# pmandros/node2vec2rank

Hardware: AMD Instinct MI355X
Metric: nodes ranked/sec + SpMM HBM GB/s, K-layer N-node graph at 1/2/4/8 GPUs (higher is better)
Workload: dtype fp32; 1 GPU; cfg4: 2-layer ER N=1M avg-deg 50, dims {8,16,32,64,128} x {cosine,euclidean}, sequential; nodes=1000000, layers=2, embed_dim=128, columns=10, comparisons=1, parallelism=single GPU

## Files before the change

### include/n2v2r.h

```cpp
#ifndef N2V2R_H
#define N2V2R_H

#include <stddef.h>
#include <stdint.h>

#ifdef __cplusplus
extern "C" {
#endif

typedef enum {
  N2V2R_OK = 0,
  N2V2R_ERR_BAD_ARG = 1,
  N2V2R_ERR_UNSUPPORTED_METRIC = 2,
  N2V2R_ERR_NO_CONVERGENCE = 3,
  N2V2R_ERR_HIP = 4,
  N2V2R_ERR_OUT_OF_MEMORY = 5,
  N2V2R_ERR_NOT_READY = 6,
  N2V2R_ERR_UNSUPPORTED_AGG = 7,
  N2V2R_ERR_INTERNAL = 8,
  N2V2R_ERR_RCCL = 9
} n2v2r_status;

enum { N2V2R_SEQUENTIAL = 0, N2V2R_ONE_VS_BEFORE = 1, N2V2R_ONE_VS_REST = 2 };
enum { N2V2R_COSINE = 0, N2V2R_EUCLIDEAN = 1, N2V2R_CORRELATION = 2 };
enum { N2V2R_SYM_DETECT = -1, N2V2R_SYM_NO = 0, N2V2R_SYM_YES = 1 };
enum { N2V2R_AGG_BORDA = 0, N2V2R_AGG_NONE = -1 };

enum { N2V2R_EIG_FULL_FIRST_PASS = 1, N2V2R_EIG_DENSE_RR = 2,
       N2V2R_EIG_TEST_REDO_CYCLE = 4 ,
       N2V2R_EIG_TEST_BAND_FAIL = 8 ,
       N2V2R_EIG_TEST_STURM_FAIL = 32 ,
       N2V2R_EIG_TIME_SPMM = 16 ,
       N2V2R_EIG_TEST_NO_STAGNATION = 64 ,
       N2V2R_EIG_TEST_FAIL_ALONE = 128  };

typedef struct n2v2r_handle n2v2r_handle;
typedef struct n2v2r_simgroup n2v2r_simgroup;

typedef struct {
  int block;
  int max_basis;
  int keep;
  int max_restarts;
  double tol;
  uint64_t seed;
  int solver_flags;
} n2v2r_eig_opts;

typedef struct {
  int restarts;
  int block_applications;
  int converged;
  int basis;
  double max_residual;
  double ms_total, ms_spmm, ms_ortho, ms_rr_host;
  int64_t spmm_launches;
  double spmm_algo_bytes;
  int stagnated;
  int rr_fallbacks;
  double gpu_ms_spmm[2];
  int64_t spmm_timed_launches[2];
  double spmm_stage_bytes[2];
  double est_scale;
  int lean_checks;
  int pool_blocks;
  int spmm_form;
  double stag_cap;
  int y_captured;
  int tri_fallbacks;
} n2v2r_eig_stats;

int n2v2r_create(int device, n2v2r_handle** out);
void n2v2r_destroy(n2v2r_handle* h);
int n2v2r_last_error(const n2v2r_handle* h, char* buf, size_t len);
const char* n2v2r_version(void);

#define N2V2R_UNIQUE_ID_BYTES 128
int n2v2r_comm_unique_id(char* out, size_t len);
int n2v2r_create_rccl(int device, int rank, int world, const char* unique_id, n2v2r_handle** out);
int n2v2r_simgroup_create(int world, n2v2r_simgroup** out);
void n2v2r_simgroup_destroy(n2v2r_simgroup* g);
int n2v2r_create_sim(int device, n2v2r_simgroup* g, int rank, n2v2r_handle** out);
int n2v2r_dist_info(const n2v2r_handle* h, int* rank, int* world, int64_t* row0, int64_t* n_local);

int n2v2r_create_multi(const int* devices, int n_gpus, n2v2r_handle** out);
int n2v2r_multi_devices(const n2v2r_handle* h, int* devices, int cap);

int n2v2r_set_num_layers(n2v2r_handle* h, int num_layers, int64_t n);
int n2v2r_set_layer_csr(n2v2r_handle* h, int k, int64_t n, int64_t nnz, const int64_t* indptr,
                        const int32_t* indices, const float* data, int symmetric);
int n2v2r_set_layer_dense(n2v2r_handle* h, int k, int64_t n, const float* A, int symmetric);
enum { N2V2R_CORR_UNSIGNED = 0, N2V2R_CORR_SIGNED = 1, N2V2R_CORR_SIGNED_HYBRID = 2,
       N2V2R_CORR_RAW = 3 };
int n2v2r_set_layer_corr(n2v2r_handle* h, int k, int64_t n, int64_t samples,
                         const double* E , int kind, double power);
int n2v2r_set_layer_csr_rows(n2v2r_handle* h, int k, int64_t n, int64_t row0, int64_t n_rows,
                             int64_t nnz, const int64_t* indptr, const int32_t* indices,
                             const float* data);

int n2v2r_uase(n2v2r_handle* h, int d, const n2v2r_eig_opts* opts, n2v2r_eig_stats* stats);
int n2v2r_get_embedding(n2v2r_handle* h, float* Y );
int n2v2r_get_left_embedding(n2v2r_handle* h, float* X );
int n2v2r_get_singular_values(n2v2r_handle* h, double* s );
int n2v2r_set_embedding(n2v2r_handle* h, int num_layers, int64_t n, int d, const float* Y);

int n2v2r_rank(n2v2r_handle* h, int strategy, const int* dims, int n_dims, const int* metrics,
               int n_metrics, int method, int* n_comparisons, int* n_cols);
int n2v2r_get_distances(n2v2r_handle* h, int comparison, double* D );
int n2v2r_get_borda(n2v2r_handle* h, int comparison, int64_t* borda );
int n2v2r_rank_timing(n2v2r_handle* h, double* ms_distances, double* ms_borda);

int n2v2r_pairwise_distances(n2v2r_handle* h, const double* m1, const double* m2, int64_t n,
                             int dim, int metric, double* out);
int n2v2r_borda_columns(n2v2r_handle* h, const double* D , int64_t n,
                        int n_cols, int64_t* borda);
int n2v2r_column_sums(n2v2r_handle* h, int k, float* out );
int n2v2r_borda_columns_ex(n2v2r_handle* h, const double* D , int64_t n,
                           int n_cols, const int32_t* given_cols, int n_given,
                           const int32_t* given_orders, int64_t* borda, int32_t* tied);

int n2v2r_project(n2v2r_handle* h, int64_t m, int64_t n, const double* W, int on_columns,
                  double* out);

int n2v2r_synchronize(n2v2r_handle* h);


#ifdef __cplusplus
}
#endif

#endif
```

### include/n2v2r_diag.h

```cpp
#ifndef N2V2R_DIAG_H
#define N2V2R_DIAG_H

#include "n2v2r.h"

#ifdef __cplusplus
extern "C" {
#endif

int n2v2r_bench_spmm(n2v2r_handle* h, int k, int transpose, int b, int reps, const float* X,
                     float* Y, double* avg_ms, double* algo_bytes);
int n2v2r_bench_spmm_tiled(n2v2r_handle* h, int k, int transpose, int b, int nb, int reps,
                           const float* X, float* Y, double* avg_ms);

int n2v2r_spmm_col_blocks(const n2v2r_handle* h, int b);

int n2v2r_rr_top(n2v2r_handle* h, int c, const double* H, int p, double* w, float* S);

int n2v2r_rr_band_top(n2v2r_handle* h, int c, int kp, const double* hband, int64_t hband_len,
                      const double* theta_prev, int p, double* w, float* S);

int n2v2r_h2d_layer_bytes(const n2v2r_handle* h, int64_t* per_rank, int cap);

int n2v2r_get_layer_dense(n2v2r_handle* h, int k, float* A );

#ifdef __cplusplus
}
#endif

#endif
```

### node2vec2rank_amd/_lib.py

```python
from __future__ import annotations

import atexit
import ctypes
import os
import threading
import weakref

import numpy as np

from .coexpression import Coexpression

_HERE = os.path.dirname(os.path.abspath(__file__))
LIB_PATH = os.environ.get("N2V2R_LIB", os.path.join(_HERE, "lib", "libn2v2r_hip.so"))

OK = 0
ERR_BAD_ARG = 1
ERR_UNSUPPORTED_METRIC = 2
ERR_NO_CONVERGENCE = 3
ERR_HIP = 4
ERR_OUT_OF_MEMORY = 5
ERR_NOT_READY = 6
ERR_UNSUPPORTED_AGG = 7
ERR_INTERNAL = 8
ERR_RCCL = 9
AGG_BORDA, AGG_NONE = 0, -1
EIG_TIME_SPMM = 16
EIG_TEST_NO_STAGNATION = 64
EIG_TEST_FAIL_ALONE = 128

STRATEGY = {"sequential": 0, "one_vs_before": 1, "one_vs_rest": 2}
METRIC = {"cosine": 0, "euclidean": 1, "correlation": 2}
SYM_DETECT, SYM_NO, SYM_YES = -1, 0, 1

EXPORTED = [
    "n2v2r_create", "n2v2r_destroy", "n2v2r_last_error", "n2v2r_version",
    "n2v2r_set_num_layers", "n2v2r_set_layer_csr", "n2v2r_uase", "n2v2r_get_embedding",
    "n2v2r_get_left_embedding", "n2v2r_get_singular_values", "n2v2r_set_embedding",
    "n2v2r_rank", "n2v2r_get_distances", "n2v2r_get_borda", "n2v2r_rank_timing",
    "n2v2r_pairwise_distances", "n2v2r_borda_columns", "n2v2r_borda_columns_ex",
    "n2v2r_column_sums",
    "n2v2r_synchronize", "n2v2r_bench_spmm", "n2v2r_bench_spmm_tiled", "n2v2r_spmm_col_blocks",
    "n2v2r_comm_unique_id", "n2v2r_create_rccl", "n2v2r_simgroup_create",
    "n2v2r_simgroup_destroy", "n2v2r_create_sim", "n2v2r_dist_info", "n2v2r_set_layer_csr_rows",
    "n2v2r_rr_top", "n2v2r_rr_band_top", "n2v2r_set_layer_dense", "n2v2r_project",
    "n2v2r_create_multi", "n2v2r_multi_devices", "n2v2r_h2d_layer_bytes",
    "n2v2r_set_layer_corr", "n2v2r_get_layer_dense",
]
UNIQUE_ID_BYTES = 128


class ArpackNoConvergence(RuntimeError):
    """UASE eigensolver did not reach the residual tolerance (scipy raises
    ``ArpackNoConvergence`` in the reference's svds path)."""


class EigOpts(ctypes.Structure):
    _fields_ = [("block", ctypes.c_int), ("max_basis", ctypes.c_int), ("keep", ctypes.c_int),
                ("max_restarts", ctypes.c_int), ("tol", ctypes.c_double),
                ("seed", ctypes.c_uint64), ("solver_flags", ctypes.c_int)]


class EigStats(ctypes.Structure):
    _fields_ = [("restarts", ctypes.c_int), ("block_applications", ctypes.c_int),
                ("converged", ctypes.c_int), ("basis", ctypes.c_int),
                ("max_residual", ctypes.c_double), ("ms_total", ctypes.c_double),
                ("ms_spmm", ctypes.c_double), ("ms_ortho", ctypes.c_double),
                ("ms_rr_host", ctypes.c_double), ("spmm_launches", ctypes.c_int64),
                ("spmm_algo_bytes", ctypes.c_double), ("stagnated", ctypes.c_int),
                ("rr_fallbacks", ctypes.c_int), ("gpu_ms_spmm", ctypes.c_double * 2),
                ("spmm_timed_launches", ctypes.c_int64 * 2),
                ("spmm_stage_bytes", ctypes.c_double * 2), ("est_scale", ctypes.c_double),
                ("lean_checks", ctypes.c_int), ("pool_blocks", ctypes.c_int),
                ("spmm_form", ctypes.c_int), ("stag_cap", ctypes.c_double),
                ("y_captured", ctypes.c_int), ("tri_fallbacks", ctypes.c_int)]

    def as_dict(self):
        out = {}
        for k, _ in self._fields_:
            v = getattr(self, k)
            out[k] = list(v) if isinstance(v, ctypes.Array) else v
        return out


_lib = None
_lock = threading.RLock()

_vp = ctypes.c_void_p
_i = ctypes.c_int
_i64 = ctypes.c_int64


def _p(dtype):
    return np.ctypeslib.ndpointer(dtype=dtype, flags="C_CONTIGUOUS")


def load(path: str | None = None):
    global _lib
    with _lock:
        if _lib is not None:
            return _lib
        p = path or LIB_PATH
        if not os.path.exists(p):
            raise RuntimeError(
                f"n2v2r HIP library not found at {p}; build it with "
                "`python -m node2vec2rank_amd.build` (there is no CPU fallback)")
        lib = ctypes.CDLL(p)
        atexit.register(_teardown)
        sig = {
            "n2v2r_create": (_i, [_i, ctypes.POINTER(_vp)]),
            "n2v2r_destroy": (None, [_vp]),
            "n2v2r_last_error": (_i, [_vp, ctypes.c_char_p, ctypes.c_size_t]),
            "n2v2r_version": (ctypes.c_char_p, []),
            "n2v2r_set_num_layers": (_i, [_vp, _i, _i64]),
            "n2v2r_set_layer_csr": (_i, [_vp, _i, _i64, _i64, _p(np.int64), _p(np.int32),
                                         _p(np.float32), _i]),
            "n2v2r_uase": (_i, [_vp, _i, ctypes.POINTER(EigOpts), ctypes.POINTER(EigStats)]),
            "n2v2r_get_embedding": (_i, [_vp, _p(np.float32)]),
            "n2v2r_get_left_embedding": (_i, [_vp, _p(np.float32)]),
            "n2v2r_get_singular_values": (_i, [_vp, _p(np.float64)]),
            "n2v2r_set_embedding": (_i, [_vp, _i, _i64, _i, _p(np.float32)]),
            "n2v2r_rank": (_i, [_vp, _i, _p(np.int32), _i, _p(np.int32), _i, _i,
                                ctypes.POINTER(_i), ctypes.POINTER(_i)]),
            "n2v2r_get_distances": (_i, [_vp, _i, _p(np.float64)]),
            "n2v2r_get_borda": (_i, [_vp, _i, _p(np.int64)]),
            "n2v2r_rank_timing": (_i, [_vp, ctypes.POINTER(ctypes.c_double),
                                       ctypes.POINTER(ctypes.c_double)]),
            "n2v2r_pairwise_distances": (_i, [_vp, _p(np.float64), _p(np.float64), _i64, _i, _i,
                                              _p(np.float64)]),
            "n2v2r_borda_columns": (_i, [_vp, _p(np.float64), _i64, _i, _p(np.int64)]),
            "n2v2r_borda_columns_ex": (_i, [_vp, _p(np.float64), _i64, _i, _vp, _i, _vp,
                                            _p(np.int64), _p(np.int32)]),
            "n2v2r_column_sums": (_i, [_vp, _i, _p(np.float32)]),
            "n2v2r_synchronize": (_i, [_vp]),
            "n2v2r_bench_spmm": (_i, [_vp, _i, _i, _i, _i, _p(np.float32), _vp,
                                      ctypes.POINTER(ctypes.c_double),
                                      ctypes.POINTER(ctypes.c_double)]),
            "n2v2r_bench_spmm_tiled": (_i, [_vp, _i, _i, _i, _i, _i, _p(np.float32), _vp,
                                            ctypes.POINTER(ctypes.c_double)]),
            "n2v2r_spmm_col_blocks": (_i, [_vp, _i]),
            "n2v2r_rr_top": (_i, [_vp, _i, _p(np.float64), _i, _p(np.float64), _p(np.float32)]),
            "n2v2r_rr_band_top": (_i, [_vp, _i, _i, _p(np.float64), ctypes.c_int64, _vp, _i,
                                       _p(np.float64), _p(np.float32)]),
            "n2v2r_set_layer_dense": (_i, [_vp, _i, _i64, _p(np.float32), _i]),
            "n2v2r_project": (_i, [_vp, _i64, _i64, _p(np.float64), _i, _p(np.float64)]),
            "n2v2r_comm_unique_id": (_i, [ctypes.c_char_p, ctypes.c_size_t]),
            "n2v2r_create_rccl": (_i, [_i, _i, _i, ctypes.c_char_p, ctypes.POINTER(_vp)]),
            "n2v2r_simgroup_create": (_i, [_i, ctypes.POINTER(_vp)]),
            "n2v2r_simgroup_destroy": (None, [_vp]),
            "n2v2r_create_sim": (_i, [_i, _vp, _i, ctypes.POINTER(_vp)]),
            "n2v2r_dist_info": (_i, [_vp, ctypes.POINTER(_i), ctypes.POINTER(_i),
                                     ctypes.POINTER(_i64), ctypes.POINTER(_i64)]),
            "n2v2r_set_layer_csr_rows": (_i, [_vp, _i, _i64, _i64, _i64, _i64, _p(np.int64),
                                              _p(np.int32), _p(np.float32)]),
            "n2v2r_create_multi": (_i, [_p(np.int32), _i, ctypes.POINTER(_vp)]),
            "n2v2r_multi_devices": (_i, [_vp, _vp, _i]),
            "n2v2r_h2d_layer_bytes": (_i, [_vp, _vp, _i]),
            "n2v2r_set_layer_corr": (_i, [_vp, _i, _i64, _i64, _p(np.float64), _i,
                                          ctypes.c_double]),
            "n2v2r_get_layer_dense": (_i, [_vp, _i, _p(np.float32)]),
        }
        for name, (res, args) in sig.items():
            f = getattr(lib, name)
            f.restype = res
            f.argtypes = args
        _lib = lib
        return lib


def comm_unique_id() -> bytes:
    lib = load()
    buf = ctypes.create_string_buffer(UNIQUE_ID_BYTES)
    st = lib.n2v2r_comm_unique_id(buf, UNIQUE_ID_BYTES)
    if st != OK:
        raise RuntimeError(f"n2v2r_comm_unique_id failed with status {st}")
    return buf.raw


class SimGroup:

    def __init__(self, world: int):
        self.lib = load()
        g = _vp()
        st = self.lib.n2v2r_simgroup_create(int(world), ctypes.byref(g))
        if st != OK:
            raise RuntimeError(f"n2v2r_simgroup_create failed with status {st}")
        self.g = g
        self.world = int(world)

    def close(self):
        if getattr(self, "g", None):
            self.lib.n2v2r_simgroup_destroy(self.g)
            self.g = None


_live = weakref.WeakSet()


def _teardown():
    for eng in list(_live):
        try:
            eng.close()
        except Exception:
            pass
    path = os.environ.get("N2V2R_EXIT_MAPS")
    if path:
        try:
            with open("/proc/self/maps") as src, open(path, "w") as dst:
                dst.write(src.read())
        except OSError:
            pass


class Engine:

    def __init__(self, device: int = 0, _handle=None):
        self.lib = load()
        if _handle is None:
            h = _vp()
            st = self.lib.n2v2r_create(int(device), ctypes.byref(h))
            if st != OK:
                raise RuntimeError(
                    f"n2v2r_create(device={device}) failed with status {st}: no usable HIP GPU "
                    "(the engine has no CPU fallback)")
        else:
            h = _handle
        self.h = h
        self.device = device
        _live.add(self)

    @classmethod
    def rccl(cls, device: int, rank: int, world: int, unique_id: bytes) -> "Engine":
        lib = load()
        h = _vp()
        st = lib.n2v2r_create_rccl(int(device), int(rank), int(world), bytes(unique_id),
                                   ctypes.byref(h))
        if st != OK:
            raise RuntimeError(f"n2v2r_create_rccl(rank={rank}, world={world}) failed: {st}")
        return cls(device, _handle=h)

    @classmethod
    def multi(cls, devices) -> "Engine":
        lib = load()
        devs = np.ascontiguousarray([int(d) for d in devices], dtype=np.int32)
        h = _vp()
        st = lib.n2v2r_create_multi(devs, int(devs.size), ctypes.byref(h))
        if st != OK:
            raise RuntimeError(f"n2v2r_create_multi(devices={devs.tolist()}) failed with status "
                               f"{st}" + (" (RCCL)" if st == ERR_RCCL else ""))
        eng = cls(int(devs[0]), _handle=h)
        eng.devices = tuple(int(d) for d in devs)
        return eng

    @classmethod
    def sim(cls, device: int, group: SimGroup, rank: int) -> "Engine":
        lib = load()
        h = _vp()
        st = lib.n2v2r_create_sim(int(device), group.g, int(rank), ctypes.byref(h))
        if st != OK:
            raise RuntimeError(f"n2v2r_create_sim(rank={rank}) failed with status {st}")
        return cls(device, _handle=h)

    def h2d_layer_bytes(self):
        out = np.zeros(64, dtype=np.int64)
        w = self.lib.n2v2r_h2d_layer_bytes(self.h, out.ctypes.data_as(ctypes.c_void_p), 64)
        if w < 0:
            self._check(w, "h2d_layer_bytes")
        return [int(x) for x in out[:w]]

    def dist_info(self):
        r, w, r0, nl = _i(), _i(), _i64(), _i64()
        self._check(self.lib.n2v2r_dist_info(self.h, ctypes.byref(r), ctypes.byref(w),
                                             ctypes.byref(r0), ctypes.byref(nl)), "dist_info")
        return r.value, w.value, r0.value, nl.value

    def close(self):
        if getattr(self, "h", None):
            self.lib.n2v2r_destroy(self.h)
            self.h = None

    def __del__(self):
        try:
            self.close()
        except Exception:
            pass

    def _err(self) -> str:
        buf = ctypes.create_string_buffer(1024)
        self.lib.n2v2r_last_error(self.h, buf, len(buf))
        return buf.value.decode(errors="replace")

    def _check(self, st: int, what: str):
        if st == OK:
            return
        msg = f"{what}: {self._err()}"
        if st == ERR_UNSUPPORTED_METRIC:
            raise NotImplementedError("Unsupported metric")
        if st == ERR_UNSUPPORTED_AGG:
            raise NotImplementedError("Aggregation method not found. Available methods: Borda")
        if st == ERR_NOT_READY:
            raise ValueError("No n2v2r embeddings found")
        if st == ERR_NO_CONVERGENCE:
            raise ArpackNoConvergence(msg)
        if st == ERR_OUT_OF_MEMORY:
            raise MemoryError(msg)
        if st == ERR_BAD_ARG:
            raise ValueError(msg)
        if st == ERR_RCCL:
            raise RuntimeError(f"RCCL failure: {msg}")
        raise RuntimeError(msg)

    def set_layers(self, layers, symmetric=SYM_DETECT, storage="auto"):
        import scipy.sparse as sp
        corr = [isinstance(a, Coexpression) for a in layers]
        if any(corr):
            if storage == "csr":
                raise ValueError("Coexpression layers are stored dense: storage='csr' does not "
                                 "apply")
            if any(sp.issparse(a) for a in layers):
                raise ValueError("a sparse layer cannot share a handle with Coexpression layers "
                                 "(all layers of a handle are CSR or all dense): pass it as a "
                                 "dense array")
            arrs = [a if c else np.ascontiguousarray(np.asarray(a), dtype=np.float32)
                    for a, c in zip(layers, corr)]
            n = arrs[0].shape[0]
            for a in arrs:
                if a.shape != (n, n):
                    raise ValueError("all layers must be square and share the node set")
            self._check(self.lib.n2v2r_set_num_layers(self.h, len(arrs), n), "set_num_layers")
            for k, a in enumerate(arrs):
                if isinstance(a, Coexpression):
                    st = self.lib.n2v2r_set_layer_corr(self.h, k, n, a.expression.shape[1],
                                                       a.expression, a.kind_id, a.power)
                else:
                    st = self.lib.n2v2r_set_layer_dense(self.h, k, n, a, int(symmetric))
                self._check(st, f"layer {k}")
            self.n = n
            self.num_layers = len(arrs)
            self.storage = "dense"
            return
        if storage == "auto":
            storage = "csr"
            if all(not sp.issparse(a) for a in layers):
                arrs = [np.asarray(a) for a in layers]
                if all(_denser_than_quarter(a) for a in arrs):
                    storage = "dense"
        if storage == "dense":
            arrs = [np.ascontiguousarray(np.asarray(a.todense() if sp.issparse(a) else a),
                                         dtype=np.float32) for a in layers]
            n = arrs[0].shape[0]
            for a in arrs:
                if a.shape != (n, n):
                    raise ValueError("all layers must be square and share the node set")
            self._check(self.lib.n2v2r_set_num_layers(self.h, len(arrs), n), "set_num_layers")
            for k, a in enumerate(arrs):
                self._check(self.lib.n2v2r_set_layer_dense(self.h, k, n, a, int(symmetric)),
                            f"layer {k}")
            self.n = n
            self.num_layers = len(arrs)
            self.storage = "dense"
            return
        mats = [sp.csr_matrix(a, dtype=np.float32) for a in layers]
        n = mats[0].shape[0]
        for m in mats:
            if m.shape != (n, n):
                raise ValueError("all layers must be square and share the node set")
        self._check(self.lib.n2v2r_set_num_layers(self.h, len(mats), n), "set_num_layers")
        for k, m in enumerate(mats):
            indptr = np.ascontiguousarray(m.indptr, dtype=np.int64)
            indices = np.ascontiguousarray(m.indices, dtype=np.int32)
            data = np.ascontiguousarray(m.data, dtype=np.float32)
            self._check(self.lib.n2v2r_set_layer_csr(self.h, k, n, int(m.nnz), indptr, indices,
                                                     data, int(symmetric)), f"layer {k}")
        self.n = n
        self.num_layers = len(mats)
        self.storage = "csr"

    def set_layer_rows(self, n: int, num_layers: int, local_layers):
        import scipy.sparse as sp
        self._check(self.lib.n2v2r_set_num_layers(self.h, int(num_layers), int(n)),
                    "set_num_layers")
        _, _, row0, nl = self.dist_info()
        for k, blk in enumerate(local_layers):
            m = sp.csr_matrix(blk, dtype=np.float32)
            m.sum_duplicates()
            m.sort_indices()
            if m.shape != (nl, n):
                raise ValueError(f"layer {k}: local block must be {nl} x {n}, got {m.shape}")
            self._check(self.lib.n2v2r_set_layer_csr_rows(
                self.h, k, int(n), int(row0), int(nl), int(m.nnz),
                np.ascontiguousarray(m.indptr, dtype=np.int64),
                np.ascontiguousarray(m.indices, dtype=np.int32),
                np.ascontiguousarray(m.data, dtype=np.float32)), f"layer {k} rows")
        self.n = int(n)
        self.num_layers = int(num_layers)

    def uase(self, d: int, block=0, max_basis=0, keep=0, max_restarts=0, tol=0.0, seed=0,
             solver_flags=0, raise_on_no_convergence=True):
        o = EigOpts(int(block), int(max_basis), int(keep), int(max_restarts), float(tol),
                    int(seed) & 0xFFFFFFFFFFFFFFFF, int(solver_flags))
        s = EigStats()
        st = self.lib.n2v2r_uase(self.h, int(d), ctypes.byref(o), ctypes.byref(s))
        if st == ERR_NO_CONVERGENCE and not raise_on_no_convergence:
            pass
        else:
            self._check(st, "uase")
        self.d = int(d)
        return s.as_dict()

    def _n_local(self):
        return self.dist_info()[3]

    def embedding(self):
        Y = np.empty((self.num_layers, self._n_local(), self.d), dtype=np.float32)
        self._check(self.lib.n2v2r_get_embedding(self.h, Y), "get_embedding")
        return Y

    def left_embedding(self):
        X = np.empty((self._n_local(), self.d), dtype=np.float32)
        self._check(self.lib.n2v2r_get_left_embedding(self.h, X), "get_left_embedding")
        return X

    def singular_values(self):
        s = np.empty(self.d, dtype=np.float64)
        self._check(self.lib.n2v2r_get_singular_values(self.h, s), "get_singular_values")
        return s

    def set_embedding(self, Y):
        Y = np.ascontiguousarray(Y, dtype=np.float32)
        K, n, d = Y.shape
        self._check(self.lib.n2v2r_set_embedding(self.h, K, n, d, Y), "set_embedding")
        self.num_layers, self.n, self.d = K, n, d

    def rank(self, strategy: str, dims, metrics, method: int = AGG_BORDA):
        if strategy not in STRATEGY:
            raise ValueError(f"unknown comp_strategy {strategy!r}")
        mids = []
        for m in metrics:
            if m not in METRIC:
                raise NotImplementedError("Unsupported metric")
            mids.append(METRIC[m])
        dims_a = np.ascontiguousarray(dims, dtype=np.int32)
        met_a = np.ascontiguousarray(mids, dtype=np.int32)
        ncmp = ctypes.c_int()
        ncol = ctypes.c_int()
        self._check(self.lib.n2v2r_rank(self.h, STRATEGY[strategy], dims_a, len(dims_a), met_a,
                                        len(met_a), int(method), ctypes.byref(ncmp),
                                        ctypes.byref(ncol)), "rank")
        self.ncmp, self.ncols = ncmp.value, ncol.value
        return self.ncmp, self.ncols

    def distances(self, comparison: int):
        D = np.empty((self.ncols, self.n), dtype=np.float64)
        self._check(self.lib.n2v2r_get_distances(self.h, int(comparison), D), "get_distances")
        return D.T

    def borda(self, comparison: int):
        b = np.empty(self.n, dtype=np.int64)
        self._check(self.lib.n2v2r_get_borda(self.h, int(comparison), b), "get_borda")
        return b

    def rank_timing(self):
        a, b = ctypes.c_double(), ctypes.c_double()
        self.lib.n2v2r_rank_timing(self.h, ctypes.byref(a), ctypes.byref(b))
        return a.value, b.value

    def pairwise_distances(self, m1, m2, metric: str):
        if metric not in METRIC:
            raise NotImplementedError("Unsupported metric")
        a = np.ascontiguousarray(m1, dtype=np.float64)
        b = np.ascontiguousarray(m2, dtype=np.float64)
        if a.ndim == 1:
            a = a[:, None]
            b = b[:, None]
        n, dim = a.shape
        out = np.empty(n, dtype=np.float64)
        self._check(self.lib.n2v2r_pairwise_distances(self.h, a, b, n, dim, METRIC[metric], out),
                    "pairwise_distances")
        return out

    def borda_columns(self, D, tie_order: str = "stable", return_tied: bool = False):
        if tie_order not in ("stable", "reference"):
            raise ValueError(f"unknown tie_order {tie_order!r}")
        Dc = np.ascontiguousarray(np.asarray(D, dtype=np.float64).T)
        c, n = Dc.shape
        out = np.empty(n, dtype=np.int64)
        tied = np.zeros(c, dtype=np.int32)
        self._check(self.lib.n2v2r_borda_columns_ex(self.h, Dc, n, c, None, 0, None, out, tied),
                    "borda_columns")
        cols = np.flatnonzero(tied)
        if tie_order == "reference" and cols.size:
            orders = np.empty((cols.size, n), dtype=np.int32)
            for g, j in enumerate(cols):
                orders[g] = reference_descending_order(Dc[j])
            gc = np.ascontiguousarray(cols, dtype=np.int32)
            self._check(self.lib.n2v2r_borda_columns_ex(
                self.h, Dc, n, c, gc.ctypes.data_as(_vp), int(cols.size),
                orders.ctypes.data_as(_vp), out, tied), "borda_columns")
        return (out, tied.astype(bool)) if return_tied else out

    def column_sums(self, k: int):
        out = np.empty(self.n, dtype=np.float32)
        self._check(self.lib.n2v2r_column_sums(self.h, int(k), out), "column_sums")
        return out

    def layer_dense(self, k: int):
        A = np.zeros((self.n, self.n), dtype=np.float32)
        self._check(self.lib.n2v2r_get_layer_dense(self.h, int(k), A), "layer_dense")
        return A

    def bench_spmm(self, k: int, X, transpose: bool = False, reps: int = 20, want_y=True):
        X = np.ascontiguousarray(X, dtype=np.float32)
        n, b = X.shape
        Y = np.empty((self._n_local(), b), dtype=np.float32) if want_y else None
        ms, by = ctypes.c_double(), ctypes.c_double()
        yp = Y.ctypes.data_as(ctypes.c_void_p) if want_y else None
        self._check(self.lib.n2v2r_bench_spmm(self.h, int(k), int(bool(transpose)), int(b),
                                              int(reps), X, yp, ctypes.byref(ms),
                                              ctypes.byref(by)), "bench_spmm")
        return Y, ms.value, by.value

    def bench_spmm_tiled(self, k: int, X, transpose: bool = False, nb: int = 0, reps: int = 20,
                         want_y=True):
        X = np.ascontiguousarray(X, dtype=np.float32)
        n, b = X.shape
        Y = np.empty((self._n_local(), b), dtype=np.float32) if want_y else None
        ms = ctypes.c_double()
        yp = Y.ctypes.data_as(ctypes.c_void_p) if want_y else None
        self._check(self.lib.n2v2r_bench_spmm_tiled(self.h, int(k), int(bool(transpose)), int(b),
                                                    int(nb), int(reps), X, yp, ctypes.byref(ms)),
                    "bench_spmm_tiled")
        return Y, ms.value

    def spmm_col_blocks(self, b: int = 8) -> bool:
        r = self.lib.n2v2r_spmm_col_blocks(self.h, int(b))
        if r < 0 or r > 1:
            self._check(r, "spmm_col_blocks")
        return r == 1

    def project(self, W, on: str = "columns"):
        W = np.ascontiguousarray(np.asarray(W), dtype=np.float64)
        m, n = W.shape
        oc = on.casefold() == "columns"
        if not oc and on.casefold() != "rows":
            raise ValueError("Unknown projection type, options are columns or rows")
        k = n if oc else m
        out = np.empty((k, k), dtype=np.float64)
        self._check(self.lib.n2v2r_project(self.h, m, n, W, int(oc), out), "project")
        return out

    def rr_top(self, H, p: int):
        H = np.ascontiguousarray(H, dtype=np.float64)
        c = H.shape[0]
        w = np.empty(p, dtype=np.float64)
        S = np.empty((c, p), dtype=np.float32)
        self._check(self.lib.n2v2r_rr_top(self.h, c, H, int(p), w, S), "rr_top")
        return w, S

    def rr_band_top(self, hband, c: int, kp: int, theta_prev, p: int):
        hband = np.ascontiguousarray(hband, dtype=np.float64).ravel()
        tp = None
        if kp > 0:
            tp = np.ascontiguousarray(theta_prev, dtype=np.float64)
        w = np.empty(p, dtype=np.float64)
        S = np.empty((c, p), dtype=np.float32)
        self._check(self.lib.n2v2r_rr_band_top(
            self.h, int(c), int(kp), hband, int(hband.size),
            None if tp is None else tp.ctypes.data_as(ctypes.c_void_p), int(p), w, S),
            "rr_band_top")
        return w, S

    def synchronize(self):
        self._check(self.lib.n2v2r_synchronize(self.h), "synchronize")


def reference_descending_order(col) -> np.ndarray:
    import pandas as pd
    return pd.Series(np.asarray(col, dtype=np.float64)).sort_values(
        ascending=False).index.to_numpy(dtype=np.int64)


_default = {}


def new_engine(device) -> Engine:
    if isinstance(device, tuple):
        return Engine.multi(device)
    return Engine(device)


def default_engine(device: int = 0) -> Engine:
    e = _default.get(device)
    if e is None or e.h is None:
        e = Engine(device)
        _default[device] = e
    return e


def _denser_than_quarter(a) -> bool:
    if a.size == 0:
        return False
    a2 = a.reshape(a.shape[0], -1) if a.ndim > 1 else a.reshape(1, -1)
    rows, cols = a2.shape
    stride = max(1, rows // max(1, (1 << 21) // max(1, cols)))
    if stride > 1:
        sample = a2[::stride]
        p = np.count_nonzero(sample) / sample.size
        if p > 0.3:
            return True
        if p < 0.2:
            return False
    need = a.size // 4
    step = max(1, (1 << 24) // max(1, cols))
    nz = 0
    for r in range(0, rows, step):
        nz += int(np.count_nonzero(a2[r:r + step]))
        if nz > need:
            return True
        if nz + (rows - r - step) * cols <= need:
            return False
    return nz > need


POOL_MAX = 4
_pool = {}
_pool_tick = [0]


def engine_owner(eng: Engine):
    ref = getattr(eng, "_owner", None)
    return ref() if ref is not None else None


def acquire_engine(device: int, owner) -> Engine:
    import weakref
    with _lock:
        handles = _pool.setdefault(device, [])
        handles[:] = [e for e in handles if e.h is not None]
        free = [e for e in handles if engine_owner(e) is None]
        if free:
            eng = free[0]
        elif len(handles) < POOL_MAX:
            eng = new_engine(device)
            handles.append(eng)
        else:
            eng = min(handles, key=lambda e: getattr(e, "_tick", 0))
            prev = engine_owner(eng)
            if prev is not None and hasattr(prev, "_hand_over"):
                prev._hand_over()
        _pool_tick[0] += 1
        eng._tick = _pool_tick[0]
        eng._owner = weakref.ref(owner)
        return eng
```

### node2vec2rank_amd/build.py

```python
from __future__ import annotations

import os
import subprocess
import sys

HERE = os.path.dirname(os.path.abspath(__file__))
CSRC = os.path.join(HERE, "csrc")
OUT_DIR = os.path.join(HERE, "lib")
_TAG = os.environ.get("N2V2R_BUILD_TAG", "")
LIB = os.path.join(OUT_DIR, f"libn2v2r_hip_{_TAG}.so" if _TAG else "libn2v2r_hip.so")
OBJ_DIR = os.path.join(OUT_DIR, f"obj_{_TAG}" if _TAG else "obj")

HIP_SOURCES = ["spmm.hip", "dense.hip", "gemm.hip", "corr.hip", "rank.hip", "rr.hip", "rr_band.hip",
               "rr_sturm.hip", "ingest.hip", "engine.cpp", "layers.cpp", "comm.cpp", "solver.cpp",
               "ranking.cpp", "multi.cpp"]
HOST_SOURCES: list = []
HEADERS = ["common.h", "spmm_args.h", "engine.h", os.path.join("..", "..", "include", "n2v2r.h"),
           os.path.join("..", "..", "include", "n2v2r_diag.h")]
ARCH = os.environ.get("N2V2R_OFFLOAD_ARCH", "gfx950")
_EXTRA = os.environ.get("N2V2R_EXTRA_HIP_FLAGS", "").split() if _TAG else []


def _hipcc():
    for c in (os.environ.get("HIPCC"), "/opt/rocm/bin/hipcc", "hipcc"):
        if c and (os.path.isabs(c) and os.path.exists(c) or not os.path.isabs(c)):
            return c
    raise RuntimeError("hipcc not found")


def _newer(target, deps):
    if not os.path.exists(target):
        return True
    t = os.path.getmtime(target)
    return any(os.path.getmtime(d) > t for d in deps if os.path.exists(d))


def build(force: bool = False, verbose: bool = False) -> str:
    os.makedirs(OBJ_DIR, exist_ok=True)
    hipcc = _hipcc()
    headers = [os.path.join(CSRC, h) for h in HEADERS]
    objs, cmds = [], []
    for src in HIP_SOURCES + HOST_SOURCES:
        path = os.path.join(CSRC, src)
        obj = os.path.join(OBJ_DIR, src + ".o")
        objs.append(obj)
        if not force and not _newer(obj, [path, __file__] + headers):
            continue
        if src in HIP_SOURCES:
            lang = ["-x", "hip"]
            cmd = [hipcc, *lang, f"--offload-arch={ARCH}", "-O3", "-std=c++17", "-fPIC",
                   "-munsafe-fp-atomics", *_EXTRA, "-c", path, "-o", obj]
        else:
            cmd = ["g++", "-O3", "-march=x86-64-v3", "-std=c++17", "-fPIC", "-c", path, "-o", obj]
        cmds.append(cmd)
    from concurrent.futures import ThreadPoolExecutor
    jobs = max(1, min(8, len(cmds), os.cpu_count() or 1))

    def _run(cmd):
        if verbose:
            print(" ".join(cmd), flush=True)
        subprocess.run(cmd, check=True)

    with ThreadPoolExecutor(jobs) as ex:
        list(ex.map(_run, cmds))
    if force or _newer(LIB, objs):
        tmp = LIB + ".tmp"
        cmd = [hipcc, f"--offload-arch={ARCH}", "-shared", "-fPIC", *objs, "-o", tmp,
               "-L/opt/rocm/lib", "-lrccl", "-Wl,-rpath,/opt/rocm/lib"]
        if verbose:
            print(" ".join(cmd), flush=True)
        subprocess.run(cmd, check=True)
        os.replace(tmp, LIB)
    return LIB


if __name__ == "__main__":
    print(build(force="--force" in sys.argv, verbose=True))
```

### node2vec2rank_amd/csrc/engine.cpp

```cpp
#include "engine.h"

using namespace n2v2r_int;

namespace n2v2r_int {
n2v2r_handle* new_handle(int device) {
  int count = 0;
  if (hipGetDeviceCount(&count) != hipSuccess || count <= 0) return nullptr;
  if (device < 0 || device >= count) return nullptr;
  auto* h = new (std::nothrow) n2v2r_handle();
  if (!h) return nullptr;
  h->device = device;
  if (hipSetDevice(device) != hipSuccess ||
      hipStreamCreateWithFlags(&h->stream, hipStreamNonBlocking) != hipSuccess) {
    delete h;
    return nullptr;
  }
  return h;
}

}

extern "C" {

const char* n2v2r_version(void) { return "n2v2r-mi355x 0.2.0 (gfx950)"; }

int n2v2r_create(int device, n2v2r_handle** out) {
  if (!out) return N2V2R_ERR_BAD_ARG;
  *out = nullptr;
  int count = 0;
  if (hipGetDeviceCount(&count) != hipSuccess || count <= 0) return N2V2R_ERR_HIP;
  if (device < 0 || device >= count) return N2V2R_ERR_BAD_ARG;
  n2v2r_handle* h = new_handle(device);
  if (!h) return N2V2R_ERR_HIP;
  *out = h;
  return N2V2R_OK;
}

void n2v2r_destroy(n2v2r_handle* h) {
  if (!h) return;
  if (h->multi()) {
    (void)multi_destroy(h);
    return;
  }
  (void)hipSetDevice(h->device);
  if (h->stream) (void)hipStreamSynchronize(h->stream);
  h->layers.clear();
  h->comm.reset();
  for (hipEvent_t& e : h->cb_ev)
    if (e) (void)hipEventDestroy(e);
  if (h->side) (void)hipStreamDestroy(h->side);
  if (h->pin) (void)hipHostFree(h->pin);
  for (hipEvent_t e : h->tev) (void)hipEventDestroy(e);
  if (h->cstream) (void)hipStreamSynchronize(h->cstream);
  for (hipEvent_t& e : h->cev)
    if (e) (void)hipEventDestroy(e);
  if (h->cstream) (void)hipStreamDestroy(h->cstream);
  if (h->stream) (void)hipStreamDestroy(h->stream);
  delete h;
}

int n2v2r_last_error(const n2v2r_handle* h, char* buf, size_t len) {
  if (!h || !buf || len == 0) return N2V2R_ERR_BAD_ARG;
  snprintf(buf, len, "%s", h->err.c_str());
  return N2V2R_OK;
}

int n2v2r_synchronize(n2v2r_handle* h) {
  if (h && h->multi()) return multi_synchronize(h);
  return guarded(h, [&]() -> int {
    HIPCHK(hipStreamSynchronize(h->stream));
    return N2V2R_OK;
  });
}

int n2v2r_rr_top(n2v2r_handle* h, int c, const double* H, int p, double* w, float* S) {
  if (h && h->multi()) h = h->ranks[0];
  return guarded(h, [&]() -> int {
    if (c < 3 || c > 768 || p < 1 || p > c || !H || !w || !S) return N2V2R_ERR_BAD_ARG;
    DevBuf a, tri, refl, y, s;
    a.ensure(sizeof(double) * c * c);
    tri.ensure(sizeof(double) * 3 * c);
    refl.ensure(sizeof(double) * c * c);
    y.ensure(sizeof(double) * c * p);
    s.ensure(sizeof(float) * c * p);
    HIPCHK(hipMemcpyAsync(a.p, H, sizeof(double) * c * c, hipMemcpyHostToDevice, h->stream));
    HIPCHK(hipStreamSynchronize(h->stream));
    double* t = tri.as<double>();
    DevBuf trs;
    trs.ensure(n2v2r_rr_tridiag_scratch_bytes(c));
    HIPCHK(n2v2r_launch_rr_tridiag(a.as<double>(), c, t, t + c, t + 2 * c, refl.as<double>(),
                                   trs.p, h->stream));
    DevBuf wd, scr;
    wd.ensure(sizeof(double) * p);
    scr.ensure(sizeof(double) * 6 * (size_t)((p + 63) / 64 * 64) * c);
    HIPCHK(n2v2r_launch_rr_tri_eig(t, t + c, c, p, wd.as<double>(), y.as<double>(),
                                   scr.as<double>(), h->stream));
    HIPCHK(hipMemcpyAsync(w, wd.p, sizeof(double) * p, hipMemcpyDeviceToHost, h->stream));
    DevBuf btf;
    btf.ensure(n2v2r_rr_bt_scratch_bytes(c));
    HIPCHK(n2v2r_launch_rr_backtransform(refl.as<double>(), t + 2 * c, c, y.as<double>(), p,
                                         s.as<float>(), p, btf.as<double>(), h->stream));
    HIPCHK(hipMemcpyAsync(S, s.p, sizeof(float) * c * p, hipMemcpyDeviceToHost, h->stream));
    HIPCHK(hipStreamSynchronize(h->stream));
    return N2V2R_OK;
  });
}

int n2v2r_rr_band_top(n2v2r_handle* h, int c, int kp, const double* hband, int64_t hband_len,
                      const double* theta_prev, int p, double* w, float* S) {
  if (h && h->multi()) h = h->ranks[0];
  return guarded(h, [&]() -> int {
    const int b = 8;
    if (c < 3 || c > 512 || c % b || kp % b || kp + b > 192 || kp >= c || p < 1 || p > c ||
        !hband || !w || !S || (kp > 0 && !theta_prev))
      return N2V2R_ERR_BAD_ARG;
    const int64_t need = (int64_t)(kp + b) * b + (int64_t)(c / b - kp / b - 1) * 2 * b * b;
    if (hband_len < need) return N2V2R_ERR_BAD_ARG;
    DevBuf hb, th, ab, va, ta, tri, y, s, er, rf;
    rf.ensure(sizeof(double) * c * n2v2r_rr_band_jm(c) * 9);
    hb.ensure(sizeof(double) * hband_len);
    th.ensure(sizeof(double) * c);
    ab.ensure(sizeof(double) * c * (b + 1));
    va.ensure(sizeof(double) * (kp + b) * (kp + b));
    ta.ensure(sizeof(double) * (kp + b));
    tri.ensure(sizeof(double) * 2 * c);
    y.ensure(sizeof(double) * c * p);
    s.ensure(sizeof(float) * c * p);
    er.ensure(4 * sizeof(int));
    HIPCHK(hipMemsetAsync(er.p, 0, 4 * sizeof(int), h->stream));
    HIPCHK(hipMemcpyAsync(hb.p, hband, sizeof(double) * hband_len, hipMemcpyHostToDevice,
                          h->stream));
    if (kp > 0)
      HIPCHK(hipMemcpyAsync(th.p, theta_prev, sizeof(double) * kp, hipMemcpyHostToDevice,
                            h->stream));
    HIPCHK(hipStreamSynchronize(h->stream));
    if (rr_sturm_enabled()) {
      DevBuf scr;
      scr.ensure(sizeof(double) * n2v2r_rr_sturm_scratch(c, p));
      HIPCHK(n2v2r_launch_rr_sturm(hb.as<double>(), c, kp, th.as<double>(), scr.as<double>(),
                                   scr.bytes / sizeof(double), y.as<double>(), s.as<float>(), p,
                                   p, er.as<int>(), h->stream));
      int e = 0;
      HIPCHK(hipMemcpyAsync(&e, er.p, sizeof(int), hipMemcpyDeviceToHost, h->stream));
      HIPCHK(hipMemcpyAsync(w, th.p, sizeof(double) * p, hipMemcpyDeviceToHost, h->stream));
      HIPCHK(hipMemcpyAsync(S, s.p, sizeof(float) * c * p, hipMemcpyDeviceToHost, h->stream));
      HIPCHK(hipStreamSynchronize(h->stream));
      if (!e) return N2V2R_OK;
      HIPCHK(hipMemsetAsync(er.p, 0, 4 * sizeof(int), h->stream));
      if (kp > 0)
        HIPCHK(hipMemcpyAsync(th.p, theta_prev, sizeof(double) * kp, hipMemcpyHostToDevice,
                              h->stream));
      HIPCHK(hipStreamSynchronize(h->stream));
    }
    HIPCHK(n2v2r_launch_rr_band(hb.as<double>(), c, kp, th.as<double>(), ab.as<double>(),
                                va.as<double>(), ta.as<double>(), tri.as<double>(),
                                tri.as<double>() + c, rf.as<double>(), y.as<double>(),
                                s.as<float>(), p, p, er.as<int>(), h->stream));
    int e = 0;
    HIPCHK(hipMemcpyAsync(&e, er.p, sizeof(int), hipMemcpyDeviceToHost, h->stream));
    HIPCHK(hipMemcpyAsync(w, th.p, sizeof(double) * p, hipMemcpyDeviceToHost, h->stream));
    HIPCHK(hipMemcpyAsync(S, s.p, sizeof(float) * c * p, hipMemcpyDeviceToHost, h->stream));
    HIPCHK(hipStreamSynchronize(h->stream));
    if (e) throw StatusFail{N2V2R_ERR_NO_CONVERGENCE, "banded Rayleigh-Ritz: bulge chase aborted"};
    return N2V2R_OK;
  });
}

int n2v2r_spmm_col_blocks(const n2v2r_handle* h, int b) {
  if (h && h->multi()) h = h->ranks[0];
  if (!h) return N2V2R_ERR_BAD_ARG;
  return col_blocks_wanted(h, b) ? 1 : 0;
}

static int time_tiled(n2v2r_handle* h, int k, int transpose, int nb, const float* xd, float* yd,
                      int reps, double* avg_ms, int b = 8) {
  if (nb <= 0) {
    nb = 4;
    while (nb < 64 && (double)h->n * 32.0 / nb > 2.0 * 1024 * 1024) nb *= 2;
  }
  if (nb != 4 && nb != 8 && nb != 16 && nb != 32 && nb != 64 && nb != 128) return N2V2R_ERR_BAD_ARG;
  LayerDev& L = *h->layers[k];
  const int wb = tile_wbits(h->layers, nb);
  if (!ensure_col_blocks(L, h->n, h->stream, nb, wb)) return N2V2R_ERR_BAD_ARG;
  const LayerDev::ColBlocks& cbs = (transpose && !L.symmetric) ? L.cb_t : L.cb;
  DevBuf tb;
  tb.ensure(sizeof(CsrBlk) * nb);
  HIPCHK(hipMemcpyAsync(tb.p, cbs.blk, sizeof(CsrBlk) * nb, hipMemcpyHostToDevice, h->stream));
  int ncu = 0;
  HIPCHK(hipDeviceGetAttribute(&ncu, hipDeviceAttributeMultiprocessorCount, h->device));
  SpmmTileArgs a{};
  a.blk = tb.as<CsrBlk>();
  a.X[0] = xd;
  a.Y[0] = yd;
  a.ldx = b;
  a.ldy = b;
  a.n = h->nloc;
  a.K = 1;
  a.nb = nb;
  a.sum = 0;
  a.tile_rows = n2v2r_spmm_tile_rows_b(h->nloc, ncu, b == 16 ? N2V2R_SPMM16_WPC : 2, wb, b);
  a.wbits = wb;
  a.width = b;
  HIPCHK(n2v2r_launch_spmm_tile(a, h->stream));
  hipEvent_t e0, e1;
  HIPCHK(hipEventCreate(&e0));
  HIPCHK(hipEventCreate(&e1));
  HIPCHK(hipEventRecord(e0, h->stream));
  for (int r = 0; r < reps; ++r) HIPCHK(n2v2r_launch_spmm_tile(a, h->stream));
  HIPCHK(hipEventRecord(e1, h->stream));
  HIPCHK(hipEventSynchronize(e1));
  float ms = 0.f;
  HIPCHK(hipEventElapsedTime(&ms, e0, e1));
  (void)hipEventDestroy(e0);
  (void)hipEventDestroy(e1);
  if (avg_ms) *avg_ms = (double)ms / reps;
  HIPCHK(hipStreamSynchronize(h->stream));
  return N2V2R_OK;
}

int n2v2r_bench_spmm(n2v2r_handle* h, int k, int transpose, int b, int reps, const float* X,
                     float* Y, double* avg_ms, double* algo_bytes) {
  if (h && h->multi()) h = h->ranks[0];
  return guarded(h, [&]() -> int {
    if (k < 0 || k >= h->K || !h->layers[k]->loaded || (b != 8 && b != 16 && b != 32 && b != 64) ||
        reps < 1 || !X)
      return N2V2R_ERR_BAD_ARG;
    const LayerDev& L = *h->layers[k];
    DevBuf xd, yd;
    xd.ensure(sizeof(float) * h->n * b);
    yd.ensure(sizeof(float) * std::max<int64_t>(h->nloc, 1) * b);
    HIPCHK(hipMemcpyAsync(xd.p, X, sizeof(float) * h->n * b, hipMemcpyHostToDevice, h->stream));
    if (L.dense) {
      const float* am = transpose ? L.dense_at() : L.dense_a();
      const float* bt = h->comm ? nullptr : (transpose ? L.dense_a() : L.dense_at());
      h->dense_apply(am, L.lda, xd.as<float>(), b, b, yd.as<float>(), b, 0.f, nullptr, bt);
      hipEvent_t e0, e1;
      HIPCHK(hipEventCreate(&e0));
      HIPCHK(hipEventCreate(&e1));
      HIPCHK(hipEventRecord(e0, h->stream));
      for (int r = 0; r < reps; ++r)
        h->dense_apply(am, L.lda, xd.as<float>(), b, b, yd.as<float>(), b, 0.f, nullptr, bt);
      HIPCHK(hipEventRecord(e1, h->stream));
      HIPCHK(hipEventSynchronize(e1));
      float ms = 0.f;
      HIPCHK(hipEventElapsedTime(&ms, e0, e1));
      (void)hipEventDestroy(e0);
      (void)hipEventDestroy(e1);
      if (avg_ms) *avg_ms = (double)ms / reps;
      if (algo_bytes)
        *algo_bytes = 4.0 * (double)h->nloc * (double)h->n + 4.0 * (double)(h->n + h->nloc) * b;
      if (Y)
        HIPCHK(hipMemcpyAsync(Y, yd.p, sizeof(float) * h->nloc * b, hipMemcpyDeviceToHost,
                              h->stream));
      HIPCHK(hipStreamSynchronize(h->stream));
      return N2V2R_OK;
    }
    if (col_blocks_wanted(h, b)) {
      double ms = 0.0;
      const int st_ = time_tiled(h, k, transpose, 0, xd.as<float>(), yd.as<float>(), reps, &ms);
      if (st_ == N2V2R_OK) {
        const CsrDev c0 = transpose ? L.csr_t() : L.csr();
        if (avg_ms) *avg_ms = ms;
        if (algo_bytes) *algo_bytes = spmm_algo_bytes(c0.nnz, c0.unit != 0, h->nloc, h->n, b);
        if (Y)
          HIPCHK(hipMemcpyAsync(Y, yd.p, sizeof(float) * h->nloc * b, hipMemcpyDeviceToHost,
                                h->stream));
        HIPCHK(hipStreamSynchronize(h->stream));
        return N2V2R_OK;
      }
    }
    SpmmArgs a{};
    a.K = 1;
    a.sum = 0;
    a.ldx = b;
    a.ldy = b;
    a.colscale = nullptr;
    a.A[0] = transpose ? L.csr_t() : L.csr();
    a.X[0] = xd.as<float>();
    a.Y[0] = yd.as<float>();
    HIPCHK(n2v2r_launch_spmm(a, b, h->stream));
    hipEvent_t e0, e1;
    HIPCHK(hipEventCreate(&e0));
    HIPCHK(hipEventCreate(&e1));
    HIPCHK(hipEventRecord(e0, h->stream));
    for (int r = 0; r < reps; ++r) HIPCHK(n2v2r_launch_spmm(a, b, h->stream));
    HIPCHK(hipEventRecord(e1, h->stream));
    HIPCHK(hipEventSynchronize(e1));
    float ms = 0.f;
    HIPCHK(hipEventElapsedTime(&ms, e0, e1));
    (void)hipEventDestroy(e0);
    (void)hipEventDestroy(e1);
    if (avg_ms) *avg_ms = (double)ms / reps;
    if (algo_bytes)
      *algo_bytes = spmm_algo_bytes(a.A[0].nnz, a.A[0].unit != 0, h->nloc, h->n, b);
    if (Y)
      HIPCHK(hipMemcpyAsync(Y, yd.p, sizeof(float) * h->nloc * b, hipMemcpyDeviceToHost,
                            h->stream));
    HIPCHK(hipStreamSynchronize(h->stream));
    return N2V2R_OK;
  });
}


int n2v2r_bench_spmm_tiled(n2v2r_handle* h, int k, int transpose, int b, int nb, int reps,
                           const float* X, float* Y, double* avg_ms) {
  if (h && h->multi()) h = h->ranks[0];
  return guarded(h, [&]() -> int {
    if (k < 0 || k >= h->K || !h->layers[k]->loaded || h->layers[k]->dense ||
        (b != 8 && b != 16) || reps < 1 || !X || h->comm)
      return N2V2R_ERR_BAD_ARG;
    DevBuf xd, yd;
    xd.ensure(sizeof(float) * h->n * b);
    yd.ensure(sizeof(float) * std::max<int64_t>(h->nloc, 1) * b);
    HIPCHK(hipMemcpyAsync(xd.p, X, sizeof(float) * h->n * b, hipMemcpyHostToDevice, h->stream));
    const int st_ =
        time_tiled(h, k, transpose, nb, xd.as<float>(), yd.as<float>(), reps, avg_ms, b);
    if (st_ != N2V2R_OK) return st_;
    if (Y)
      HIPCHK(hipMemcpyAsync(Y, yd.p, sizeof(float) * h->nloc * b, hipMemcpyDeviceToHost,
                            h->stream));
    HIPCHK(hipStreamSynchronize(h->stream));
    return N2V2R_OK;
  });
}

}
```

### node2vec2rank_amd/csrc/engine.h

```cpp
#pragma once

#include <hip/hip_runtime.h>
#include <rccl/rccl.h>

#include <algorithm>
#include <chrono>
#include <cmath>
#include <condition_variable>
#include <cstdarg>
#include <cstdlib>
#include <cstdio>
#include <cstring>
#include <memory>
#include <mutex>
#include <numeric>
#include <string>
#include <thread>
#include <exception>
#include <system_error>
#include <vector>

#include "../../include/n2v2r.h"
#include "../../include/n2v2r_diag.h"
#include "common.h"

#include "spmm_args.h"
#define DIST_MAX_COLS 256
struct DistPlan {
  int n_cols;
  int col_dim[DIST_MAX_COLS];
  int col_metric[DIST_MAX_COLS];
  int col_out[DIST_MAX_COLS];
  int dmax;
};
extern "C" {
hipError_t n2v2r_launch_spmm(const SpmmArgs& args, int B, hipStream_t stream);
int n2v2r_spmm_rpw(const SpmmArgs& args, int B);
hipError_t n2v2r_launch_row_sums(const CsrDev& A, float* out, hipStream_t stream);
hipError_t n2v2r_launch_spmm_tile(const SpmmTileArgs& a, hipStream_t stream);
hipError_t n2v2r_launch_chunk_major_keys(uint64_t* keys, int64_t nnz, int64_t npad, int W,
                                         int64_t rc, hipStream_t stream);
int n2v2r_spmm_tile_rows(int64_t n, int ncu, int wpc, int wbits);
int n2v2r_spmm_tile_rows_b(int64_t n, int ncu, int wpc, int wbits, int b);
hipError_t n2v2r_launch_cb_count(const CsrDev& A, int64_t cw, int nb, int32_t* cnt,
                                 hipStream_t stream);
hipError_t n2v2r_launch_cb_rowptrs(const int32_t* cnt, int64_t n, int nb, int64_t nnz,
                                   int64_t* tsum, size_t tsum_elems, int64_t* rp, int32_t* wo,
                                   int wbits, hipStream_t stream);
int64_t n2v2r_cb_scan_tiles(int64_t n, int nb);
hipError_t n2v2r_launch_cb_fill(const CsrDev& A, int64_t cw, int nb, const int64_t* rp,
                                int32_t* idx, float* dat, int cbits, int wbits,
                                hipStream_t stream);
hipError_t n2v2r_launch_ts_tn(const BlockList& A, const BlockList& B, int64_t n, double* partial,
                              size_t partial_elems, double* out, const int* cond,
                              hipStream_t stream);
hipError_t n2v2r_launch_ritz_nn(const BlockList& A0, const BlockList& A1, const float* G, int ldg,
                                int cb, const OutBlockList& O0, const OutBlockList& O1, int64_t n,
                                int grid, hipStream_t stream);
hipError_t n2v2r_launch_ts_nn(const BlockList& A, const float* G, int ldg, int cb,
                              const OutBlockList& O, const BlockList& C, float alpha, float beta,
                              int64_t n, const int* cond, const int* flags, uint64_t seed,
                              hipStream_t stream);
hipError_t n2v2r_launch_pip_chol(const double* G, int c, int b, double* xinv, int* flags,
                                 int* any_flag, const int* cond, double* save, int save_row0,
                                 int save_rows, float* fout, int* sticky, double* rsave,
                                 int first, hipStream_t stream);
hipError_t n2v2r_launch_rr_band(const double* hband, int c, int kp, double* theta, double* AB,
                                double* Varr, double* taua, double* d, double* e, double* refl,
                                double* Y, float* S, int ldS, int p, int* err,
                                hipStream_t stream);
int n2v2r_rr_band_jm(int c);
inline bool pip_fused() { return true; }
hipError_t n2v2r_launch_ts_tn2(const BlockList& A, const float* Za, const float* Zb, int64_t n,
                               double* partial, size_t partial_elems, double* out,
                               hipStream_t stream);
hipError_t n2v2r_launch_rmul8(const double* r2, double* r1, hipStream_t stream);
hipError_t n2v2r_launch_pair_fixup(double* g2, int nblk_all, int nq_old, double* ra,
                                   hipStream_t stream);
constexpr size_t N2V2R_PAIR_PLAN_WORDS = 208 + (size_t)(N2V2R_BAND_MAXC / 8) * 129;
hipError_t n2v2r_launch_pip_pair(const BlockList& Q, float* Za, float* Zb, double* g2, int64_t n,
                                 int* flags, int* any_flag, int* sticky, uint64_t seed_a,
                                 uint64_t seed_b, int64_t row0, float skip_tol, int* skipped,
                                 int* plan, size_t plan_bytes, hipStream_t stream);
hipError_t n2v2r_launch_pip_fused(const BlockList& Q, const float* Zin, float* Zout,
                                  const double* G, int c, int64_t n, const int* cond, int* flags,
                                  int* any_flag, double* save, int save_row0, int save_rows,
                                  int* sticky, uint64_t seed, int64_t row0, double* rsave,
                                  float skip_tol, int* skipped, int first, hipStream_t stream);
hipError_t n2v2r_launch_pip_apply(const BlockList& QZ, const float* F, int c, int b,
                                  const OutBlockList& Z, int64_t n, const int* cond,
                                  const int* flags, uint64_t seed, int64_t row0,
                                  hipStream_t stream);
hipError_t n2v2r_launch_fill_normal(float* blk, int w, int64_t n, uint64_t seed, const int* flags,
                                    const int* cond, uint64_t ctr0, hipStream_t stream);
hipError_t n2v2r_launch_resid(const BlockList& X, const BlockList& MX, const double* theta,
                              int64_t n, double* partial, size_t partial_elems, double* out,
                              hipStream_t stream);
hipError_t n2v2r_launch_scale_cols(float* blk, int w, int64_t n, const float* s,
                                   hipStream_t stream);
hipError_t n2v2r_launch_colmax_keys(const float* U, int64_t ldu, int64_t n, int d, int64_t row0,
                                    unsigned long long* keys, size_t key_elems,
                                    unsigned long long* best, hipStream_t stream);
hipError_t n2v2r_launch_colmax_sign(const unsigned long long* best, int ncols_padded,
                                    const float* U, int64_t ldu, int d, int64_t row0, int64_t n,
                                    float* sign, hipStream_t stream);
hipError_t n2v2r_launch_distances(const float* Y, int K, int64_t n, int64_t ldy, int64_t lrows,
                                  int strategy, int layer_i, const DistPlan& plan, double* out,
                                  int64_t ldo, hipStream_t stream);
hipError_t n2v2r_launch_pairwise(const double* a, const double* b, int64_t n, int dim, int metric,
                                 double* out, hipStream_t stream);
hipError_t n2v2r_launch_borda_init(const double* vals, int64_t n, int nseg, uint64_t* keys,
                                   int32_t* idx, unsigned long long* seg_or,
                                   unsigned long long* seg_and, hipStream_t stream);
int n2v2r_radix_tiles(int64_t n);
size_t n2v2r_radix_hist_elems(int64_t n, int nseg);
hipError_t n2v2r_launch_radix_pass(const uint64_t* kin, const int32_t* pin, uint64_t* kout,
                                   int32_t* pout, int64_t n, int nseg, int shift, uint32_t* hist,
                                   hipStream_t stream);
hipError_t n2v2r_launch_borda_finish(const int32_t* sorted_idx, int64_t n, int nseg, int ncols,
                                     int32_t* pos, int64_t* borda, hipStream_t stream);
hipError_t n2v2r_launch_tie_flags(const uint64_t* sorted_keys, int64_t n, int nseg, int32_t* tied,
                                  hipStream_t stream);
hipError_t n2v2r_launch_dense_tn(const float* B, int64_t ldb, int64_t ncols, int64_t kdim,
                                 const float* X, int ldx, int b, float* Y, int64_t ldy, float beta,
                                 const float* colscale, float* work, size_t work_elems,
                                 hipStream_t stream);
hipError_t n2v2r_launch_dense_gemm(const float* A, int64_t lda, int64_t rows, int64_t kdim,
                                   const float* X, int ldx, int b, float* Y, int64_t ldy,
                                   float beta, const float* colscale, float* work,
                                   size_t work_elems, hipStream_t stream);
hipError_t n2v2r_launch_syrk_f64(const double* W, int64_t sk, int64_t si, int64_t kd, int64_t r,
                                 double* out, int64_t ldo, hipStream_t stream);
int64_t n2v2r_corr_spad(int64_t s);
hipError_t n2v2r_launch_corr_standardise(const double* E, int64_t n, int64_t s, double* Z,
                                         unsigned* bad, hipStream_t stream);
hipError_t n2v2r_launch_corr_tiles(const double* Z, int64_t s, int64_t n, int64_t row0,
                                   int64_t nloc, float* A, int64_t lda, int kind, double power,
                                   hipStream_t stream);
hipError_t n2v2r_launch_transpose(const float* in, int64_t ldi, int64_t rows, int64_t cols,
                                  float* out, int64_t ldo, hipStream_t stream);
hipError_t n2v2r_launch_mismatch(const float* a, const float* b, int64_t ld, int64_t rows,
                                 int64_t cols, unsigned long long* count, hipStream_t stream);
hipError_t n2v2r_launch_rr_tridiag(double* A, int c, double* d, double* e, double* tau, double* V,
                                   void* scratch, hipStream_t stream);
size_t n2v2r_rr_tridiag_scratch_bytes(int c);
int* n2v2r_rr_tridiag_err(void* scratch, int c);
hipError_t n2v2r_launch_rr_tri_eig(const double* d, const double* e, int c, int p, double* w,
                                   double* Y, double* scratch, hipStream_t stream);
hipError_t n2v2r_launch_rr_backtransform(const double* V, const double* tau, int c,
                                         const double* Y, int p, float* S, int lds, double* tfac,
                                         hipStream_t stream);
size_t n2v2r_rr_bt_scratch_bytes(int c);
hipError_t n2v2r_launch_lds_poison(hipStream_t stream);
hipError_t n2v2r_launch_nonfinite(const void* p, int64_t count, int f64, int* flag,
                                  hipStream_t stream);
hipError_t n2v2r_launch_ts_tn_zsum(const BlockList& A, int64_t n, const float* const* parts,
                                   int count, float* zout, double* partial, size_t partial_elems,
                                   double* out, hipStream_t stream);
hipError_t n2v2r_launch_pack_words(void* const* src, const int* dst_word, const int* words,
                                   const int* clear, int count, void* dst, hipStream_t stream);
hipError_t n2v2r_launch_zsum(const float* const* parts, int count, float* zout, int64_t n,
                             hipStream_t stream);
hipError_t n2v2r_launch_rr_sturm(const double* hband, int c, int kp, double* theta, double* scr,
                                 size_t scr_elems, double* Y, float* S, int ldS, int p, int* err,
                                 hipStream_t stream);
size_t n2v2r_rr_sturm_scratch(int c, int p);
hipError_t n2v2r_launch_rr_band_expand(const double* hband, int c, int kp, const double* theta,
                                       double* H, hipStream_t stream);
hipError_t n2v2r_launch_csr_scan(const int64_t* ip, const int32_t* ix, const float* dv,
                                 int64_t n_rows, int64_t n_cols, uint64_t* keys, int32_t* idx,
                                 unsigned* flags, hipStream_t stream);
hipError_t n2v2r_launch_csr_from_sorted(const uint64_t* keys, const int32_t* idx, const float* dv,
                                        int64_t nnz, int64_t n_cols, int64_t* tp, int32_t* tx,
                                        float* td, hipStream_t stream);
hipError_t n2v2r_launch_csr_compare(const int64_t* ap, const int32_t* ax, const float* av,
                                    const int64_t* bp, const int32_t* bx, const float* bv,
                                    int64_t n_rows, int64_t nnz, unsigned* flag,
                                    hipStream_t stream);
hipError_t n2v2r_launch_csr_rebase(const int64_t* ip, int64_t r0, int64_t nr, int64_t* out,
                                   hipStream_t stream);
}

inline bool rr_sturm_enabled() {
  const char* e = std::getenv("N2V2R_RR");
  return !(e && e[0] == 'b');
}

inline bool ritz_nn_enabled() { return true; }

inline bool lean_enabled() {
  const char* e = std::getenv("N2V2R_LEAN_W");
  return !(e && e[0] == '0');
}


namespace n2v2r_int {

struct HipFail {
  hipError_t e;
  std::string where;
};
struct StatusFail {
  int code;
  std::string msg;
};

#define HIPCHK(expr)                                                  \
  do {                                                                \
    hipError_t _e = (expr);                                           \
    if (_e != hipSuccess) throw HipFail{_e, #expr};                   \
  } while (0)

inline double now_ms() {
  using namespace std::chrono;
  return duration<double, std::milli>(steady_clock::now().time_since_epoch()).count();
}

inline bool env_flag(const char* name) {
  const char* e = std::getenv(name);
  return e && *e && *e != '0';
}
inline bool debug_poison() {
  static const bool v = env_flag("N2V2R_POISON");
  return v;
}
inline bool debug_finite() {
  static const bool v = env_flag("N2V2R_DEBUG_FINITE");
  return v;
}
inline bool debug_ortho() {
  static const bool v = env_flag("N2V2R_DEBUG_ORTHO");
  return v;
}

struct DevBuf {
  void* p = nullptr;
  size_t bytes = 0;
  DevBuf() = default;
  DevBuf(const DevBuf&) = delete;
  DevBuf& operator=(const DevBuf&) = delete;
  ~DevBuf() { release(); }
  void release() {
    if (p) (void)hipFree(p);
    p = nullptr;
    bytes = 0;
  }
  void ensure(size_t b, hipStream_t st = nullptr) {
    if (bytes >= b && p) return;
    release();
    if (b == 0) b = 16;
    hipError_t e = hipMalloc(&p, b);
    if (e != hipSuccess) {
      p = nullptr;
      throw StatusFail{N2V2R_ERR_OUT_OF_MEMORY,
                       "hipMalloc of " + std::to_string(b) + " bytes failed"};
    }
    const int fill = debug_poison() ? 0xFF : 0;
    if (st) {
      e = hipMemsetAsync(p, fill, b, st);
    } else {
      e = hipMemset(p, fill, b);
      if (e == hipSuccess) e = hipDeviceSynchronize();
    }
    if (e != hipSuccess) throw HipFail{e, "hipMemset"};
    bytes = b;
  }
  void ensure_raw(size_t b) {
    if (bytes >= b && p) return;
    if (b == 0) b = 16;
    if (debug_poison()) return ensure(b);
    release();
    if (hipMalloc(&p, b) != hipSuccess) {
      p = nullptr;
      throw StatusFail{N2V2R_ERR_OUT_OF_MEMORY,
                       "hipMalloc of " + std::to_string(b) + " bytes failed"};
    }
    bytes = b;
  }
  template <class T>
  T* as() const {
    return static_cast<T*>(p);
  }
};

struct LayerDev {
  DevBuf indptr, indices, data;
  DevBuf t_indptr, t_indices, t_data;
  int64_t nnz = 0, t_nnz = 0;
  int64_t n_rows = 0;
  bool unit = false, t_unit = false;
  bool symmetric = true;
  bool loaded = false;
  bool dense = false;
  DevBuf dA, dAT;
  int64_t lda = 0;
  const float* dense_a() const { return dA.as<float>(); }
  const float* dense_at() const { return symmetric ? dA.as<float>() : dAT.as<float>(); }
  CsrDev csr() const {
    return CsrDev{indptr.as<int64_t>(), indices.as<int32_t>(), data.as<float>(), n_rows, nnz,
                  unit ? 1 : 0};
  }
  CsrDev csr_t() const {
    if (symmetric) return csr();
    return CsrDev{t_indptr.as<int64_t>(), t_indices.as<int32_t>(), t_data.as<float>(), n_rows,
                  t_nnz, t_unit ? 1 : 0};
  }
  struct ColBlocks {
    DevBuf wo, idx, dat;
    CsrBlk blk[CB_MAX];
    int nb = 0;
    int wbits = 0;
    int cbits = 0;
    int64_t ncols = 0;
    bool built = false;
    bool usable = false;
  };
  ColBlocks cb, cb_t;
  DevBuf c_indptr, c_indices, c_data;
  int64_t c_nnz = 0, c_rows = 0;
  int64_t c_rc = 0;
  bool c_built = false;
  CsrDev csr_c() const {
    return CsrDev{c_indptr.as<int64_t>(), c_indices.as<int32_t>(), c_data.as<float>(), c_rows,
                  c_nnz, (symmetric ? unit : t_unit) ? 1 : 0};
  }
  void drop_col_blocks() {
    for (ColBlocks* c : {&cb, &cb_t}) {
      c->wo.release();
      c->idx.release();
      c->dat.release();
      c->built = false;
    }
    c_indptr.release();
    c_indices.release();
    c_data.release();
    c_built = false;
  }
};

void build_col_blocks(const CsrDev& A, int64_t ncols, LayerDev::ColBlocks& out, hipStream_t st,
                      int nb, int wbits);
bool ensure_col_blocks(LayerDev& L, int64_t ncols, hipStream_t st, int nb, int wbits);
int tile_wbits(const std::vector<std::unique_ptr<LayerDev>>& layers, int nb);
void ensure_colcsr(LayerDev& L, int64_t ncols, int64_t rows_out, hipStream_t st, int64_t npad = 0,
                   int W = 1, int64_t rc = 0);

struct Comm {
  int rank = 0, world = 1;
  virtual ~Comm() = default;
  virtual void allgather(const void* send, void* recv, size_t bytes, hipStream_t st) = 0;
  virtual void allreduce_sum_f64(double* buf, size_t count, hipStream_t st) = 0;
  virtual void allreduce_max_u64(unsigned long long* buf, size_t count, hipStream_t st) = 0;
  virtual void allreduce_sum_f32(float* buf, size_t count, hipStream_t st) = 0;
  virtual void reduce_scatter_sum_f32(const float* send, float* recv, size_t count,
                                      hipStream_t st) = 0;
  virtual const char* kind() const = 0;
  virtual bool shares_device() const { return false; }
  virtual void abort() {}
};

struct NcclFail {
  ncclResult_t r;
  std::string where;
};
#define NCCLCHK(expr)                                   \
  do {                                                  \
    ncclResult_t _r = (expr);                           \
    if (_r != ncclSuccess) throw NcclFail{_r, #expr};   \
  } while (0)

std::unique_ptr<Comm> make_rccl_comm(ncclComm_t c, int rank, int world);
}

struct n2v2r_simgroup {
  int world = 1;
  std::mutex m;
  std::condition_variable cv;
  int arrived = 0;
  uint64_t generation = 0;
  bool aborted = false;
  std::vector<const void*> ptrs;
  std::vector<std::vector<unsigned char>> host;
  std::vector<int> dev;
  void barrier() {
    std::unique_lock<std::mutex> lk(m);
    const uint64_t gen = generation;
    if (aborted) throw n2v2r_int::StatusFail{N2V2R_ERR_INTERNAL, "thread group aborted"};
    if (++arrived == world) {
      arrived = 0;
      ++generation;
      cv.notify_all();
    } else {
      cv.wait(lk, [&] { return generation != gen || aborted; });
      if (generation == gen)
        throw n2v2r_int::StatusFail{N2V2R_ERR_INTERNAL, "thread group aborted"};
    }
  }
  void abort() {
    std::lock_guard<std::mutex> lk(m);
    aborted = true;
    cv.notify_all();
  }
};

namespace n2v2r_int {
std::unique_ptr<Comm> make_thread_comm(n2v2r_simgroup* g, int rank, int device);

struct EigWorkspace {
  std::vector<std::unique_ptr<DevBuf>> pool;
  size_t block_bytes = 0;
  std::vector<std::unique_ptr<DevBuf>> zk;
  DevBuf zg;
  DevBuf rinv, flg, anyflag, gsmall, csmall;
  DevBuf rback;
  DevBuf tri, refl, ytri, tscr;
  DevBuf trcoop;
  DevBuf btf;
  DevBuf hband, band, varr, taua, rrerr;
  DevBuf fcoef;
  DevBuf dbgflag;
  DevBuf tflag;
  DevBuf s2part;
  DevBuf g2, pair_ra;
  DevBuf pair_plan;
  DevBuf sturm;
  DevBuf rres;
  DevBuf skipc;
  DevBuf tblk;
};
}

using n2v2r_int::Comm;
using n2v2r_int::DevBuf;
using n2v2r_int::LayerDev;
using n2v2r_int::EigWorkspace;
using n2v2r_int::HipFail;
using n2v2r_int::StatusFail;

struct n2v2r_handle {
  int device = 0;
  hipStream_t stream = nullptr;
  hipStream_t side = nullptr;
  hipEvent_t cb_ev[2 * SPMM_MAX_LAYERS] = {};
  void* pin = nullptr;
  size_t pin_bytes = 0;
  void ensure_pin(size_t bytes) {
    if (pin_bytes >= bytes) return;
    if (pin) (void)hipHostFree(pin);
    pin = nullptr;
    pin_bytes = 0;
    if (hipHostMalloc(&pin, bytes, hipHostMallocDefault) != hipSuccess) {
      (void)hipGetLastError();
      throw std::bad_alloc();
    }
    pin_bytes = bytes;
  }
  std::string err;
  int K = 0;
  int64_t n = 0;
  std::unique_ptr<Comm> comm;
  int rank = 0, world = 1;
  int64_t row0 = 0, nloc = 0, npad = 0;
  int64_t h2d_layer_bytes = 0;
  std::vector<std::unique_ptr<LayerDev>> layers;

  int d = 0;
  int ldy = 0;
  DevBuf Y;
  DevBuf U;
  std::vector<double> sigma;
  bool have_embedding = false;

  int ncmp = 0, ncols = 0;
  DevBuf D;
  DevBuf Dloc;
  DevBuf Dgat;
  DevBuf borda;
  bool have_borda = false;
  std::vector<hipEvent_t> tev;
  double ms_dist = 0, ms_borda = 0;

  DevBuf partial;
  size_t partial_elems = 0;
  DevBuf theta;
  DevBuf resid;
  DevBuf colscale;
  DevBuf keys, best;
  DevBuf gath;
  EigWorkspace ews;
  DevBuf dense_work;
  size_t dense_work_elems = 0;
  bool dense_layers() const { return !layers.empty() && layers[0]->dense; }
  void dense_apply(const float* Aloc, int64_t lda, const float* X, int ldx, int b, float* Y,
                   int64_t ldy, float beta, const float* colscale, const float* Bt = nullptr) {
    const size_t need = (size_t)std::max<int64_t>(nloc, 1) * b * 16;
    if (dense_work_elems < need) {
      dense_work.ensure(sizeof(float) * need);
      dense_work_elems = need;
    }
    const char* tn = std::getenv("N2V2R_DENSE_TN");
    if (Bt && nloc == n && !(tn && tn[0] == '0')) {
      const hipError_t e = n2v2r_launch_dense_tn(Bt, lda, nloc, n, X, ldx, b, Y, ldy, beta,
                                                 colscale, dense_work.as<float>(),
                                                 dense_work_elems, stream);
      if (e == hipSuccess) return;
      if (e != hipErrorNotSupported) throw HipFail{e, "n2v2r_launch_dense_tn"};
    }
    HIPCHK(n2v2r_launch_dense_gemm(Aloc, lda, nloc, n, X, ldx, b, Y, ldy, beta, colscale,
                                   dense_work.as<float>(), dense_work_elems, stream));
  }
  DevBuf rs_keys[2], rs_idx[2], rs_pos, rs_hist, rs_or, rs_and;
  DevBuf ing_keys[2], ing_pay[2], ing_hist, ing_flag;
  DevBuf ypanel;


  void set_err(const char* fmt, ...) {
    char buf[1024];
    va_list ap;
    va_start(ap, fmt);
    vsnprintf(buf, sizeof(buf), fmt, ap);
    va_end(ap);
    err = buf;
  }

  void set_partition(int64_t n_global) {
    n = n_global;
    if (world <= 1) {
      row0 = 0;
      nloc = npad = n;
      return;
    }
    npad = (n + world - 1) / world;
    row0 = std::min<int64_t>(n, (int64_t)rank * npad);
    nloc = std::max<int64_t>(0, std::min<int64_t>(n, row0 + npad) - row0);
  }

  void gather_panel(const float* local, float* global, int w) {
    if (!comm) {
      if (local != global)
        HIPCHK(hipMemcpyAsync(global, local, sizeof(float) * npad * w, hipMemcpyDeviceToDevice,
                              stream));
      return;
    }
    comm->allgather(local, global, sizeof(float) * npad * w, stream);
  }
  hipStream_t cstream = nullptr;
  hipEvent_t cev[2 * SPMM_MAX_LAYERS] = {};
  void gather_panel_async(const float* local, float* global, int w, int slot) {
    if (!cstream) {
      HIPCHK(hipStreamCreateWithFlags(&cstream, hipStreamNonBlocking));
      for (hipEvent_t& e : cev) HIPCHK(hipEventCreateWithFlags(&e, hipEventDisableTiming));
    }
    HIPCHK(hipEventRecord(cev[2 * slot], stream));
    HIPCHK(hipStreamWaitEvent(cstream, cev[2 * slot], 0));
    comm->allgather(local, global, sizeof(float) * npad * w, cstream);
    HIPCHK(hipEventRecord(cev[2 * slot + 1], cstream));
  }
  void gather_wait(int slot) { HIPCHK(hipStreamWaitEvent(stream, cev[2 * slot + 1], 0)); }
  hipEvent_t rev[SPMM_MAX_LAYERS + 1] = {};
  int rs_pending = 0;
  void reduce_scatter_async(const float* send, float* recv, size_t count) {
    if (!cstream) {
      HIPCHK(hipStreamCreateWithFlags(&cstream, hipStreamNonBlocking));
      for (hipEvent_t& e : cev) HIPCHK(hipEventCreateWithFlags(&e, hipEventDisableTiming));
    }
    if (!rev[0])
      for (hipEvent_t& e : rev) HIPCHK(hipEventCreateWithFlags(&e, hipEventDisableTiming));
    HIPCHK(hipEventRecord(rev[rs_pending], stream));
    HIPCHK(hipStreamWaitEvent(cstream, rev[rs_pending], 0));
    comm->reduce_scatter_sum_f32(send, recv, count, cstream);
    ++rs_pending;
  }
  void rs_wait_all() {
    if (!rs_pending) return;
    HIPCHK(hipEventRecord(rev[SPMM_MAX_LAYERS], cstream));
    HIPCHK(hipStreamWaitEvent(stream, rev[SPMM_MAX_LAYERS], 0));
    rs_pending = 0;
  }
  void allreduce_f64(double* buf, size_t count) {
    if (comm) comm->allreduce_sum_f64(buf, count, stream);
  }

  std::vector<n2v2r_handle*> ranks;
  std::unique_ptr<n2v2r_simgroup> own_group;
  struct n2v2r_int_rank_pool* pool = nullptr;
  bool broken = false;
  bool multi() const { return !ranks.empty(); }
};

namespace n2v2r_int {

template <class F>
int guarded(n2v2r_handle* h, F&& f) {
  if (!h) return N2V2R_ERR_BAD_ARG;
  try {
    hipError_t e = hipSetDevice(h->device);
    if (e != hipSuccess) throw HipFail{e, "hipSetDevice"};
    return f();
  } catch (const HipFail& hf) {
    h->set_err("HIP error %d (%s) at %s", (int)hf.e, hipGetErrorString(hf.e), hf.where.c_str());
    return N2V2R_ERR_HIP;
  } catch (const NcclFail& nf) {
    h->set_err("RCCL error %d (%s) at %s", (int)nf.r, ncclGetErrorString(nf.r), nf.where.c_str());
    return N2V2R_ERR_RCCL;
  } catch (const StatusFail& sf) {
    h->err = sf.msg;
    return sf.code;
  } catch (const std::bad_alloc&) {
    h->err = "host allocation failed";
    return N2V2R_ERR_OUT_OF_MEMORY;
  } catch (const std::exception& ex) {
    h->err = std::string("host error: ") + ex.what();
    return N2V2R_ERR_INTERNAL;
  }
}

int host_threads();
template <class F>
void parallel_chunks(int nt, F&& fn);
bool host_indices_in_range(int64_t nnz, const int32_t* ix, int64_t n);
bool upload_rows(hipStream_t st, int64_t r0, int64_t nr, const int64_t* ip, const int32_t* ix,
                 const float* dv, DevBuf& dip, DevBuf& dix, DevBuf& ddv, int64_t& nnz_out);
bool host_csr_symmetric(int64_t n, const int64_t* ip, const int32_t* ix, const float* dv);
void host_transpose_rows(int64_t n, const int64_t* ip, const int32_t* ix, const float* dv,
                         int64_t r0, int64_t nr, std::vector<int64_t>& tip,
                         std::vector<int32_t>& tix, std::vector<float>& tdv);
int set_layer_rows_directed(n2v2r_handle* h, int k, const int64_t* aip, const int32_t* aix,
                            const float* adv, const int64_t* tip, const int32_t* tix,
                            const float* tdv);

template <class F>
void parallel_chunks(int nt, F&& fn) {
  std::vector<std::thread> pool;
  pool.reserve(nt);
  int t = 0;
  try {
    for (; t < nt; ++t) pool.emplace_back([&fn, t] { fn(t); });
  } catch (const std::system_error&) {
  }
  std::exception_ptr err;
  try {
    for (; t < nt; ++t) fn(t);
  } catch (...) {
    err = std::current_exception();
  }
  for (auto& th : pool) th.join();
  if (err) std::rethrow_exception(err);
}
inline double spmm_algo_bytes(int64_t nnz, bool unit, int64_t rows, int64_t panel_rows, int b) {
  return (unit ? 4.0 : 8.0) * (double)nnz + 8.0 * (double)(rows + 1) +
         4.0 * (double)(panel_rows + rows) * b;
}

bool col_blocks_wanted(const n2v2r_handle* h, int b);
n2v2r_handle* new_handle(int device);
void copy_embedding(n2v2r_handle* h, float* Y, int64_t layer_stride);

int multi_destroy(n2v2r_handle* h);
int multi_synchronize(n2v2r_handle* h);
int multi_set_num_layers(n2v2r_handle* h, int num_layers, int64_t n);
int multi_set_layer_csr(n2v2r_handle* h, int k, int64_t n, int64_t nnz, const int64_t* indptr,
                        const int32_t* indices, const float* data, int symmetric);
int multi_set_layer_dense(n2v2r_handle* h, int k, int64_t n, const float* A, int symmetric);
int multi_set_layer_corr(n2v2r_handle* h, int k, int64_t n, int64_t samples, const double* E,
                         int kind, double power);
int multi_get_layer_dense(n2v2r_handle* h, int k, float* A);
int multi_column_sums(n2v2r_handle* h, int k, float* out);
int multi_uase(n2v2r_handle* h, int d, const n2v2r_eig_opts* opts, n2v2r_eig_stats* stats);
int multi_get_embedding(n2v2r_handle* h, float* Y);
int multi_get_left_embedding(n2v2r_handle* h, float* X);
int multi_rank(n2v2r_handle* h, int strategy, const int* dims, int n_dims, const int* metrics,
               int n_metrics, int method, int* n_comparisons, int* n_cols);
}
using n2v2r_int::guarded;
```

### node2vec2rank_amd/csrc/ingest.hip

```cpp
#include "common.h"

__global__ __launch_bounds__(256) void csr_scan_kernel(const int64_t* __restrict__ ip,
                                                       const int32_t* __restrict__ ix,
                                                       const float* __restrict__ dv, int64_t n_rows,
                                                       int64_t n_cols, uint64_t* __restrict__ keys,
                                                       int32_t* __restrict__ idx,
                                                       unsigned* __restrict__ flags) {
  const int lane = threadIdx.x & 63;
  const int64_t nw = (int64_t)gridDim.x * (blockDim.x >> 6);
  unsigned f = 0;
  for (int64_t r = (int64_t)blockIdx.x * (blockDim.x >> 6) + (threadIdx.x >> 6); r < n_rows;
       r += nw) {
    const int64_t p0 = ip[r], p1 = ip[r + 1];
    for (int64_t p = p0 + lane; p < p1; p += 64) {
      const int32_t c = ix[p];
      const bool bad = c < 0 || (int64_t)c >= n_cols;
      f |= bad ? 1u : 0u;
      f |= (dv[p] != 1.0f) ? 2u : 0u;
      if (p > p0 && ix[p - 1] > c) f |= 4u;
      if (keys) {
        keys[p] = ((uint64_t)(uint32_t)(bad ? 0 : c) << 32) | (uint64_t)(uint32_t)r;
        idx[p] = (int32_t)p;
      }
    }
  }
#pragma unroll
  for (int m = 32; m >= 1; m >>= 1) f |= (unsigned)__shfl_xor((int)f, m, 64);
  if (lane == 0 && f) atomicOr(flags, f);
}

__global__ __launch_bounds__(256) void csr_from_sorted_kernel(const uint64_t* __restrict__ keys,
                                                              const int32_t* __restrict__ idx,
                                                              const float* __restrict__ dv,
                                                              int64_t nnz, int64_t n_cols,
                                                              int64_t* __restrict__ tp,
                                                              int32_t* __restrict__ tx,
                                                              float* __restrict__ td) {
  const int64_t q = (int64_t)blockIdx.x * blockDim.x + threadIdx.x;
  if (q >= nnz) return;
  const uint64_t k = keys[q];
  const int64_t c = (int64_t)(k >> 32);
  tx[q] = (int32_t)(uint32_t)(k & 0xFFFFFFFFull);
  if (td) td[q] = dv[idx[q]];
  const int64_t prev = q > 0 ? (int64_t)(keys[q - 1] >> 32) : -1;
  for (int64_t x = prev + 1; x <= c; ++x) tp[x] = q;
  if (q == nnz - 1)
    for (int64_t x = c + 1; x <= n_cols; ++x) tp[x] = nnz;
}

__global__ __launch_bounds__(256) void csr_compare_kernel(const int64_t* __restrict__ ap,
                                                          const int32_t* __restrict__ ax,
                                                          const float* __restrict__ av,
                                                          const int64_t* __restrict__ bp,
                                                          const int32_t* __restrict__ bx,
                                                          const float* __restrict__ bv,
                                                          int64_t n_rows, int64_t nnz,
                                                          unsigned* __restrict__ flag) {
  const int64_t t = (int64_t)blockIdx.x * blockDim.x + threadIdx.x;
  const int64_t nt = (int64_t)gridDim.x * blockDim.x;
  bool diff = false;
  for (int64_t i = t; i <= n_rows; i += nt) diff |= ap[i] != bp[i];
  for (int64_t p = t; p < nnz; p += nt) diff |= (ax[p] != bx[p]) || !(av[p] == bv[p]);
  const unsigned long long m = __ballot(diff);
  if ((threadIdx.x & 63) == 0 && m) atomicOr(flag, 1u);
}

__global__ void csr_rebase_kernel(const int64_t* __restrict__ ip, int64_t r0, int64_t nr,
                                  int64_t* __restrict__ out) {
  const int64_t r = (int64_t)blockIdx.x * blockDim.x + threadIdx.x;
  if (r <= nr) out[r] = ip[r0 + r] - ip[r0];
}

static unsigned grid_for(int64_t work, int per_block, unsigned cap) {
  int64_t g = (work + per_block - 1) / per_block;
  if (g < 1) g = 1;
  if (g > cap) g = cap;
  return (unsigned)g;
}

extern "C" hipError_t n2v2r_launch_csr_scan(const int64_t* ip, const int32_t* ix, const float* dv,
                                            int64_t n_rows, int64_t n_cols, uint64_t* keys,
                                            int32_t* idx, unsigned* flags, hipStream_t stream) {
  if (n_rows <= 0) return hipSuccess;
  hipLaunchKernelGGL(csr_scan_kernel, dim3(grid_for(n_rows, 4, 65536)), dim3(256), 0, stream, ip,
                     ix, dv, n_rows, n_cols, keys, idx, flags);
  return hipGetLastError();
}

extern "C" hipError_t n2v2r_launch_csr_from_sorted(const uint64_t* keys, const int32_t* idx,
                                                   const float* dv, int64_t nnz, int64_t n_cols,
                                                   int64_t* tp, int32_t* tx, float* td,
                                                   hipStream_t stream) {
  if (nnz <= 0) return hipMemsetAsync(tp, 0, sizeof(int64_t) * (n_cols + 1), stream);
  hipLaunchKernelGGL(csr_from_sorted_kernel, dim3((unsigned)((nnz + 255) / 256)), dim3(256), 0,
                     stream, keys, idx, dv, nnz, n_cols, tp, tx, td);
  return hipGetLastError();
}

extern "C" hipError_t n2v2r_launch_csr_compare(const int64_t* ap, const int32_t* ax,
                                               const float* av, const int64_t* bp,
                                               const int32_t* bx, const float* bv, int64_t n_rows,
                                               int64_t nnz, unsigned* flag, hipStream_t stream) {
  const int64_t work = nnz > n_rows ? nnz : n_rows + 1;
  hipLaunchKernelGGL(csr_compare_kernel, dim3(grid_for(work, 256 * 8, 8192)), dim3(256), 0,
                     stream, ap, ax, av, bp, bx, bv, n_rows, nnz, flag);
  return hipGetLastError();
}

extern "C" hipError_t n2v2r_launch_csr_rebase(const int64_t* ip, int64_t r0, int64_t nr,
                                              int64_t* out, hipStream_t stream) {
  hipLaunchKernelGGL(csr_rebase_kernel, dim3((unsigned)((nr + 1 + 255) / 256)), dim3(256), 0,
                     stream, ip, r0, nr, out);
  return hipGetLastError();
}

__global__ void chunk_major_keys_kernel(uint64_t* __restrict__ keys, int64_t nnz, int64_t npad,
                                        int W, int64_t rc) {
  for (int64_t e = (int64_t)blockIdx.x * blockDim.x + threadIdx.x; e < nnz;
       e += (int64_t)gridDim.x * blockDim.x) {
    const uint64_t k = keys[e];
    const int64_t j = (int64_t)(k >> 32);
    const int64_t g = j / npad, i = j - g * npad;
    const int64_t c = i / rc;
    const int64_t rows_c = rc < npad - c * rc ? rc : npad - c * rc;
    const int64_t pos = c * W * rc + g * rows_c + (i - c * rc);
    keys[e] = ((uint64_t)pos << 32) | (k & 0xFFFFFFFFull);
  }
}

extern "C" hipError_t n2v2r_launch_chunk_major_keys(uint64_t* keys, int64_t nnz, int64_t npad,
                                                   int W, int64_t rc, hipStream_t stream) {
  if (nnz <= 0) return hipSuccess;
  if (W < 1 || rc < 1 || npad < 1) return hipErrorInvalidValue;
  hipLaunchKernelGGL(chunk_major_keys_kernel, dim3(grid_for(nnz, 256, 8192)), dim3(256), 0, stream,
                     keys, nnz, npad, W, rc);
  return hipGetLastError();
}
```

### node2vec2rank_amd/csrc/layers.cpp

```cpp
#include "engine.h"

using namespace n2v2r_int;

namespace n2v2r_int {
void build_col_blocks(const CsrDev& A, int64_t ncols, LayerDev::ColBlocks& out, hipStream_t st,
                      int nb, int wbits) {
  const int64_t n = A.n_rows;
  const int64_t cw = (ncols + nb - 1) / nb;
  int cbits = 1;
  while (((int64_t)1 << cbits) < cw) ++cbits;
  out.ncols = ncols;
  out.nb = nb;
  out.wbits = wbits;
  out.cbits = cbits + wbits <= 31 ? cbits : 0;
  out.built = true;
  out.usable = false;
  if (n <= 0 || out.cbits == 0) return;
  DevBuf cnt, rp64, tsum;
  cnt.ensure(sizeof(int32_t) * nb * n, st);
  HIPCHK(n2v2r_launch_cb_count(A, cw, nb, cnt.as<int32_t>(), st));
  const int64_t ntiles = n2v2r_cb_scan_tiles(n, nb);
  tsum.ensure(sizeof(int64_t) * ntiles, st);
  rp64.ensure(sizeof(int64_t) * nb * (n + 1), st);
  const int64_t nw1 = ((n + ((int64_t)1 << wbits) - 1) >> wbits) + 1;
  out.wo.ensure(sizeof(int32_t) * nb * nw1, st);
  HIPCHK(n2v2r_launch_cb_rowptrs(cnt.as<int32_t>(), n, nb, A.nnz, tsum.as<int64_t>(),
                                 (size_t)ntiles, rp64.as<int64_t>(), out.wo.as<int32_t>(), wbits,
                                 st));
  std::vector<int64_t> ends(2 * (size_t)nb);
  for (int j = 0; j < nb; ++j) {
    HIPCHK(hipMemcpyAsync(&ends[2 * j], rp64.as<int64_t>() + (size_t)j * (n + 1),
                          sizeof(int64_t), hipMemcpyDeviceToHost, st));
    HIPCHK(hipMemcpyAsync(&ends[2 * j + 1], rp64.as<int64_t>() + (size_t)j * (n + 1) + n,
                          sizeof(int64_t), hipMemcpyDeviceToHost, st));
  }
  HIPCHK(hipStreamSynchronize(st));
  if (ends[2 * (nb - 1) + 1] != A.nnz || ends[0] != 0)
    throw StatusFail{N2V2R_ERR_INTERNAL, "column-block split lost entries"};
  for (int j = 0; j < nb; ++j)
    if (ends[2 * j + 1] - ends[2 * j] > (int64_t)INT32_MAX) return;
  out.idx.ensure(sizeof(int32_t) * std::max<int64_t>(A.nnz, 1), st);
  if (!A.unit) out.dat.ensure(sizeof(float) * std::max<int64_t>(A.nnz, 1), st);
  HIPCHK(n2v2r_launch_cb_fill(A, cw, nb, rp64.as<int64_t>(), out.idx.as<int32_t>(),
                              A.unit ? nullptr : out.dat.as<float>(), out.cbits, wbits, st));
  HIPCHK(hipStreamSynchronize(st));
  for (int j = 0; j < nb; ++j)
    out.blk[j] = CsrBlk{out.wo.as<int32_t>() + (size_t)j * nw1, out.idx.as<int32_t>(),
                        A.unit ? nullptr : out.dat.as<float>(), ends[2 * j], n,
                        ends[2 * j + 1] - ends[2 * j], A.unit, out.cbits, (int64_t)j * cw};
  out.usable = true;
}

bool ensure_col_blocks(LayerDev& L, int64_t ncols, hipStream_t st, int nb, int wbits) {
  auto stale = [&](const LayerDev::ColBlocks& c) {
    return !c.built || c.ncols != ncols || c.nb != nb || c.wbits != wbits;
  };
  if (stale(L.cb)) build_col_blocks(L.csr(), ncols, L.cb, st, nb, wbits);
  if (!L.symmetric && stale(L.cb_t)) build_col_blocks(L.csr_t(), ncols, L.cb_t, st, nb, wbits);
  return L.cb.usable && L.cb.cbits && (L.symmetric || (L.cb_t.usable && L.cb_t.cbits));
}

int tile_wbits(const std::vector<std::unique_ptr<LayerDev>>& layers, int nb) {
  (void)layers;
  (void)nb;
  if (const char* e = std::getenv("N2V2R_SPMM_WBITS")) {
    const int v = std::atoi(e);
    if (v >= CB_WIN_BITS_MIN && v <= CB_WIN_BITS_MAX) return v;
  }
  return 6;
}

void ensure_colcsr(LayerDev& L, int64_t ncols, int64_t rows_out, hipStream_t st, int64_t npad,
                   int W, int64_t rc) {
  if (rc <= 0 || rc >= npad) rc = 0;
  if (L.c_built && L.c_rows == rows_out && L.c_rc == rc) return;
  const CsrDev s = L.csr_t();
  const int64_t nnz = s.nnz;
  if (nnz > (int64_t)INT32_MAX)
    throw StatusFail{N2V2R_ERR_BAD_ARG, "a rank's layer block over 2^31 - 1 entries"};
  L.c_indptr.ensure(sizeof(int64_t) * (rows_out + 1));
  L.c_indices.ensure(sizeof(int32_t) * std::max<int64_t>(nnz, 1));
  if (!s.unit) L.c_data.ensure(sizeof(float) * std::max<int64_t>(nnz, 1));
  if (nnz == 0) {
    HIPCHK(n2v2r_launch_csr_from_sorted(nullptr, nullptr, nullptr, 0, rows_out,
                                        L.c_indptr.as<int64_t>(), nullptr, nullptr, st));
  } else {
    DevBuf keys[2], pay[2], hist, flag;
    for (int i = 0; i < 2; ++i) {
      keys[i].ensure(sizeof(uint64_t) * nnz);
      pay[i].ensure(sizeof(int32_t) * nnz);
    }
    flag.ensure(sizeof(unsigned) * 4, st);
    HIPCHK(hipMemsetAsync(flag.p, 0, sizeof(unsigned) * 4, st));
    HIPCHK(n2v2r_launch_csr_scan(s.indptr, s.indices, s.data, s.n_rows, ncols,
                                 keys[0].as<uint64_t>(), pay[0].as<int32_t>(),
                                 flag.as<unsigned>(), st));
    if (rc > 0)
      HIPCHK(n2v2r_launch_chunk_major_keys(keys[0].as<uint64_t>(), nnz, npad, W, rc, st));
    hist.ensure(sizeof(uint32_t) * n2v2r_radix_hist_elems(nnz, 1));
    int bits = 1;
    const int64_t span = rc > 0 ? rows_out : ncols;
    while (bits < 31 && ((int64_t)1 << bits) < span) ++bits;
    int cur = 0;
    for (int sh = 32; sh < 32 + bits; sh += 8) {
      HIPCHK(n2v2r_launch_radix_pass(keys[cur].as<uint64_t>(), pay[cur].as<int32_t>(),
                                     keys[cur ^ 1].as<uint64_t>(), pay[cur ^ 1].as<int32_t>(),
                                     nnz, 1, sh, hist.as<uint32_t>(), st));
      cur ^= 1;
    }
    HIPCHK(n2v2r_launch_csr_from_sorted(keys[cur].as<uint64_t>(), pay[cur].as<int32_t>(), s.data,
                                        nnz, rows_out, L.c_indptr.as<int64_t>(),
                                        L.c_indices.as<int32_t>(),
                                        s.unit ? nullptr : L.c_data.as<float>(), st));
    HIPCHK(hipStreamSynchronize(st));
  }
  L.c_nnz = nnz;
  L.c_rows = rows_out;
  L.c_rc = rc;
  L.c_built = true;
}

int host_threads() {
  return (int)std::min<unsigned>(16u, std::max(1u, std::thread::hardware_concurrency()));
}

bool host_all_ones(int64_t nnz, const float* dv) {
  auto ok = [&](int64_t p0, int64_t p1) {
    bool good = true;
    for (int64_t p = p0; p < p1; ++p) good &= dv[p] == 1.0f;
    return good;
  };
  int nt = host_threads();
  if (nnz < (int64_t)1 << 22) nt = 1;
  if (nt == 1) return ok(0, nnz);
  std::vector<char> res(nt, 1);
  const int64_t per = (nnz + nt - 1) / nt;
  parallel_chunks(nt, [&](int t) {
    const int64_t p0 = std::min<int64_t>(nnz, t * per);
    res[t] = ok(p0, std::min<int64_t>(nnz, p0 + per)) ? 1 : 0;
  });
  for (char c : res)
    if (!c) return false;
  return true;
}

bool host_indices_in_range(int64_t nnz, const int32_t* ix, int64_t n) {
  auto ok = [&](int64_t p0, int64_t p1) {
    bool good = true;
    for (int64_t p = p0; p < p1; ++p) good &= (ix[p] >= 0) & ((int64_t)ix[p] < n);
    return good;
  };
  int nt = host_threads();
  if (nnz < (int64_t)1 << 22) nt = 1;
  if (nt == 1) return ok(0, nnz);
  std::vector<char> res(nt, 1);
  const int64_t per = (nnz + nt - 1) / nt;
  parallel_chunks(nt, [&](int t) {
    const int64_t p0 = std::min<int64_t>(nnz, t * per);
    res[t] = ok(p0, std::min<int64_t>(nnz, p0 + per)) ? 1 : 0;
  });
  for (char c : res)
    if (!c) return false;
  return true;
}

bool upload_rows(hipStream_t st, int64_t r0, int64_t nr, const int64_t* ip, const int32_t* ix,
                 const float* dv, DevBuf& dip, DevBuf& dix, DevBuf& ddv, int64_t& nnz_out) {
  const int64_t p0 = ip[r0], p1 = ip[r0 + nr];
  nnz_out = p1 - p0;
  const bool unit = host_all_ones(nnz_out, dv + p0);
  std::vector<int64_t> lip(nr + 1);
  for (int64_t r = 0; r <= nr; ++r) lip[r] = ip[r0 + r] - p0;
  dip.ensure(sizeof(int64_t) * (nr + 1));
  dix.ensure(sizeof(int32_t) * std::max<int64_t>(nnz_out, 1));
  ddv.ensure(sizeof(float) * std::max<int64_t>(nnz_out, 1));
  HIPCHK(hipMemcpyAsync(dip.p, lip.data(), sizeof(int64_t) * (nr + 1), hipMemcpyHostToDevice, st));
  if (nnz_out) {
    HIPCHK(hipMemcpyAsync(dix.p, ix + p0, sizeof(int32_t) * nnz_out, hipMemcpyHostToDevice, st));
    if (unit)
      HIPCHK(hipMemsetD32Async((hipDeviceptr_t)ddv.p, 0x3F800000, (size_t)nnz_out, st));
    else
      HIPCHK(hipMemcpyAsync(ddv.p, dv + p0, sizeof(float) * nnz_out, hipMemcpyHostToDevice, st));
  }
  HIPCHK(hipStreamSynchronize(st));
  return unit;
}

namespace {
inline uint64_t mix64(uint64_t z) {
  z = (z ^ (z >> 30)) * 0xBF58476D1CE4E5B9ull;
  z = (z ^ (z >> 27)) * 0x94D049BB133111EBull;
  return z ^ (z >> 31);
}
}

bool host_csr_symmetric(int64_t n, const int64_t* ip, const int32_t* ix, const float* dv) {
  int nt = host_threads();
  const int64_t nnz = ip[n];
  if (nnz < (int64_t)1 << 20) nt = 1;
  std::vector<uint64_t> acc((size_t)nt * 4, 0);
  const int64_t per = (n + nt - 1) / nt;
  parallel_chunks(nt, [&](int t) {
    const int64_t r0 = std::min<int64_t>(n, t * per), r1 = std::min<int64_t>(n, r0 + per);
    uint64_t a1 = 0, a2 = 0, b1 = 0, b2 = 0;
    for (int64_t r = r0; r < r1; ++r)
      for (int64_t p = ip[r]; p < ip[r + 1]; ++p) {
        uint32_t vb;
        std::memcpy(&vb, dv + p, sizeof(vb));
        const uint64_t c = (uint32_t)ix[p], rr = (uint64_t)r;
        const uint64_t kf = (rr << 32) | c, kt = (c << 32) | rr;
        a1 += mix64(mix64(kf + 0x9E3779B97F4A7C15ull) ^ vb);
        b1 += mix64(mix64(kt + 0x9E3779B97F4A7C15ull) ^ vb);
        a2 += mix64(mix64(kf ^ 0xD1B54A32D192ED03ull) + ((uint64_t)vb << 17));
        b2 += mix64(mix64(kt ^ 0xD1B54A32D192ED03ull) + ((uint64_t)vb << 17));
      }
    acc[(size_t)t * 4 + 0] = a1;
    acc[(size_t)t * 4 + 1] = a2;
    acc[(size_t)t * 4 + 2] = b1;
    acc[(size_t)t * 4 + 3] = b2;
  });
  uint64_t s[4] = {0, 0, 0, 0};
  for (int t = 0; t < nt; ++t)
    for (int i = 0; i < 4; ++i) s[i] += acc[(size_t)t * 4 + i];
  return s[0] == s[2] && s[1] == s[3];
}

void host_transpose_rows(int64_t n, const int64_t* ip, const int32_t* ix, const float* dv,
                         int64_t r0, int64_t nr, std::vector<int64_t>& tip,
                         std::vector<int32_t>& tix, std::vector<float>& tdv) {
  tip.assign((size_t)nr + 1, 0);
  const uint64_t span = (uint64_t)nr;
  for (int64_t r = 0; r < n; ++r)
    for (int64_t p = ip[r]; p < ip[r + 1]; ++p) {
      const uint64_t c = (uint64_t)((int64_t)ix[p] - r0);
      if (c < span) ++tip[c + 1];
    }
  for (int64_t i = 0; i < nr; ++i) tip[i + 1] += tip[i];
  tix.resize((size_t)std::max<int64_t>(tip[nr], 1));
  tdv.resize((size_t)std::max<int64_t>(tip[nr], 1));
  std::vector<int64_t> pos(tip.begin(), tip.end() - 1);
  for (int64_t r = 0; r < n; ++r)
    for (int64_t p = ip[r]; p < ip[r + 1]; ++p) {
      const uint64_t c = (uint64_t)((int64_t)ix[p] - r0);
      if (c < span) {
        const int64_t q = pos[c]++;
        tix[q] = (int32_t)r;
        tdv[q] = dv[p];
      }
    }
}

int set_layer_rows_directed(n2v2r_handle* h, int k, const int64_t* aip, const int32_t* aix,
                            const float* adv, const int64_t* tip, const int32_t* tix,
                            const float* tdv) {
  return guarded(h, [&]() -> int {
    const int64_t nr = h->nloc;
    if (k < 0 || k >= h->K || aip[0] != 0 || tip[0] != 0) return N2V2R_ERR_BAD_ARG;
    for (int64_t r = 0; r < nr; ++r)
      if (aip[r + 1] < aip[r]) {
        h->set_err("layer %d: indptr not monotone", k);
        return N2V2R_ERR_BAD_ARG;
      }
    if (!host_indices_in_range(aip[nr], aix, h->n)) {
      h->set_err("layer %d: column index out of range", k);
      return N2V2R_ERR_BAD_ARG;
    }
    for (int j = 0; j < h->K; ++j)
      if (j != k && h->layers[j]->loaded && h->layers[j]->dense) {
        h->err = "layers must be all CSR or all dense";
        return N2V2R_ERR_BAD_ARG;
      }
    LayerDev& L = *h->layers[k];
    L.dense = false;
    L.loaded = false;
    L.drop_col_blocks();
    L.n_rows = nr;
    L.unit = upload_rows(h->stream, 0, nr, aip, aix, adv, L.indptr, L.indices, L.data, L.nnz);
    L.t_unit = upload_rows(h->stream, 0, nr, tip, tix, tdv, L.t_indptr, L.t_indices, L.t_data,
                           L.t_nnz);
    h->h2d_layer_bytes += 16 * (nr + 1) + (L.unit ? 4 : 8) * L.nnz + (L.t_unit ? 4 : 8) * L.t_nnz;
    L.symmetric = false;
    L.loaded = true;
    h->have_embedding = false;
    return N2V2R_OK;
  });
}
}

extern "C" {

int n2v2r_set_num_layers(n2v2r_handle* h, int num_layers, int64_t n) {
  if (h && h->multi()) return multi_set_num_layers(h, num_layers, n);
  return guarded(h, [&]() -> int {
    if (num_layers < 1 || n < 1 || n > (int64_t)INT32_MAX) {
      h->set_err("bad layer count %d or node count %lld", num_layers, (long long)n);
      return N2V2R_ERR_BAD_ARG;
    }
    if (num_layers > SPMM_MAX_LAYERS) {
      h->set_err("at most %d layers are supported", SPMM_MAX_LAYERS);
      return N2V2R_ERR_BAD_ARG;
    }
    h->K = num_layers;
    h->set_partition(n);
    h->layers.clear();
    for (int k = 0; k < num_layers; ++k) h->layers.emplace_back(new LayerDev());
    h->have_embedding = false;
    h->ncmp = h->ncols = 0;
    return N2V2R_OK;
  });
}

int n2v2r_set_layer_csr(n2v2r_handle* h, int k, int64_t n, int64_t nnz, const int64_t* indptr,
                        const int32_t* indices, const float* data, int symmetric) {
  if (h && h->multi()) return multi_set_layer_csr(h, k, n, nnz, indptr, indices, data, symmetric);
  return guarded(h, [&]() -> int {
    if (k < 0 || k >= h->K || n != h->n || nnz < 0 || !indptr || (nnz > 0 && (!indices || !data))) {
      h->set_err("bad CSR arguments for layer %d", k);
      return N2V2R_ERR_BAD_ARG;
    }
    if (indptr[0] != 0 || indptr[n] != nnz) {
      h->set_err("layer %d: indptr must start at 0 and end at nnz", k);
      return N2V2R_ERR_BAD_ARG;
    }
    if (symmetric != N2V2R_SYM_YES && nnz > (int64_t)INT32_MAX) {
      h->set_err("layer %d: more than 2^31 - 1 entries need symmetric = N2V2R_SYM_YES (the GPU "
                 "transpose / symmetry test sorts int32 entry indices)", k);
      return N2V2R_ERR_BAD_ARG;
    }
    for (int64_t r = 0; r < n; ++r)
      if (indptr[r + 1] < indptr[r]) {
        h->set_err("layer %d: indptr not monotone", k);
        return N2V2R_ERR_BAD_ARG;
      }
    for (int j = 0; j < h->K; ++j)
      if (j != k && h->layers[j]->loaded && h->layers[j]->dense) {
        h->err = "layers must be all CSR or all dense";
        return N2V2R_ERR_BAD_ARG;
      }
    LayerDev& L = *h->layers[k];
    L.dense = false;
    L.loaded = false;
    L.drop_col_blocks();
    L.n_rows = h->nloc;
    const hipStream_t st = h->stream;
    const bool whole = !h->comm;
    DevBuf gip, gix, gdv;
    DevBuf& dip = whole ? L.indptr : gip;
    DevBuf& dix = whole ? L.indices : gix;
    DevBuf& ddv = whole ? L.data : gdv;
    dip.ensure(sizeof(int64_t) * (n + 1));
    dix.ensure(sizeof(int32_t) * std::max<int64_t>(nnz, 1));
    ddv.ensure(sizeof(float) * std::max<int64_t>(nnz, 1));
    HIPCHK(hipMemcpyAsync(dip.p, indptr, sizeof(int64_t) * (n + 1), hipMemcpyHostToDevice, st));
    const bool ones = nnz > 0 && host_all_ones(nnz, data);
    if (nnz) {
      HIPCHK(hipMemcpyAsync(dix.p, indices, sizeof(int32_t) * nnz, hipMemcpyHostToDevice, st));
      if (ones)
        HIPCHK(hipMemsetD32Async((hipDeviceptr_t)ddv.p, 0x3F800000, (size_t)nnz, st));
      else
        HIPCHK(hipMemcpyAsync(ddv.p, data, sizeof(float) * nnz, hipMemcpyHostToDevice, st));
    }
    h->h2d_layer_bytes += 8 * (n + 1) + (ones ? 4 : 8) * nnz;
    const bool need_t = symmetric != N2V2R_SYM_YES;
    DevBuf* keys = h->ing_keys;
    DevBuf* pay = h->ing_pay;
    DevBuf& hist = h->ing_hist;
    DevBuf& flag = h->ing_flag;
    flag.ensure_raw(sizeof(unsigned) * 4);
    HIPCHK(hipMemsetAsync(flag.p, 0, sizeof(unsigned) * 4, st));
    if (need_t && nnz) {
      keys[0].ensure_raw(sizeof(uint64_t) * nnz);
      pay[0].ensure_raw(sizeof(int32_t) * nnz);
    }
    HIPCHK(n2v2r_launch_csr_scan(dip.as<int64_t>(), dix.as<int32_t>(), ddv.as<float>(), n, n,
                                 need_t && nnz ? keys[0].as<uint64_t>() : nullptr,
                                 need_t && nnz ? pay[0].as<int32_t>() : nullptr,
                                 flag.as<unsigned>(), st));
    unsigned fl = 0;
    HIPCHK(hipMemcpyAsync(&fl, flag.p, sizeof(unsigned), hipMemcpyDeviceToHost, st));
    HIPCHK(hipStreamSynchronize(st));
    if (fl & 1u) {
      h->set_err("layer %d: column index out of range", k);
      return N2V2R_ERR_BAD_ARG;
    }
    const bool unit = !(fl & 2u);
    const bool sorted = !(fl & 4u);
    auto transpose = [&](const int64_t* ip_, const int32_t* ix_, const float* dv_, bool have_keys,
                         DevBuf& tp, DevBuf& tx, DevBuf& td) {
      tp.ensure(sizeof(int64_t) * (n + 1));
      tx.ensure(sizeof(int32_t) * std::max<int64_t>(nnz, 1));
      if (!unit) td.ensure(sizeof(float) * std::max<int64_t>(nnz, 1));
      if (nnz == 0) {
        HIPCHK(n2v2r_launch_csr_from_sorted(nullptr, nullptr, nullptr, 0, n, tp.as<int64_t>(),
                                            nullptr, nullptr, st));
        return;
      }
      keys[0].ensure_raw(sizeof(uint64_t) * nnz);
      pay[0].ensure_raw(sizeof(int32_t) * nnz);
      keys[1].ensure_raw(sizeof(uint64_t) * nnz);
      pay[1].ensure_raw(sizeof(int32_t) * nnz);
      if (!have_keys)
        HIPCHK(n2v2r_launch_csr_scan(ip_, ix_, dv_, n, n, keys[0].as<uint64_t>(),
                                     pay[0].as<int32_t>(), flag.as<unsigned>() + 1, st));
      hist.ensure_raw(sizeof(uint32_t) * n2v2r_radix_hist_elems(nnz, 1));
      int bits = 1;
      while (bits < 31 && ((int64_t)1 << bits) < n) ++bits;
      int cur = 0;
      for (int sh = 32; sh < 32 + bits; sh += 8) {
        HIPCHK(n2v2r_launch_radix_pass(keys[cur].as<uint64_t>(), pay[cur].as<int32_t>(),
                                       keys[cur ^ 1].as<uint64_t>(), pay[cur ^ 1].as<int32_t>(),
                                       nnz, 1, sh, hist.as<uint32_t>(), st));
        cur ^= 1;
      }
      HIPCHK(n2v2r_launch_csr_from_sorted(keys[cur].as<uint64_t>(), pay[cur].as<int32_t>(), dv_,
                                          nnz, n, tp.as<int64_t>(), tx.as<int32_t>(),
                                          unit ? nullptr : td.as<float>(), st));
    };
    bool sym = symmetric == N2V2R_SYM_YES;
    DevBuf gtp, gtx, gtd;
    DevBuf& tp = whole ? L.t_indptr : gtp;
    DevBuf& tx = whole ? L.t_indices : gtx;
    DevBuf& td = whole ? L.t_data : gtd;
    if (need_t) {
      transpose(dip.as<int64_t>(), dix.as<int32_t>(), ddv.as<float>(), true, tp, tx, td);
      if (symmetric == N2V2R_SYM_DETECT) {
        const float* tv = unit ? ddv.as<float>() : td.as<float>();
        HIPCHK(hipMemsetAsync(flag.as<unsigned>() + 2, 0, sizeof(unsigned), st));
        if (sorted) {
          HIPCHK(n2v2r_launch_csr_compare(dip.as<int64_t>(), dix.as<int32_t>(), ddv.as<float>(),
                                          tp.as<int64_t>(), tx.as<int32_t>(), tv, n, nnz,
                                          flag.as<unsigned>() + 2, st));
        } else {
          DevBuf sp_, sx, sv;
          transpose(tp.as<int64_t>(), tx.as<int32_t>(), tv, false, sp_, sx, sv);
          HIPCHK(n2v2r_launch_csr_compare(sp_.as<int64_t>(), sx.as<int32_t>(),
                                          unit ? ddv.as<float>() : sv.as<float>(),
                                          tp.as<int64_t>(), tx.as<int32_t>(), tv, n, nnz,
                                          flag.as<unsigned>() + 2, st));
          HIPCHK(hipStreamSynchronize(st));
        }
        unsigned mism = 0;
        HIPCHK(hipMemcpyAsync(&mism, flag.as<unsigned>() + 2, sizeof(unsigned),
                              hipMemcpyDeviceToHost, st));
        HIPCHK(hipStreamSynchronize(st));
        sym = mism == 0;
      }
    }
    HIPCHK(hipStreamSynchronize(st));
    keys[0].release();
    keys[1].release();
    pay[0].release();
    pay[1].release();
    auto slice = [&](DevBuf& sip, DevBuf& six, DevBuf& sdv, bool copy_values, DevBuf& oip,
                     DevBuf& oix, DevBuf& odv, int64_t& onnz) {
      int64_t p0 = 0, p1 = 0;
      HIPCHK(hipMemcpyAsync(&p0, sip.as<int64_t>() + h->row0, sizeof(int64_t),
                            hipMemcpyDeviceToHost, st));
      HIPCHK(hipMemcpyAsync(&p1, sip.as<int64_t>() + h->row0 + h->nloc, sizeof(int64_t),
                            hipMemcpyDeviceToHost, st));
      HIPCHK(hipStreamSynchronize(st));
      onnz = p1 - p0;
      oip.ensure(sizeof(int64_t) * (h->nloc + 1));
      oix.ensure(sizeof(int32_t) * std::max<int64_t>(onnz, 1));
      odv.ensure(sizeof(float) * std::max<int64_t>(onnz, 1));
      HIPCHK(n2v2r_launch_csr_rebase(sip.as<int64_t>(), h->row0, h->nloc, oip.as<int64_t>(), st));
      if (onnz) {
        HIPCHK(hipMemcpyAsync(oix.p, six.as<int32_t>() + p0, sizeof(int32_t) * onnz,
                              hipMemcpyDeviceToDevice, st));
        if (copy_values)
          HIPCHK(hipMemcpyAsync(odv.p, sdv.as<float>() + p0, sizeof(float) * onnz,
                                hipMemcpyDeviceToDevice, st));
      }
      HIPCHK(hipStreamSynchronize(st));
    };
    if (whole) {
      L.nnz = nnz;
      L.t_nnz = nnz;
      if (sym) {
        L.t_indptr.release();
        L.t_indices.release();
        L.t_data.release();
      }
    } else {
      slice(gip, gix, gdv, true, L.indptr, L.indices, L.data, L.nnz);
      if (!sym) slice(gtp, gtx, gtd, !unit, L.t_indptr, L.t_indices, L.t_data, L.t_nnz);
    }
    L.unit = unit;
    L.t_unit = unit;
    L.symmetric = sym;
    L.loaded = true;
    h->have_embedding = false;
    return N2V2R_OK;
  });
}

int n2v2r_set_layer_dense(n2v2r_handle* h, int k, int64_t n, const float* A, int symmetric) {
  if (h && h->multi()) return multi_set_layer_dense(h, k, n, A, symmetric);
  return guarded(h, [&]() -> int {
    if (k < 0 || k >= h->K || n != h->n || !A) {
      h->set_err("bad dense arguments for layer %d", k);
      return N2V2R_ERR_BAD_ARG;
    }
    for (int j = 0; j < h->K; ++j)
      if (j != k && h->layers[j]->loaded && !h->layers[j]->dense) {
        h->err = "layers must be all CSR or all dense";
        return N2V2R_ERR_BAD_ARG;
      }
    LayerDev& L = *h->layers[k];
    L.dense = true;
    L.n_rows = h->nloc;
    L.lda = (n + 63) / 64 * 64;
    const int64_t nl = std::max<int64_t>(h->nloc, 1);
    L.dA.ensure(sizeof(float) * nl * L.lda);
    HIPCHK(hipMemcpy2D(L.dA.p, sizeof(float) * L.lda, A + h->row0 * n, sizeof(float) * n,
                       sizeof(float) * n, h->nloc, hipMemcpyHostToDevice));
    bool sym = symmetric == N2V2R_SYM_YES;
    if (!sym) {
      DevBuf full;
      const float* src = L.dA.as<float>();
      if (h->comm) {
        full.ensure(sizeof(float) * n * L.lda);
        HIPCHK(hipMemcpy2D(full.p, sizeof(float) * L.lda, A, sizeof(float) * n,
                           sizeof(float) * n, n, hipMemcpyHostToDevice));
        src = full.as<float>();
      }
      L.dAT.ensure(sizeof(float) * nl * L.lda);
      HIPCHK(n2v2r_launch_transpose(src + h->row0, L.lda, n, h->nloc, L.dAT.as<float>(), L.lda,
                                    h->stream));
      if (symmetric == N2V2R_SYM_DETECT) {
        DevBuf cnt;
        cnt.ensure(sizeof(unsigned long long));
        HIPCHK(n2v2r_launch_mismatch(L.dA.as<float>(), L.dAT.as<float>(), L.lda, h->nloc, n,
                                     cnt.as<unsigned long long>(), h->stream));
        unsigned long long mism = 0;
        HIPCHK(hipMemcpyAsync(&mism, cnt.p, sizeof(mism), hipMemcpyDeviceToHost, h->stream));
        HIPCHK(hipStreamSynchronize(h->stream));
        sym = mism == 0;
      }
      HIPCHK(hipStreamSynchronize(h->stream));
      if (sym) L.dAT.release();
    }
    L.symmetric = sym;
    L.loaded = true;
    h->have_embedding = false;
    return N2V2R_OK;
  });
}

int n2v2r_set_layer_corr(n2v2r_handle* h, int k, int64_t n, int64_t samples, const double* E,
                         int kind, double power) {
  if (h && h->multi()) return multi_set_layer_corr(h, k, n, samples, E, kind, power);
  return guarded(h, [&]() -> int {
    if (k < 0 || k >= h->K || n != h->n || n < 1 || !E) {
      h->set_err("bad co-expression arguments for layer %d", k);
      return N2V2R_ERR_BAD_ARG;
    }
    LayerDev& L = *h->layers[k];
    L.loaded = false;
    h->have_embedding = false;
    if (samples < 2) {
      h->set_err("layer %d: a correlation needs at least 2 samples, got %lld", k,
                 (long long)samples);
      return N2V2R_ERR_BAD_ARG;
    }
    if (kind != N2V2R_CORR_UNSIGNED && kind != N2V2R_CORR_SIGNED &&
        kind != N2V2R_CORR_SIGNED_HYBRID && kind != N2V2R_CORR_RAW) {
      h->set_err("layer %d: unknown correlation kind %d", k, kind);
      return N2V2R_ERR_BAD_ARG;
    }
    if (!std::isfinite(power) || power < 1.0) {
      h->set_err("layer %d: power must be finite and >= 1, got %g", k, power);
      return N2V2R_ERR_BAD_ARG;
    }
    if (kind == N2V2R_CORR_RAW && power != 1.0) {
      h->set_err("layer %d: a raw correlation layer takes power 1 (r may be negative), got %g", k,
                 power);
      return N2V2R_ERR_BAD_ARG;
    }
    for (int j = 0; j < h->K; ++j)
      if (j != k && h->layers[j]->loaded && !h->layers[j]->dense) {
        h->err = "layers must be all CSR or all dense";
        return N2V2R_ERR_BAD_ARG;
      }
    hipStream_t st = h->stream;
    const int64_t npad = (n + 63) / 64 * 64, sp = n2v2r_corr_spad(samples);
    DevBuf e, z;
    e.ensure_raw(sizeof(double) * n * samples);
    z.ensure_raw(sizeof(double) * npad * sp);
    DevBuf& flag = h->ing_flag;
    flag.ensure_raw(sizeof(unsigned) * 4);
    HIPCHK(hipMemcpyAsync(e.p, E, sizeof(double) * n * samples, hipMemcpyHostToDevice, st));
    h->h2d_layer_bytes += 8 * n * samples;
    HIPCHK(hipMemsetAsync(flag.p, 0xFF, sizeof(unsigned), st));
    HIPCHK(n2v2r_launch_corr_standardise(e.as<double>(), n, samples, z.as<double>(),
                                         flag.as<unsigned>(), st));
    unsigned bad = 0;
    HIPCHK(hipMemcpyAsync(&bad, flag.p, sizeof(unsigned), hipMemcpyDeviceToHost, st));
    HIPCHK(hipStreamSynchronize(st));
    if (bad != 0xFFFFFFFFu) {
      h->set_err("layer %d: row %u of the expression matrix holds a non-finite value or is "
                 "constant (zero variance): its correlations are undefined", k, bad);
      return N2V2R_ERR_BAD_ARG;
    }
    L.dense = true;
    L.n_rows = h->nloc;
    L.lda = npad;
    L.dA.ensure(sizeof(float) * std::max<int64_t>(h->nloc, 1) * L.lda);
    L.dAT.release();
    HIPCHK(n2v2r_launch_corr_tiles(z.as<double>(), samples, n, h->row0, h->nloc, L.dA.as<float>(),
                                   L.lda, kind, power, st));
    HIPCHK(hipStreamSynchronize(st));
    L.symmetric = true;
    L.loaded = true;
    return N2V2R_OK;
  });
}

int n2v2r_get_layer_dense(n2v2r_handle* h, int k, float* A) {
  if (h && h->multi()) return multi_get_layer_dense(h, k, A);
  return guarded(h, [&]() -> int {
    if (k < 0 || k >= h->K || !A || !h->layers[k]->loaded || !h->layers[k]->dense) {
      h->set_err("get_layer_dense: layer %d is not a loaded dense layer", k);
      return N2V2R_ERR_BAD_ARG;
    }
    const LayerDev& L = *h->layers[k];
    HIPCHK(hipStreamSynchronize(h->stream));
    if (h->nloc > 0)
      HIPCHK(hipMemcpy2D(A + h->row0 * h->n, sizeof(float) * h->n, L.dA.p, sizeof(float) * L.lda,
                         sizeof(float) * h->n, h->nloc, hipMemcpyDeviceToHost));
    return N2V2R_OK;
  });
}

int n2v2r_set_layer_csr_rows(n2v2r_handle* h, int k, int64_t n, int64_t row0, int64_t n_rows,
                             int64_t nnz, const int64_t* indptr, const int32_t* indices,
                             const float* data) {
  return guarded(h, [&]() -> int {
    if (h->multi()) {
      h->err = "n2v2r_set_layer_csr_rows: a multi-GPU handle takes whole layers (it slices them)";
      return N2V2R_ERR_BAD_ARG;
    }
    if (k < 0 || k >= h->K || n != h->n || row0 != h->row0 || n_rows != h->nloc || nnz < 0 ||
        !indptr || (nnz > 0 && (!indices || !data)) || indptr[0] != 0 || indptr[n_rows] != nnz) {
      h->set_err("bad local CSR rows for layer %d (expected rows [%lld, %lld))", k,
                 (long long)h->row0, (long long)(h->row0 + h->nloc));
      return N2V2R_ERR_BAD_ARG;
    }
    for (int64_t r = 0; r < n_rows; ++r)
      if (indptr[r + 1] < indptr[r]) {
        h->set_err("layer %d: indptr not monotone", k);
        return N2V2R_ERR_BAD_ARG;
      }
    if (!host_indices_in_range(nnz, indices, n)) {
      h->set_err("layer %d: column index out of range", k);
      return N2V2R_ERR_BAD_ARG;
    }
    for (int j = 0; j < h->K; ++j)
      if (j != k && h->layers[j]->loaded && h->layers[j]->dense) {
        h->err = "layers must be all CSR or all dense";
        return N2V2R_ERR_BAD_ARG;
      }
    LayerDev& L = *h->layers[k];
    L.dense = false;
    L.drop_col_blocks();
    L.n_rows = h->nloc;
    L.unit = upload_rows(h->stream, 0, n_rows, indptr, indices, data, L.indptr, L.indices, L.data,
                         L.nnz);
    h->h2d_layer_bytes += 8 * (n_rows + 1) + (L.unit ? 4 : 8) * L.nnz;
    L.symmetric = true;
    L.loaded = true;
    h->have_embedding = false;
    return N2V2R_OK;
  });
}

int n2v2r_column_sums(n2v2r_handle* h, int k, float* out) {
  if (h && h->multi()) return multi_column_sums(h, k, out);
  return guarded(h, [&]() -> int {
    if (k < 0 || k >= h->K || !out || !h->layers[k]->loaded) return N2V2R_ERR_BAD_ARG;
    DevBuf o, g;
    o.ensure(sizeof(float) * h->npad);
    if (h->layers[k]->dense) {
      DevBuf ones;
      ones.ensure(sizeof(float) * h->n);
      std::vector<float> one(h->n, 1.f);
      HIPCHK(hipMemcpy(ones.p, one.data(), sizeof(float) * h->n, hipMemcpyHostToDevice));
      h->dense_apply(h->layers[k]->dense_at(), h->layers[k]->lda, ones.as<float>(), 1, 1,
                     o.as<float>(), 1, 0.f, nullptr);
    } else {
      HIPCHK(n2v2r_launch_row_sums(h->layers[k]->csr_t(), o.as<float>(), h->stream));
    }
    const float* src = o.as<float>();
    if (h->comm) {
      g.ensure(sizeof(float) * h->world * h->npad);
      h->comm->allgather(o.p, g.p, sizeof(float) * h->npad, h->stream);
      src = g.as<float>();
    }
    HIPCHK(hipMemcpyAsync(out, src, sizeof(float) * h->n, hipMemcpyDeviceToHost, h->stream));
    HIPCHK(hipStreamSynchronize(h->stream));
    return N2V2R_OK;
  });
}

int n2v2r_project(n2v2r_handle* h, int64_t m, int64_t n, const double* W, int on_columns,
                  double* out) {
  if (h && h->multi()) h = h->ranks[0];
  return guarded(h, [&]() -> int {
    if (m < 1 || n < 1 || !W || !out) return N2V2R_ERR_BAD_ARG;
    DevBuf w, o;
    w.ensure(sizeof(double) * m * n);
    HIPCHK(hipMemcpyAsync(w.p, W, sizeof(double) * m * n, hipMemcpyHostToDevice, h->stream));
    const int64_t r = on_columns ? n : m, kd = on_columns ? m : n;
    const int64_t sk = on_columns ? n : 1, si = on_columns ? 1 : n;
    o.ensure(sizeof(double) * r * r);
    HIPCHK(n2v2r_launch_syrk_f64(w.as<double>(), sk, si, kd, r, o.as<double>(), r, h->stream));
    HIPCHK(hipMemcpyAsync(out, o.p, sizeof(double) * r * r, hipMemcpyDeviceToHost, h->stream));
    HIPCHK(hipStreamSynchronize(h->stream));
    return N2V2R_OK;
  });
}

}
```

### node2vec2rank_amd/csrc/ranking.cpp

```cpp
#include "engine.h"

using namespace n2v2r_int;

extern "C" {

struct GivenOrder {
  int col;
  const int32_t* order_dev;
};
static void run_borda(n2v2r_handle* h, const double* Ddev, int64_t n, int nseg, int ncols,
                      int64_t* borda_dev, int32_t* tied_dev = nullptr,
                      const std::vector<GivenOrder>* given = nullptr) {
  hipStream_t st = h->stream;
  const size_t tot = (size_t)nseg * n;
  for (int i = 0; i < 2; ++i) {
    h->rs_keys[i].ensure(sizeof(uint64_t) * tot);
    h->rs_idx[i].ensure(sizeof(int32_t) * tot);
  }
  h->rs_pos.ensure(sizeof(int32_t) * tot);
  h->rs_hist.ensure(sizeof(uint32_t) * n2v2r_radix_hist_elems(n, nseg));
  h->rs_or.ensure(sizeof(unsigned long long) * nseg);
  h->rs_and.ensure(sizeof(unsigned long long) * nseg);
  HIPCHK(n2v2r_launch_borda_init(Ddev, n, nseg, h->rs_keys[0].as<uint64_t>(),
                                 h->rs_idx[0].as<int32_t>(), h->rs_or.as<unsigned long long>(),
                                 h->rs_and.as<unsigned long long>(), st));
  std::vector<unsigned long long> kor(nseg), kand(nseg);
  HIPCHK(hipMemcpyAsync(kor.data(), h->rs_or.p, sizeof(unsigned long long) * nseg,
                        hipMemcpyDeviceToHost, st));
  HIPCHK(hipMemcpyAsync(kand.data(), h->rs_and.p, sizeof(unsigned long long) * nseg,
                        hipMemcpyDeviceToHost, st));
  HIPCHK(hipStreamSynchronize(st));
  unsigned long long varying = 0;
  for (int s = 0; s < nseg; ++s) varying |= kor[s] ^ kand[s];
  int cur = 0;
  for (int pass = 0; pass < 8; ++pass) {
    const int shift = pass * 8;
    if (((varying >> shift) & 0xFFull) == 0) continue;
    HIPCHK(n2v2r_launch_radix_pass(h->rs_keys[cur].as<uint64_t>(), h->rs_idx[cur].as<int32_t>(),
                                   h->rs_keys[cur ^ 1].as<uint64_t>(),
                                   h->rs_idx[cur ^ 1].as<int32_t>(), n, nseg, shift,
                                   h->rs_hist.as<uint32_t>(), st));
    cur ^= 1;
  }
  if (tied_dev) HIPCHK(n2v2r_launch_tie_flags(h->rs_keys[cur].as<uint64_t>(), n, nseg, tied_dev, st));
  if (given)
    for (const GivenOrder& g : *given)
      HIPCHK(hipMemcpyAsync(h->rs_idx[cur].as<int32_t>() + (size_t)g.col * n, g.order_dev,
                            sizeof(int32_t) * n, hipMemcpyDeviceToDevice, st));
  HIPCHK(n2v2r_launch_borda_finish(h->rs_idx[cur].as<int32_t>(), n, nseg, ncols,
                                   h->rs_pos.as<int32_t>(), borda_dev, st));
}

int n2v2r_rank(n2v2r_handle* h, int strategy, const int* dims, int n_dims, const int* metrics,
               int n_metrics, int method, int* n_comparisons, int* n_cols) {
  if (h && h->multi())
    return multi_rank(h, strategy, dims, n_dims, metrics, n_metrics, method, n_comparisons, n_cols);
  return guarded(h, [&]() -> int {
    if (method != N2V2R_AGG_BORDA && method != N2V2R_AGG_NONE) {
      h->err = "Aggregation method not found. Available methods: Borda";
      return N2V2R_ERR_UNSUPPORTED_AGG;
    }
    if (!h->have_embedding) {
      h->err = "No n2v2r embeddings found";
      return N2V2R_ERR_NOT_READY;
    }
    if (strategy < 0 || strategy > 2 || n_dims < 1 || n_metrics < 1 || !dims || !metrics) {
      h->err = "bad rank arguments";
      return N2V2R_ERR_BAD_ARG;
    }
    for (int m = 0; m < n_metrics; ++m)
      if (metrics[m] < 0 || metrics[m] > 2) {
        h->err = "Unsupported metric";
        return N2V2R_ERR_UNSUPPORTED_METRIC;
      }
    std::vector<std::pair<int, int>> cols;
    for (int i = 0; i < n_dims; ++i) {
      if (dims[i] < 1 || dims[i] > h->d) {
        h->set_err("dimension %d outside [1, %d]", dims[i], h->d);
        return N2V2R_ERR_BAD_ARG;
      }
      for (int m = 0; m < n_metrics; ++m) {
        if (metrics[m] == N2V2R_COSINE && dims[i] == 1) continue;
        cols.emplace_back(dims[i], metrics[m]);
      }
    }
    if (cols.empty() || (int)cols.size() > DIST_MAX_COLS) {
      h->err = "no ranking columns (or too many)";
      return N2V2R_ERR_BAD_ARG;
    }
    DistPlan plan{};
    plan.n_cols = (int)cols.size();
    std::vector<int> order(cols.size());
    std::iota(order.begin(), order.end(), 0);
    std::stable_sort(order.begin(), order.end(),
                     [&](int a, int b) { return cols[a].first < cols[b].first; });
    plan.dmax = 0;
    for (int e = 0; e < plan.n_cols; ++e) {
      plan.col_dim[e] = cols[order[e]].first;
      plan.col_metric[e] = cols[order[e]].second;
      plan.col_out[e] = order[e];
      plan.dmax = std::max(plan.dmax, plan.col_dim[e]);
    }
    std::vector<int> layer_i;
    for (int i = 0; i < h->K; ++i) {
      if (i == 0 && strategy != N2V2R_ONE_VS_REST) continue;
      layer_i.push_back(i);
    }
    if (layer_i.empty()) {
      h->err = "need at least two layers to compare";
      return N2V2R_ERR_BAD_ARG;
    }
    const int ncmp = (int)layer_i.size();
    const int C = plan.n_cols;
    const int64_t n = h->n;
    h->D.ensure(sizeof(double) * (size_t)ncmp * C * n);
    h->borda.ensure(sizeof(int64_t) * (size_t)ncmp * n);
    const double t0 = now_ms();
    if (!h->comm) {
      for (int c = 0; c < ncmp; ++c)
        HIPCHK(n2v2r_launch_distances(h->Y.as<float>(), h->K, n, h->ldy, h->npad, strategy,
                                      layer_i[c], plan, h->D.as<double>() + (size_t)c * C * n, n,
                                      h->stream));
    } else {
      h->Dloc.ensure(sizeof(double) * (size_t)ncmp * C * h->npad);
      h->Dgat.ensure(sizeof(double) * (size_t)h->world * h->npad);
      for (int c = 0; c < ncmp; ++c)
        HIPCHK(n2v2r_launch_distances(h->Y.as<float>(), h->K, h->nloc, h->ldy, h->npad, strategy,
                                      layer_i[c], plan,
                                      h->Dloc.as<double>() + (size_t)c * C * h->npad, h->npad,
                                      h->stream));
      for (int s = 0; s < ncmp * C; ++s) {
        h->comm->allgather(h->Dloc.as<double>() + (size_t)s * h->npad, h->Dgat.p,
                           sizeof(double) * h->npad, h->stream);
        HIPCHK(hipMemcpyAsync(h->D.as<double>() + (size_t)s * n, h->Dgat.p, sizeof(double) * n,
                              hipMemcpyDeviceToDevice, h->stream));
      }
    }
    HIPCHK(hipStreamSynchronize(h->stream));
    const double t1 = now_ms();
    h->have_borda = method == N2V2R_AGG_BORDA;
    if (h->have_borda) run_borda(h, h->D.as<double>(), n, ncmp * C, C, h->borda.as<int64_t>());
    HIPCHK(hipStreamSynchronize(h->stream));
    h->ms_dist = t1 - t0;
    h->ms_borda = now_ms() - t1;
    h->ncmp = ncmp;
    h->ncols = C;
    if (n_comparisons) *n_comparisons = ncmp;
    if (n_cols) *n_cols = C;
    return N2V2R_OK;
  });
}

int n2v2r_get_distances(n2v2r_handle* h, int comparison, double* D) {
  if (h && h->multi()) h = h->ranks[0];
  return guarded(h, [&]() -> int {
    if (comparison < 0 || comparison >= h->ncmp || !D) return N2V2R_ERR_BAD_ARG;
    HIPCHK(hipMemcpyAsync(D, h->D.as<double>() + (size_t)comparison * h->ncols * h->n,
                          sizeof(double) * h->ncols * h->n, hipMemcpyDeviceToHost, h->stream));
    HIPCHK(hipStreamSynchronize(h->stream));
    return N2V2R_OK;
  });
}

int n2v2r_get_borda(n2v2r_handle* h, int comparison, int64_t* borda) {
  if (h && h->multi()) h = h->ranks[0];
  return guarded(h, [&]() -> int {
    if (comparison < 0 || comparison >= h->ncmp || !borda) return N2V2R_ERR_BAD_ARG;
    if (!h->have_borda) {
      h->err = "n2v2r_rank ran without aggregation (N2V2R_AGG_NONE)";
      return N2V2R_ERR_NOT_READY;
    }
    HIPCHK(hipMemcpyAsync(borda, h->borda.as<int64_t>() + (size_t)comparison * h->n,
                          sizeof(int64_t) * h->n, hipMemcpyDeviceToHost, h->stream));
    HIPCHK(hipStreamSynchronize(h->stream));
    return N2V2R_OK;
  });
}

int n2v2r_rank_timing(n2v2r_handle* h, double* ms_distances, double* ms_borda) {
  if (!h) return N2V2R_ERR_BAD_ARG;
  if (h->multi()) h = h->ranks[0];
  if (ms_distances) *ms_distances = h->ms_dist;
  if (ms_borda) *ms_borda = h->ms_borda;
  return N2V2R_OK;
}

int n2v2r_pairwise_distances(n2v2r_handle* h, const double* m1, const double* m2, int64_t n,
                             int dim, int metric, double* out) {
  if (h && h->multi()) h = h->ranks[0];
  return guarded(h, [&]() -> int {
    if (metric < 0 || metric > 2) {
      h->err = "Unsupported metric";
      return N2V2R_ERR_UNSUPPORTED_METRIC;
    }
    if (n < 1 || dim < 1 || !m1 || !m2 || !out) return N2V2R_ERR_BAD_ARG;
    DevBuf a, b, o;
    a.ensure(sizeof(double) * n * dim);
    b.ensure(sizeof(double) * n * dim);
    o.ensure(sizeof(double) * n);
    HIPCHK(hipMemcpyAsync(a.p, m1, sizeof(double) * n * dim, hipMemcpyHostToDevice, h->stream));
    HIPCHK(hipMemcpyAsync(b.p, m2, sizeof(double) * n * dim, hipMemcpyHostToDevice, h->stream));
    HIPCHK(n2v2r_launch_pairwise(a.as<double>(), b.as<double>(), n, dim, metric, o.as<double>(),
                                 h->stream));
    HIPCHK(hipMemcpyAsync(out, o.p, sizeof(double) * n, hipMemcpyDeviceToHost, h->stream));
    HIPCHK(hipStreamSynchronize(h->stream));
    return N2V2R_OK;
  });
}

int n2v2r_borda_columns(n2v2r_handle* h, const double* D, int64_t n, int n_cols, int64_t* borda) {
  if (h && h->multi()) h = h->ranks[0];
  return guarded(h, [&]() -> int {
    if (n < 1 || n_cols < 1 || !D || !borda) return N2V2R_ERR_BAD_ARG;
    DevBuf dd, bo;
    dd.ensure(sizeof(double) * n * n_cols);
    bo.ensure(sizeof(int64_t) * n);
    HIPCHK(hipMemcpyAsync(dd.p, D, sizeof(double) * n * n_cols, hipMemcpyHostToDevice, h->stream));
    run_borda(h, dd.as<double>(), n, n_cols, n_cols, bo.as<int64_t>());
    HIPCHK(hipMemcpyAsync(borda, bo.p, sizeof(int64_t) * n, hipMemcpyDeviceToHost, h->stream));
    HIPCHK(hipStreamSynchronize(h->stream));
    return N2V2R_OK;
  });
}

int n2v2r_borda_columns_ex(n2v2r_handle* h, const double* D, int64_t n, int n_cols,
                           const int32_t* given_cols, int n_given, const int32_t* given_orders,
                           int64_t* borda, int32_t* tied) {
  if (h && h->multi()) h = h->ranks[0];
  return guarded(h, [&]() -> int {
    if (n < 1 || n_cols < 1 || !D || !borda || n_given < 0 || n_given > n_cols ||
        (n_given > 0 && (!given_cols || !given_orders)) || n > INT32_MAX)
      return N2V2R_ERR_BAD_ARG;
    std::vector<char> seen_col(n_cols, 0), seen((size_t)n);
    for (int g = 0; g < n_given; ++g) {
      const int c = given_cols[g];
      if (c < 0 || c >= n_cols || seen_col[c]) {
        h->set_err("given column %d out of range or repeated", c);
        return N2V2R_ERR_BAD_ARG;
      }
      seen_col[c] = 1;
      std::fill(seen.begin(), seen.end(), 0);
      const int32_t* o = given_orders + (size_t)g * n;
      for (int64_t i = 0; i < n; ++i) {
        if (o[i] < 0 || o[i] >= n || seen[o[i]]) {
          h->set_err("given order of column %d is not a permutation of 0..n-1", c);
          return N2V2R_ERR_BAD_ARG;
        }
        seen[o[i]] = 1;
      }
    }
    DevBuf dd, bo, tf, go;
    dd.ensure(sizeof(double) * n * n_cols);
    bo.ensure(sizeof(int64_t) * n);
    tf.ensure(sizeof(int32_t) * n_cols);
    HIPCHK(hipMemcpyAsync(dd.p, D, sizeof(double) * n * n_cols, hipMemcpyHostToDevice, h->stream));
    std::vector<GivenOrder> given;
    if (n_given > 0) {
      go.ensure(sizeof(int32_t) * (size_t)n_given * n);
      HIPCHK(hipMemcpyAsync(go.p, given_orders, sizeof(int32_t) * (size_t)n_given * n,
                            hipMemcpyHostToDevice, h->stream));
      for (int g = 0; g < n_given; ++g)
        given.push_back({given_cols[g], go.as<int32_t>() + (size_t)g * n});
    }
    run_borda(h, dd.as<double>(), n, n_cols, n_cols, bo.as<int64_t>(), tf.as<int32_t>(),
              n_given > 0 ? &given : nullptr);
    HIPCHK(hipMemcpyAsync(borda, bo.p, sizeof(int64_t) * n, hipMemcpyDeviceToHost, h->stream));
    if (tied)
      HIPCHK(hipMemcpyAsync(tied, tf.p, sizeof(int32_t) * n_cols, hipMemcpyDeviceToHost,
                            h->stream));
    HIPCHK(hipStreamSynchronize(h->stream));
    return N2V2R_OK;
  });
}

}
```

Before: 690,100 nodes/s.

## Batch multi-layer CSR ingest and stage large result downloads through pinned ring

Adds a batched set_layers_csr entry point that uploads all layers on a separate copy stream. Host-side validation (all-ones data, monotone indptr) runs on a thread pool while the copies are in flight, and later-layer ingest overlaps earlier layers' device classification. Large D/borda downloads now go through a pinned multi-slot ring with parallel memcpy into pageable destinations, and a GPU symmetry lookup kernel is added. This trades extra threads, pinned memory and complexity for less time in pageable transfers and layer setup, which may or may not fall inside the timed region.

```diff
diff --git a/include/n2v2r.h b/include/n2v2r.h
--- a/include/n2v2r.h
+++ b/include/n2v2r.h
@@ -89,6 +89,9 @@
 int n2v2r_set_num_layers(n2v2r_handle* h, int num_layers, int64_t n);
 int n2v2r_set_layer_csr(n2v2r_handle* h, int k, int64_t n, int64_t nnz, const int64_t* indptr,
                         const int32_t* indices, const float* data, int symmetric);
+int n2v2r_set_layers_csr(n2v2r_handle* h, int num_layers, int64_t n, const int64_t* nnz,
+                         const int64_t* const* indptr, const int32_t* const* indices,
+                         const float* const* data, int symmetric);
 int n2v2r_set_layer_dense(n2v2r_handle* h, int k, int64_t n, const float* A, int symmetric);
 enum { N2V2R_CORR_UNSIGNED = 0, N2V2R_CORR_SIGNED = 1, N2V2R_CORR_SIGNED_HYBRID = 2,
        N2V2R_CORR_RAW = 3 };
diff --git a/include/n2v2r_diag.h b/include/n2v2r_diag.h
--- a/include/n2v2r_diag.h
+++ b/include/n2v2r_diag.h
@@ -23,6 +23,8 @@
 
 int n2v2r_get_layer_dense(n2v2r_handle* h, int k, float* A );
 
+int n2v2r_layer_symmetric(n2v2r_handle* h, int k);
+
 #ifdef __cplusplus
 }
 #endif
diff --git a/node2vec2rank_amd/_lib.py b/node2vec2rank_amd/_lib.py
--- a/node2vec2rank_amd/_lib.py
+++ b/node2vec2rank_amd/_lib.py
@@ -44,7 +44,8 @@
     "n2v2r_simgroup_destroy", "n2v2r_create_sim", "n2v2r_dist_info", "n2v2r_set_layer_csr_rows",
     "n2v2r_rr_top", "n2v2r_rr_band_top", "n2v2r_set_layer_dense", "n2v2r_project",
     "n2v2r_create_multi", "n2v2r_multi_devices", "n2v2r_h2d_layer_bytes",
-    "n2v2r_set_layer_corr", "n2v2r_get_layer_dense",
+    "n2v2r_set_layer_corr", "n2v2r_get_layer_dense", "n2v2r_set_layers_csr",
+    "n2v2r_layer_symmetric",
 ]
 UNIQUE_ID_BYTES = 128
 
@@ -158,6 +159,8 @@
             "n2v2r_set_layer_corr": (_i, [_vp, _i, _i64, _i64, _p(np.float64), _i,
                                           ctypes.c_double]),
             "n2v2r_get_layer_dense": (_i, [_vp, _i, _p(np.float32)]),
+            "n2v2r_set_layers_csr": (_i, [_vp, _i, _i64, _p(np.int64), _vp, _vp, _vp, _i]),
+            "n2v2r_layer_symmetric": (_i, [_vp, _i]),
         }
         for name, (res, args) in sig.items():
             f = getattr(lib, name)
@@ -309,7 +312,7 @@
             raise RuntimeError(f"RCCL failure: {msg}")
         raise RuntimeError(msg)
 
-    def set_layers(self, layers, symmetric=SYM_DETECT, storage="auto"):
+    def set_layers(self, layers, symmetric=SYM_DETECT, storage="auto", per_layer=False):
         import scipy.sparse as sp
         corr = [isinstance(a, Coexpression) for a in layers]
         if any(corr):
@@ -365,12 +368,20 @@
             if m.shape != (n, n):
                 raise ValueError("all layers must be square and share the node set")
         self._check(self.lib.n2v2r_set_num_layers(self.h, len(mats), n), "set_num_layers")
-        for k, m in enumerate(mats):
-            indptr = np.ascontiguousarray(m.indptr, dtype=np.int64)
-            indices = np.ascontiguousarray(m.indices, dtype=np.int32)
-            data = np.ascontiguousarray(m.data, dtype=np.float32)
-            self._check(self.lib.n2v2r_set_layer_csr(self.h, k, n, int(m.nnz), indptr, indices,
-                                                     data, int(symmetric)), f"layer {k}")
+        arrs = [(np.ascontiguousarray(m.indptr, dtype=np.int64),
+                 np.ascontiguousarray(m.indices, dtype=np.int32),
+                 np.ascontiguousarray(m.data, dtype=np.float32)) for m in mats]
+        if per_layer:
+            for k, (indptr, indices, data) in enumerate(arrs):
+                self._check(self.lib.n2v2r_set_layer_csr(self.h, k, n, int(indices.size), indptr,
+                                                         indices, data, int(symmetric)),
+                            f"layer {k}")
+        else:
+            nnz = np.ascontiguousarray([a[1].size for a in arrs], dtype=np.int64)
+            ptrs = [(ctypes.c_void_p * len(arrs))(*[a[j].ctypes.data for a in arrs])
+                    for j in range(3)]
+            self._check(self.lib.n2v2r_set_layers_csr(self.h, len(arrs), n, nnz, ptrs[0], ptrs[1],
+                                                      ptrs[2], int(symmetric)), "set_layers")
         self.n = n
         self.num_layers = len(mats)
         self.storage = "csr"
@@ -497,6 +508,12 @@
                 self.h, Dc, n, c, gc.ctypes.data_as(_vp), int(cols.size),
                 orders.ctypes.data_as(_vp), out, tied), "borda_columns")
         return (out, tied.astype(bool)) if return_tied else out
+
+    def layer_symmetric(self, k: int) -> bool:
+        r = self.lib.n2v2r_layer_symmetric(self.h, int(k))
+        if r < 0:
+            raise ValueError(f"layer {k} is not loaded")
+        return r == 1
 
     def column_sums(self, k: int):
         out = np.empty(self.n, dtype=np.float32)
diff --git a/node2vec2rank_amd/build.py b/node2vec2rank_amd/build.py
--- a/node2vec2rank_amd/build.py
+++ b/node2vec2rank_amd/build.py
@@ -15,7 +15,7 @@
                "rr_sturm.hip", "ingest.hip", "engine.cpp", "layers.cpp", "comm.cpp", "solver.cpp",
                "ranking.cpp", "multi.cpp"]
 HOST_SOURCES: list = []
-HEADERS = ["common.h", "spmm_args.h", "engine.h", os.path.join("..", "..", "include", "n2v2r.h"),
+HEADERS = ["common.h", "spmm_args.h", "engine.h", "stage_ring.h", os.path.join("..", "..", "include", "n2v2r.h"),
            os.path.join("..", "..", "include", "n2v2r_diag.h")]
 ARCH = os.environ.get("N2V2R_OFFLOAD_ARCH", "gfx950")
 _EXTRA = os.environ.get("N2V2R_EXTRA_HIP_FLAGS", "").split() if _TAG else []
diff --git a/node2vec2rank_amd/csrc/engine.cpp b/node2vec2rank_amd/csrc/engine.cpp
--- a/node2vec2rank_amd/csrc/engine.cpp
+++ b/node2vec2rank_amd/csrc/engine.cpp
@@ -55,6 +55,14 @@
   for (hipEvent_t& e : h->cev)
     if (e) (void)hipEventDestroy(e);
   if (h->cstream) (void)hipStreamDestroy(h->cstream);
+  if (h->copy) (void)hipStreamSynchronize(h->copy);
+  for (hipEvent_t& e : h->copy_ev)
+    if (e) (void)hipEventDestroy(e);
+  for (hipEvent_t& e : h->ring_ev)
+    if (e) (void)hipEventDestroy(e);
+  if (h->copy) (void)hipStreamDestroy(h->copy);
+  if (h->ing_pin) (void)hipHostFree(h->ing_pin);
+  if (h->ring.base) (void)hipHostFree(h->ring.base);
   if (h->stream) (void)hipStreamDestroy(h->stream);
   delete h;
 }
diff --git a/node2vec2rank_amd/csrc/engine.h b/node2vec2rank_amd/csrc/engine.h
--- a/node2vec2rank_amd/csrc/engine.h
+++ b/node2vec2rank_amd/csrc/engine.h
@@ -23,6 +23,7 @@
 #include "../../include/n2v2r.h"
 #include "../../include/n2v2r_diag.h"
 #include "common.h"
+#include "stage_ring.h"
 
 #include "spmm_args.h"
 #define DIST_MAX_COLS 256
@@ -177,6 +178,8 @@
                                     const int64_t* bp, const int32_t* bx, const float* bv,
                                     int64_t n_rows, int64_t nnz, unsigned* flag,
                                     hipStream_t stream);
+hipError_t n2v2r_launch_csr_sym_lookup(const int64_t* ip, const int32_t* ix, const float* dv,
+                                       int64_t n_rows, unsigned* counts, hipStream_t stream);
 hipError_t n2v2r_launch_csr_rebase(const int64_t* ip, int64_t r0, int64_t nr, int64_t* out,
                                    hipStream_t stream);
 }
@@ -323,6 +326,19 @@
   CsrDev csr_c() const {
     return CsrDev{c_indptr.as<int64_t>(), c_indices.as<int32_t>(), c_data.as<float>(), c_rows,
                   c_nnz, (symmetric ? unit : t_unit) ? 1 : 0};
+  }
+  void stale_col_blocks() {
+    for (ColBlocks* c : {&cb, &cb_t}) c->built = c->usable = false;
+    c_indptr.release();
+    c_indices.release();
+    c_data.release();
+    c_built = false;
+  }
+  void drop_col_blocks_t() {
+    cb_t.wo.release();
+    cb_t.idx.release();
+    cb_t.dat.release();
+    cb_t.built = false;
   }
   void drop_col_blocks() {
     for (ColBlocks* c : {&cb, &cb_t}) {
@@ -513,6 +529,79 @@
   DevBuf ing_keys[2], ing_pay[2], ing_hist, ing_flag;
   DevBuf ypanel;
 
+  static constexpr int RING_SLOTS = 4;
+  hipStream_t copy = nullptr;
+  hipEvent_t copy_ev[2] = {};
+  hipEvent_t ring_ev[RING_SLOTS] = {};
+  unsigned* ing_pin = nullptr;
+  std::unique_ptr<n2v2r_stage::Pool> stage;
+  n2v2r_stage::Ring ring;
+  size_t ring_min = 0;
+  bool ring_tried = false;
+  void ensure_copy_stream() {
+    if (copy) return;
+    HIPCHK(hipStreamCreateWithFlags(&copy, hipStreamNonBlocking));
+    for (hipEvent_t& e : copy_ev) HIPCHK(hipEventCreateWithFlags(&e, hipEventDisableTiming));
+    HIPCHK(hipHostMalloc((void**)&ing_pin, sizeof(unsigned) * 4 * SPMM_MAX_LAYERS,
+                         hipHostMallocDefault));
+  }
+  n2v2r_stage::Pool& stage_pool() {
+    if (!stage) {
+      int nt = (int)std::min<unsigned>(n2v2r_stage::MAX_WORKERS,
+                                       std::max(1u, std::thread::hardware_concurrency()));
+      if (const char* e = std::getenv("N2V2R_STAGE_THREADS")) {
+        const int v = std::atoi(e);
+        if (v >= 1 && v <= n2v2r_stage::MAX_WORKERS) nt = v;
+      }
+      stage.reset(new n2v2r_stage::Pool(nt));
+    }
+    return *stage;
+  }
+  size_t ring_chunk = 0;
+  bool ring_wanted(size_t bytes) {
+    if (!ring_tried) {
+      ring_tried = true;
+      ring_chunk = (size_t)4 << 20;
+      ring_min = (size_t)32 << 20;
+      if (const char* e = std::getenv("N2V2R_STAGE_CHUNK")) {
+        ring_chunk = (size_t)std::strtoull(e, nullptr, 10) / 64 * 64;
+        ring_min = 0;
+      }
+    }
+    if (!ring_chunk || bytes < ring_min || bytes == 0) return false;
+    if (!ring.base) {
+      ensure_copy_stream();
+      void* p = nullptr;
+      if (hipHostMalloc(&p, ring_chunk * RING_SLOTS, hipHostMallocDefault) != hipSuccess) {
+        (void)hipGetLastError();
+        throw std::bad_alloc();
+      }
+      ring.base = static_cast<unsigned char*>(p);
+      ring.chunk = ring_chunk;
+      ring.slots = RING_SLOTS;
+      for (hipEvent_t& e : ring_ev) HIPCHK(hipEventCreateWithFlags(&e, hipEventDisableTiming));
+    }
+    return true;
+  }
+  void ring_d2h(void* dst, const void* src_dev, size_t bytes) {
+    HIPCHK(hipEventRecord(copy_ev[0], stream));
+    HIPCHK(hipStreamWaitEvent(copy, copy_ev[0], 0));
+    hipError_t bad = hipSuccess;
+    n2v2r_stage::download(
+        stage_pool(), ring, dst, bytes,
+        [&](int s, void* slot, size_t off, size_t nb) {
+          hipError_t e = hipMemcpyAsync(slot, static_cast<const unsigned char*>(src_dev) + off, nb,
+                                        hipMemcpyDeviceToHost, copy);
+          if (e == hipSuccess) e = hipEventRecord(ring_ev[s], copy);
+          if (e != hipSuccess && bad == hipSuccess) bad = e;
+        },
+        [&](int s) {
+          const hipError_t e = hipEventSynchronize(ring_ev[s]);
+          if (e != hipSuccess && bad == hipSuccess) bad = e;
+        });
+    if (bad != hipSuccess) throw HipFail{bad, "staged device -> host copy"};
+  }
+
 
   void set_err(const char* fmt, ...) {
     char buf[1024];
diff --git a/node2vec2rank_amd/csrc/ingest.hip b/node2vec2rank_amd/csrc/ingest.hip
--- a/node2vec2rank_amd/csrc/ingest.hip
+++ b/node2vec2rank_amd/csrc/ingest.hip
@@ -17,7 +17,11 @@
       const bool bad = c < 0 || (int64_t)c >= n_cols;
       f |= bad ? 1u : 0u;
       f |= (dv[p] != 1.0f) ? 2u : 0u;
-      if (p > p0 && ix[p - 1] > c) f |= 4u;
+      if (p > p0) {
+        const int32_t cp = ix[p - 1];
+        f |= cp > c ? 4u : 0u;
+        f |= cp == c ? 8u : 0u;
+      }
       if (keys) {
         keys[p] = ((uint64_t)(uint32_t)(bad ? 0 : c) << 32) | (uint64_t)(uint32_t)r;
         idx[p] = (int32_t)p;
@@ -65,6 +69,45 @@
   if ((threadIdx.x & 63) == 0 && m) atomicOr(flag, 1u);
 }
 
+__global__ __launch_bounds__(256) void csr_sym_lookup_kernel(const int64_t* __restrict__ ip,
+                                                             const int32_t* __restrict__ ix,
+                                                             const float* __restrict__ dv,
+                                                             int64_t n_rows,
+                                                             unsigned* __restrict__ counts) {
+  const int lane = threadIdx.x & 63;
+  const int64_t nw = (int64_t)gridDim.x * (blockDim.x >> 6);
+  unsigned miss = 0;
+  int bal = 0;
+  for (int64_t r = (int64_t)blockIdx.x * (blockDim.x >> 6) + (threadIdx.x >> 6); r < n_rows;
+       r += nw) {
+    const int64_t p0 = ip[r], p1 = ip[r + 1];
+    for (int64_t p = p0 + lane; p < p1; p += 64) {
+      const int64_t c = ix[p];
+      if (c < r) {
+        --bal;
+      } else if (c == r) {
+        if (dv && !(dv[p] == dv[p])) ++miss;
+      } else {
+        ++bal;
+        int64_t lo = ip[c], hi = ip[c + 1];
+        while (lo < hi) {
+          const int64_t mid = lo + ((hi - lo) >> 1);
+          if ((int64_t)ix[mid] < r) lo = mid + 1; else hi = mid;
+        }
+        const bool found = lo < ip[c + 1] && (int64_t)ix[lo] == r;
+        if (!found || (dv && !(dv[p] == dv[lo]))) ++miss;
+      }
+    }
+  }
+#pragma unroll
+  for (int m = 32; m >= 1; m >>= 1) {
+    miss += (unsigned)__shfl_xor((int)miss, m, 64);
+    bal += __shfl_xor(bal, m, 64);
+  }
+  if (lane == 0 && miss) atomicAdd(counts, miss);
+  if (lane == 0 && bal) atomicAdd(counts + 1, (unsigned)bal);
+}
+
 __global__ void csr_rebase_kernel(const int64_t* __restrict__ ip, int64_t r0, int64_t nr,
                                   int64_t* __restrict__ out) {
   const int64_t r = (int64_t)blockIdx.x * blockDim.x + threadIdx.x;
@@ -107,6 +150,15 @@
   return hipGetLastError();
 }
 
+extern "C" hipError_t n2v2r_launch_csr_sym_lookup(const int64_t* ip, const int32_t* ix,
+                                                  const float* dv, int64_t n_rows,
+                                                  unsigned* counts, hipStream_t stream) {
+  if (n_rows <= 0) return hipSuccess;
+  hipLaunchKernelGGL(csr_sym_lookup_kernel, dim3(grid_for(n_rows, 4, 65536)), dim3(256), 0,
+                     stream, ip, ix, dv, n_rows, counts);
+  return hipGetLastError();
+}
+
 extern "C" hipError_t n2v2r_launch_csr_rebase(const int64_t* ip, int64_t r0, int64_t nr,
                                               int64_t* out, hipStream_t stream) {
   hipLaunchKernelGGL(csr_rebase_kernel, dim3((unsigned)((nr + 1 + 255) / 256)), dim3(256), 0,
diff --git a/node2vec2rank_amd/csrc/layers.cpp b/node2vec2rank_amd/csrc/layers.cpp
--- a/node2vec2rank_amd/csrc/layers.cpp
+++ b/node2vec2rank_amd/csrc/layers.cpp
@@ -28,12 +28,10 @@
                                  (size_t)ntiles, rp64.as<int64_t>(), out.wo.as<int32_t>(), wbits,
                                  st));
   std::vector<int64_t> ends(2 * (size_t)nb);
-  for (int j = 0; j < nb; ++j) {
-    HIPCHK(hipMemcpyAsync(&ends[2 * j], rp64.as<int64_t>() + (size_t)j * (n + 1),
-                          sizeof(int64_t), hipMemcpyDeviceToHost, st));
-    HIPCHK(hipMemcpyAsync(&ends[2 * j + 1], rp64.as<int64_t>() + (size_t)j * (n + 1) + n,
-                          sizeof(int64_t), hipMemcpyDeviceToHost, st));
-  }
+  for (int e = 0; e < 2; ++e)
+    HIPCHK(hipMemcpy2DAsync(&ends[e], 2 * sizeof(int64_t), rp64.as<int64_t>() + (e ? n : 0),
+                            sizeof(int64_t) * (n + 1), sizeof(int64_t), nb, hipMemcpyDeviceToHost,
+                            st));
   HIPCHK(hipStreamSynchronize(st));
   if (ends[2 * (nb - 1) + 1] != A.nnz || ends[0] != 0)
     throw StatusFail{N2V2R_ERR_INTERNAL, "column-block split lost entries"};
@@ -41,6 +39,7 @@
     if (ends[2 * j + 1] - ends[2 * j] > (int64_t)INT32_MAX) return;
   out.idx.ensure(sizeof(int32_t) * std::max<int64_t>(A.nnz, 1), st);
   if (!A.unit) out.dat.ensure(sizeof(float) * std::max<int64_t>(A.nnz, 1), st);
+  else out.dat.release();
   HIPCHK(n2v2r_launch_cb_fill(A, cw, nb, rp64.as<int64_t>(), out.idx.as<int32_t>(),
                               A.unit ? nullptr : out.dat.as<float>(), out.cbits, wbits, st));
   HIPCHK(hipStreamSynchronize(st));
@@ -287,170 +286,166 @@
 }
 }
 
-extern "C" {
-
-int n2v2r_set_num_layers(n2v2r_handle* h, int num_layers, int64_t n) {
-  if (h && h->multi()) return multi_set_num_layers(h, num_layers, n);
-  return guarded(h, [&]() -> int {
-    if (num_layers < 1 || n < 1 || n > (int64_t)INT32_MAX) {
-      h->set_err("bad layer count %d or node count %lld", num_layers, (long long)n);
-      return N2V2R_ERR_BAD_ARG;
-    }
-    if (num_layers > SPMM_MAX_LAYERS) {
-      h->set_err("at most %d layers are supported", SPMM_MAX_LAYERS);
-      return N2V2R_ERR_BAD_ARG;
-    }
-    h->K = num_layers;
-    h->set_partition(n);
-    h->layers.clear();
-    for (int k = 0; k < num_layers; ++k) h->layers.emplace_back(new LayerDev());
-    h->have_embedding = false;
-    h->ncmp = h->ncols = 0;
-    return N2V2R_OK;
-  });
-}
-
-int n2v2r_set_layer_csr(n2v2r_handle* h, int k, int64_t n, int64_t nnz, const int64_t* indptr,
-                        const int32_t* indices, const float* data, int symmetric) {
-  if (h && h->multi()) return multi_set_layer_csr(h, k, n, nnz, indptr, indices, data, symmetric);
-  return guarded(h, [&]() -> int {
-    if (k < 0 || k >= h->K || n != h->n || nnz < 0 || !indptr || (nnz > 0 && (!indices || !data))) {
-      h->set_err("bad CSR arguments for layer %d", k);
-      return N2V2R_ERR_BAD_ARG;
-    }
-    if (indptr[0] != 0 || indptr[n] != nnz) {
-      h->set_err("layer %d: indptr must start at 0 and end at nnz", k);
-      return N2V2R_ERR_BAD_ARG;
-    }
-    if (symmetric != N2V2R_SYM_YES && nnz > (int64_t)INT32_MAX) {
-      h->set_err("layer %d: more than 2^31 - 1 entries need symmetric = N2V2R_SYM_YES (the GPU "
-                 "transpose / symmetry test sorts int32 entry indices)", k);
-      return N2V2R_ERR_BAD_ARG;
-    }
-    for (int64_t r = 0; r < n; ++r)
-      if (indptr[r + 1] < indptr[r]) {
-        h->set_err("layer %d: indptr not monotone", k);
-        return N2V2R_ERR_BAD_ARG;
-      }
-    for (int j = 0; j < h->K; ++j)
-      if (j != k && h->layers[j]->loaded && h->layers[j]->dense) {
-        h->err = "layers must be all CSR or all dense";
-        return N2V2R_ERR_BAD_ARG;
-      }
-    LayerDev& L = *h->layers[k];
+namespace {
+int csr_args_check(n2v2r_handle* h, int k, int64_t n, int64_t nnz, const int64_t* indptr,
+                   const int32_t* indices, const float* data, int symmetric) {
+  if (k < 0 || k >= h->K || n != h->n || nnz < 0 || !indptr || (nnz > 0 && (!indices || !data))) {
+    h->set_err("bad CSR arguments for layer %d", k);
+    return N2V2R_ERR_BAD_ARG;
+  }
+  if (indptr[0] != 0 || indptr[n] != nnz) {
+    h->set_err("layer %d: indptr must start at 0 and end at nnz", k);
+    return N2V2R_ERR_BAD_ARG;
+  }
+  if (symmetric != N2V2R_SYM_YES && nnz > (int64_t)INT32_MAX) {
+    h->set_err("layer %d: more than 2^31 - 1 entries need symmetric = N2V2R_SYM_YES (the GPU "
+               "transpose / symmetry test sorts int32 entry indices)", k);
+    return N2V2R_ERR_BAD_ARG;
+  }
+  return N2V2R_OK;
+}
+
+bool sym_lookup_enabled() {
+  const char* e = std::getenv("N2V2R_SYM_LOOKUP");
+  return !(e && e[0] == '0');
+}
+
+struct CsrIngest {
+  n2v2r_handle* h;
+  LayerDev& L;
+  const int k;
+  const int64_t n, nnz;
+  const int symmetric;
+  const bool whole;
+  DevBuf gip, gix, gdv, gtp, gtx, gtd;
+  DevBuf *dip, *dix, *ddv, *tp, *tx, *td;
+  unsigned* dfl = nullptr;
+  unsigned* hfl = nullptr;
+  bool have_keys = false, unit = false, sorted = false, lookup = false;
+
+  CsrIngest(n2v2r_handle* h_, int k_, int64_t n_, int64_t nnz_, int symmetric_)
+      : h(h_), L(*h_->layers[k_]), k(k_), n(n_), nnz(nnz_), symmetric(symmetric_),
+        whole(!h_->comm) {
+    dip = whole ? &L.indptr : &gip;
+    dix = whole ? &L.indices : &gix;
+    ddv = whole ? &L.data : &gdv;
+    tp = whole ? &L.t_indptr : &gtp;
+    tx = whole ? &L.t_indices : &gtx;
+    td = whole ? &L.t_data : &gtd;
+    h->ing_flag.ensure_raw(sizeof(unsigned) * 4 * SPMM_MAX_LAYERS);
+    dfl = h->ing_flag.as<unsigned>() + 4 * k;
+    hfl = h->ing_pin + 4 * k;
+  }
+  void alloc() {
     L.dense = false;
     L.loaded = false;
-    L.drop_col_blocks();
+    L.stale_col_blocks();
     L.n_rows = h->nloc;
+    dip->ensure(sizeof(int64_t) * (n + 1));
+    dix->ensure(sizeof(int32_t) * std::max<int64_t>(nnz, 1));
+    ddv->ensure(sizeof(float) * std::max<int64_t>(nnz, 1));
+  }
+  void scan() {
     const hipStream_t st = h->stream;
-    const bool whole = !h->comm;
-    DevBuf gip, gix, gdv;
-    DevBuf& dip = whole ? L.indptr : gip;
-    DevBuf& dix = whole ? L.indices : gix;
-    DevBuf& ddv = whole ? L.data : gdv;
-    dip.ensure(sizeof(int64_t) * (n + 1));
-    dix.ensure(sizeof(int32_t) * std::max<int64_t>(nnz, 1));
-    ddv.ensure(sizeof(float) * std::max<int64_t>(nnz, 1));
-    HIPCHK(hipMemcpyAsync(dip.p, indptr, sizeof(int64_t) * (n + 1), hipMemcpyHostToDevice, st));
-    const bool ones = nnz > 0 && host_all_ones(nnz, data);
-    if (nnz) {
-      HIPCHK(hipMemcpyAsync(dix.p, indices, sizeof(int32_t) * nnz, hipMemcpyHostToDevice, st));
-      if (ones)
-        HIPCHK(hipMemsetD32Async((hipDeviceptr_t)ddv.p, 0x3F800000, (size_t)nnz, st));
-      else
-        HIPCHK(hipMemcpyAsync(ddv.p, data, sizeof(float) * nnz, hipMemcpyHostToDevice, st));
-    }
-    h->h2d_layer_bytes += 8 * (n + 1) + (ones ? 4 : 8) * nnz;
-    const bool need_t = symmetric != N2V2R_SYM_YES;
+    HIPCHK(hipMemsetAsync(dfl, 0, sizeof(unsigned) * 4, st));
+    have_keys = nnz && (symmetric == N2V2R_SYM_NO ||
+                        (symmetric == N2V2R_SYM_DETECT && !sym_lookup_enabled()));
+    if (have_keys) {
+      h->ing_keys[0].ensure_raw(sizeof(uint64_t) * nnz);
+      h->ing_pay[0].ensure_raw(sizeof(int32_t) * nnz);
+    }
+    HIPCHK(n2v2r_launch_csr_scan(dip->as<int64_t>(), dix->as<int32_t>(), ddv->as<float>(), n, n,
+                                 have_keys ? h->ing_keys[0].as<uint64_t>() : nullptr,
+                                 have_keys ? h->ing_pay[0].as<int32_t>() : nullptr, dfl, st));
+    HIPCHK(hipMemcpyAsync(hfl, dfl, sizeof(unsigned), hipMemcpyDeviceToHost, st));
+  }
+  void transpose(const int64_t* ip_, const int32_t* ix_, const float* dv_, bool keys_ready,
+                 DevBuf& tp_, DevBuf& tx_, DevBuf& td_) {
+    const hipStream_t st = h->stream;
     DevBuf* keys = h->ing_keys;
     DevBuf* pay = h->ing_pay;
-    DevBuf& hist = h->ing_hist;
-    DevBuf& flag = h->ing_flag;
-    flag.ensure_raw(sizeof(unsigned) * 4);
-    HIPCHK(hipMemsetAsync(flag.p, 0, sizeof(unsigned) * 4, st));
-    if (need_t && nnz) {
-      keys[0].ensure_raw(sizeof(uint64_t) * nnz);
-      pay[0].ensure_raw(sizeof(int32_t) * nnz);
-    }
-    HIPCHK(n2v2r_launch_csr_scan(dip.as<int64_t>(), dix.as<int32_t>(), ddv.as<float>(), n, n,
-                                 need_t && nnz ? keys[0].as<uint64_t>() : nullptr,
-                                 need_t && nnz ? pay[0].as<int32_t>() : nullptr,
-                                 flag.as<unsigned>(), st));
-    unsigned fl = 0;
-    HIPCHK(hipMemcpyAsync(&fl, flag.p, sizeof(unsigned), hipMemcpyDeviceToHost, st));
+    tp_.ensure(sizeof(int64_t) * (n + 1));
+    tx_.ensure(sizeof(int32_t) * std::max<int64_t>(nnz, 1));
+    if (!unit) td_.ensure(sizeof(float) * std::max<int64_t>(nnz, 1));
+    if (nnz == 0) {
+      HIPCHK(n2v2r_launch_csr_from_sorted(nullptr, nullptr, nullptr, 0, n, tp_.as<int64_t>(),
+                                          nullptr, nullptr, st));
+      return;
+    }
+    keys[0].ensure_raw(sizeof(uint64_t) * nnz);
+    pay[0].ensure_raw(sizeof(int32_t) * nnz);
+    keys[1].ensure_raw(sizeof(uint64_t) * nnz);
+    pay[1].ensure_raw(sizeof(int32_t) * nnz);
+    if (!keys_ready)
+      HIPCHK(n2v2r_launch_csr_scan(ip_, ix_, dv_, n, n, keys[0].as<uint64_t>(),
+                                   pay[0].as<int32_t>(), dfl + 1, st));
+    h->ing_hist.ensure_raw(sizeof(uint32_t) * n2v2r_radix_hist_elems(nnz, 1));
+    int bits = 1;
+    while (bits < 31 && ((int64_t)1 << bits) < n) ++bits;
+    int cur = 0;
+    for (int sh = 32; sh < 32 + bits; sh += 8) {
+      HIPCHK(n2v2r_launch_radix_pass(keys[cur].as<uint64_t>(), pay[cur].as<int32_t>(),
+                                     keys[cur ^ 1].as<uint64_t>(), pay[cur ^ 1].as<int32_t>(),
+                                     nnz, 1, sh, h->ing_hist.as<uint32_t>(), st));
+      cur ^= 1;
+    }
+    HIPCHK(n2v2r_launch_csr_from_sorted(keys[cur].as<uint64_t>(), pay[cur].as<int32_t>(), dv_,
+                                        nnz, n, tp_.as<int64_t>(), tx_.as<int32_t>(),
+                                        unit ? nullptr : td_.as<float>(), st));
+  }
+  void transpose_a() {
+    transpose(dip->as<int64_t>(), dix->as<int32_t>(), ddv->as<float>(), have_keys, *tp, *tx, *td);
+  }
+  int classify() {
+    const hipStream_t st = h->stream;
     HIPCHK(hipStreamSynchronize(st));
+    const unsigned fl = hfl[0];
     if (fl & 1u) {
       h->set_err("layer %d: column index out of range", k);
       return N2V2R_ERR_BAD_ARG;
     }
-    const bool unit = !(fl & 2u);
-    const bool sorted = !(fl & 4u);
-    auto transpose = [&](const int64_t* ip_, const int32_t* ix_, const float* dv_, bool have_keys,
-                         DevBuf& tp, DevBuf& tx, DevBuf& td) {
-      tp.ensure(sizeof(int64_t) * (n + 1));
-      tx.ensure(sizeof(int32_t) * std::max<int64_t>(nnz, 1));
-      if (!unit) td.ensure(sizeof(float) * std::max<int64_t>(nnz, 1));
-      if (nnz == 0) {
-        HIPCHK(n2v2r_launch_csr_from_sorted(nullptr, nullptr, nullptr, 0, n, tp.as<int64_t>(),
-                                            nullptr, nullptr, st));
-        return;
-      }
-      keys[0].ensure_raw(sizeof(uint64_t) * nnz);
-      pay[0].ensure_raw(sizeof(int32_t) * nnz);
-      keys[1].ensure_raw(sizeof(uint64_t) * nnz);
-      pay[1].ensure_raw(sizeof(int32_t) * nnz);
-      if (!have_keys)
-        HIPCHK(n2v2r_launch_csr_scan(ip_, ix_, dv_, n, n, keys[0].as<uint64_t>(),
-                                     pay[0].as<int32_t>(), flag.as<unsigned>() + 1, st));
-      hist.ensure_raw(sizeof(uint32_t) * n2v2r_radix_hist_elems(nnz, 1));
-      int bits = 1;
-      while (bits < 31 && ((int64_t)1 << bits) < n) ++bits;
-      int cur = 0;
-      for (int sh = 32; sh < 32 + bits; sh += 8) {
-        HIPCHK(n2v2r_launch_radix_pass(keys[cur].as<uint64_t>(), pay[cur].as<int32_t>(),
-                                       keys[cur ^ 1].as<uint64_t>(), pay[cur ^ 1].as<int32_t>(),
-                                       nnz, 1, sh, hist.as<uint32_t>(), st));
-        cur ^= 1;
-      }
-      HIPCHK(n2v2r_launch_csr_from_sorted(keys[cur].as<uint64_t>(), pay[cur].as<int32_t>(), dv_,
-                                          nnz, n, tp.as<int64_t>(), tx.as<int32_t>(),
-                                          unit ? nullptr : td.as<float>(), st));
-    };
-    bool sym = symmetric == N2V2R_SYM_YES;
-    DevBuf gtp, gtx, gtd;
-    DevBuf& tp = whole ? L.t_indptr : gtp;
-    DevBuf& tx = whole ? L.t_indices : gtx;
-    DevBuf& td = whole ? L.t_data : gtd;
-    if (need_t) {
-      transpose(dip.as<int64_t>(), dix.as<int32_t>(), ddv.as<float>(), true, tp, tx, td);
-      if (symmetric == N2V2R_SYM_DETECT) {
-        const float* tv = unit ? ddv.as<float>() : td.as<float>();
-        HIPCHK(hipMemsetAsync(flag.as<unsigned>() + 2, 0, sizeof(unsigned), st));
+    unit = !(fl & 2u);
+    sorted = !(fl & 4u);
+    const bool nodup = !(fl & 8u);
+    if (symmetric == N2V2R_SYM_NO) {
+      transpose_a();
+    } else if (symmetric == N2V2R_SYM_DETECT) {
+      lookup = sorted && nodup && sym_lookup_enabled();
+      if (lookup) {
+        HIPCHK(n2v2r_launch_csr_sym_lookup(dip->as<int64_t>(), dix->as<int32_t>(),
+                                           unit ? nullptr : ddv->as<float>(), n, dfl + 2, st));
+      } else {
+        transpose_a();
+        const float* tv = unit ? ddv->as<float>() : td->as<float>();
         if (sorted) {
-          HIPCHK(n2v2r_launch_csr_compare(dip.as<int64_t>(), dix.as<int32_t>(), ddv.as<float>(),
-                                          tp.as<int64_t>(), tx.as<int32_t>(), tv, n, nnz,
-                                          flag.as<unsigned>() + 2, st));
+          HIPCHK(n2v2r_launch_csr_compare(dip->as<int64_t>(), dix->as<int32_t>(),
+                                          ddv->as<float>(), tp->as<int64_t>(), tx->as<int32_t>(),
+                                          tv, n, nnz, dfl + 2, st));
         } else {
           DevBuf sp_, sx, sv;
-          transpose(tp.as<int64_t>(), tx.as<int32_t>(), tv, false, sp_, sx, sv);
+          transpose(tp->as<int64_t>(), tx->as<int32_t>(), tv, false, sp_, sx, sv);
           HIPCHK(n2v2r_launch_csr_compare(sp_.as<int64_t>(), sx.as<int32_t>(),
-                                          unit ? ddv.as<float>() : sv.as<float>(),
-                                          tp.as<int64_t>(), tx.as<int32_t>(), tv, n, nnz,
-                                          flag.as<unsigned>() + 2, st));
+                                          unit ? ddv->as<float>() : sv.as<float>(),
+                                          tp->as<int64_t>(), tx->as<int32_t>(), tv, n, nnz,
+                                          dfl + 2, st));
           HIPCHK(hipStreamSynchronize(st));
         }
-        unsigned mism = 0;
-        HIPCHK(hipMemcpyAsync(&mism, flag.as<unsigned>() + 2, sizeof(unsigned),
-                              hipMemcpyDeviceToHost, st));
+      }
+      HIPCHK(hipMemcpyAsync(hfl + 2, dfl + 2, sizeof(unsigned) * 2, hipMemcpyDeviceToHost, st));
+    }
+    return N2V2R_OK;
+  }
+  void finish() {
+    const hipStream_t st = h->stream;
+    HIPCHK(hipStreamSynchronize(st));
+    bool sym = symmetric == N2V2R_SYM_YES;
+    if (symmetric == N2V2R_SYM_DETECT) {
+      sym = hfl[2] == 0 && (!lookup || hfl[3] == 0);
+      if (lookup && !sym) {
+        transpose_a();
         HIPCHK(hipStreamSynchronize(st));
-        sym = mism == 0;
-      }
-    }
-    HIPCHK(hipStreamSynchronize(st));
-    keys[0].release();
-    keys[1].release();
-    pay[0].release();
-    pay[1].release();
+      }
+    }
     auto slice = [&](DevBuf& sip, DevBuf& six, DevBuf& sdv, bool copy_values, DevBuf& oip,
                      DevBuf& oix, DevBuf& odv, int64_t& onnz) {
       int64_t p0 = 0, p1 = 0;
@@ -485,13 +480,178 @@
       slice(gip, gix, gdv, true, L.indptr, L.indices, L.data, L.nnz);
       if (!sym) slice(gtp, gtx, gtd, !unit, L.t_indptr, L.t_indices, L.t_data, L.t_nnz);
     }
+    if (sym) L.drop_col_blocks_t();
     L.unit = unit;
     L.t_unit = unit;
     L.symmetric = sym;
     L.loaded = true;
     h->have_embedding = false;
-    return N2V2R_OK;
-  });
+  }
+};
+
+struct SortScratchRelease {
+  n2v2r_handle* h;
+  ~SortScratchRelease() {
+    (void)hipStreamSynchronize(h->stream);
+    h->ing_keys[0].release();
+    h->ing_keys[1].release();
+    h->ing_pay[0].release();
+    h->ing_pay[1].release();
+  }
+};
+}
+
+extern "C" {
+
+int n2v2r_set_num_layers(n2v2r_handle* h, int num_layers, int64_t n) {
+  if (h && h->multi()) return multi_set_num_layers(h, num_layers, n);
+  return guarded(h, [&]() -> int {
+    if (num_layers < 1 || n < 1 || n > (int64_t)INT32_MAX) {
+      h->set_err("bad layer count %d or node count %lld", num_layers, (long long)n);
+      return N2V2R_ERR_BAD_ARG;
+    }
+    if (num_layers > SPMM_MAX_LAYERS) {
+      h->set_err("at most %d layers are supported", SPMM_MAX_LAYERS);
+      return N2V2R_ERR_BAD_ARG;
+    }
+    h->K = num_layers;
+    h->set_partition(n);
+    h->layers.clear();
+    for (int k = 0; k < num_layers; ++k) h->layers.emplace_back(new LayerDev());
+    h->have_embedding = false;
+    h->ncmp = h->ncols = 0;
+    return N2V2R_OK;
+  });
+}
+
+int n2v2r_set_layer_csr(n2v2r_handle* h, int k, int64_t n, int64_t nnz, const int64_t* indptr,
+                        const int32_t* indices, const float* data, int symmetric) {
+  if (h && h->multi()) return multi_set_layer_csr(h, k, n, nnz, indptr, indices, data, symmetric);
+  return guarded(h, [&]() -> int {
+    if (int bad = csr_args_check(h, k, n, nnz, indptr, indices, data, symmetric)) return bad;
+    for (int64_t r = 0; r < n; ++r)
+      if (indptr[r + 1] < indptr[r]) {
+        h->set_err("layer %d: indptr not monotone", k);
+        return N2V2R_ERR_BAD_ARG;
+      }
+    for (int j = 0; j < h->K; ++j)
+      if (j != k && h->layers[j]->loaded && h->layers[j]->dense) {
+        h->err = "layers must be all CSR or all dense";
+        return N2V2R_ERR_BAD_ARG;
+      }
+    const hipStream_t st = h->stream;
+    h->ensure_copy_stream();
+    SortScratchRelease scratch{h};
+    CsrIngest in(h, k, n, nnz, symmetric);
+    in.alloc();
+    HIPCHK(hipMemcpyAsync(in.dip->p, indptr, sizeof(int64_t) * (n + 1), hipMemcpyHostToDevice, st));
+    const bool ones = nnz > 0 && host_all_ones(nnz, data);
+    if (nnz) {
+      HIPCHK(hipMemcpyAsync(in.dix->p, indices, sizeof(int32_t) * nnz, hipMemcpyHostToDevice, st));
+      if (ones)
+        HIPCHK(hipMemsetD32Async((hipDeviceptr_t)in.ddv->p, 0x3F800000, (size_t)nnz, st));
+      else
+        HIPCHK(hipMemcpyAsync(in.ddv->p, data, sizeof(float) * nnz, hipMemcpyHostToDevice, st));
+    }
+    h->h2d_layer_bytes += 8 * (n + 1) + (ones ? 4 : 8) * nnz;
+    in.scan();
+    if (int bad = in.classify()) return bad;
+    in.finish();
+    return N2V2R_OK;
+  });
+}
+
+int n2v2r_set_layers_csr(n2v2r_handle* h, int num_layers, int64_t n, const int64_t* nnz,
+                         const int64_t* const* indptr, const int32_t* const* indices,
+                         const float* const* data, int symmetric) {
+  if (!h) return N2V2R_ERR_BAD_ARG;
+  if (!nnz || !indptr || !indices || !data || num_layers < 1 || num_layers != h->K) {
+    h->set_err("bad CSR arguments (%d layers for a handle of %d)", num_layers, h->K);
+    return N2V2R_ERR_BAD_ARG;
+  }
+  if (h->multi() || h->comm) {
+    for (int k = 0; k < num_layers; ++k) {
+      const int st = n2v2r_set_layer_csr(h, k, n, nnz[k], indptr[k], indices[k], data[k], symmetric);
+      if (st != N2V2R_OK) {
+        const std::string msg = h->err;
+        (void)n2v2r_set_num_layers(h, num_layers, n);
+        h->err = msg;
+        return st;
+      }
+    }
+    return N2V2R_OK;
+  }
+  const int rc = guarded(h, [&]() -> int {
+    const int K = num_layers;
+    for (auto& L : h->layers) L->loaded = false;
+    h->have_embedding = false;
+    for (int k = 0; k < K; ++k)
+      if (int bad = csr_args_check(h, k, n, nnz[k], indptr[k], indices[k], data[k], symmetric))
+        return bad;
+    h->ensure_copy_stream();
+    n2v2r_stage::Pool& pool = h->stage_pool();
+    const hipStream_t st = h->stream, cs = h->copy;
+    struct Drain {
+      hipStream_t s;
+      ~Drain() { (void)hipStreamSynchronize(s); }
+    } drain{cs};
+    SortScratchRelease scratch{h};
+    HIPCHK(hipEventRecord(h->copy_ev[0], st));
+    HIPCHK(hipStreamWaitEvent(cs, h->copy_ev[0], 0));
+    std::vector<std::unique_ptr<CsrIngest>> in(K);
+    for (int k = 0; k < K; ++k) {
+      in[k].reset(new CsrIngest(h, k, n, nnz[k], symmetric));
+      CsrIngest& I = *in[k];
+      I.alloc();
+      hipError_t ce = hipSuccess;
+      const int64_t* ip = indptr[k];
+      const bool mono = n2v2r_stage::scan_beside(
+          pool, (size_t)n + 1,
+          [&] {
+            ce = hipMemcpyAsync(I.dip->p, ip, sizeof(int64_t) * (n + 1), hipMemcpyHostToDevice, cs);
+          },
+          [&](size_t e0, size_t e1) {
+            return n2v2r_stage::monotone_i64(ip, e0, e1, (size_t)n + 1);
+          });
+      HIPCHK(ce);
+      if (k > 0)
+        if (int bad = in[k - 1]->classify()) return bad;
+      if (!mono) {
+        h->set_err("layer %d: indptr not monotone", k);
+        return N2V2R_ERR_BAD_ARG;
+      }
+      bool ones = false;
+      if (nnz[k]) {
+        const float* dv = data[k];
+        const int32_t* ix = indices[k];
+        ones = n2v2r_stage::scan_beside(
+            pool, (size_t)nnz[k],
+            [&] {
+              ce = hipMemcpyAsync(I.dix->p, ix, sizeof(int32_t) * nnz[k], hipMemcpyHostToDevice, cs);
+            },
+            [&](size_t e0, size_t e1) { return n2v2r_stage::all_ones_f32(dv, e0, e1); });
+        HIPCHK(ce);
+        if (ones)
+          HIPCHK(hipMemsetD32Async((hipDeviceptr_t)I.ddv->p, 0x3F800000, (size_t)nnz[k], cs));
+        else
+          HIPCHK(hipMemcpyAsync(I.ddv->p, dv, sizeof(float) * nnz[k], hipMemcpyHostToDevice, cs));
+      }
+      h->h2d_layer_bytes += 8 * (n + 1) + (ones ? 4 : 8) * nnz[k];
+      HIPCHK(hipEventRecord(h->copy_ev[1], cs));
+      HIPCHK(hipStreamWaitEvent(st, h->copy_ev[1], 0));
+      I.scan();
+      if (k > 0) {
+        in[k - 1]->finish();
+        in[k - 1].reset();
+      }
+    }
+    if (int bad = in[K - 1]->classify()) return bad;
+    in[K - 1]->finish();
+    return N2V2R_OK;
+  });
+  if (rc != N2V2R_OK)
+    for (auto& L : h->layers) L->loaded = false;
+  return rc;
 }
 
 int n2v2r_set_layer_dense(n2v2r_handle* h, int k, int64_t n, const float* A, int symmetric) {
@@ -674,6 +834,13 @@
   });
 }
 
+int n2v2r_layer_symmetric(n2v2r_handle* h, int k) {
+  if (!h) return -1;
+  if (h->multi()) h = h->ranks[0];
+  if (k < 0 || k >= h->K || !h->layers[k]->loaded) return -1;
+  return h->layers[k]->symmetric ? 1 : 0;
+}
+
 int n2v2r_column_sums(n2v2r_handle* h, int k, float* out) {
   if (h && h->multi()) return multi_column_sums(h, k, out);
   return guarded(h, [&]() -> int {
diff --git a/node2vec2rank_amd/csrc/ranking.cpp b/node2vec2rank_amd/csrc/ranking.cpp
--- a/node2vec2rank_amd/csrc/ranking.cpp
+++ b/node2vec2rank_amd/csrc/ranking.cpp
@@ -1,6 +1,12 @@
 #include "engine.h"
 
 using namespace n2v2r_int;
+
+static void result_d2h(n2v2r_handle* h, void* dst, const void* src_dev, size_t bytes) {
+  if (h->ring_wanted(bytes)) return h->ring_d2h(dst, src_dev, bytes);
+  HIPCHK(hipMemcpyAsync(dst, src_dev, bytes, hipMemcpyDeviceToHost, h->stream));
+  HIPCHK(hipStreamSynchronize(h->stream));
+}
 
 extern "C" {
 
@@ -155,9 +161,8 @@
   if (h && h->multi()) h = h->ranks[0];
   return guarded(h, [&]() -> int {
     if (comparison < 0 || comparison >= h->ncmp || !D) return N2V2R_ERR_BAD_ARG;
-    HIPCHK(hipMemcpyAsync(D, h->D.as<double>() + (size_t)comparison * h->ncols * h->n,
-                          sizeof(double) * h->ncols * h->n, hipMemcpyDeviceToHost, h->stream));
-    HIPCHK(hipStreamSynchronize(h->stream));
+    result_d2h(h, D, h->D.as<double>() + (size_t)comparison * h->ncols * h->n,
+               sizeof(double) * h->ncols * h->n);
     return N2V2R_OK;
   });
 }
@@ -170,9 +175,8 @@
       h->err = "n2v2r_rank ran without aggregation (N2V2R_AGG_NONE)";
       return N2V2R_ERR_NOT_READY;
     }
-    HIPCHK(hipMemcpyAsync(borda, h->borda.as<int64_t>() + (size_t)comparison * h->n,
-                          sizeof(int64_t) * h->n, hipMemcpyDeviceToHost, h->stream));
-    HIPCHK(hipStreamSynchronize(h->stream));
+    result_d2h(h, borda, h->borda.as<int64_t>() + (size_t)comparison * h->n,
+               sizeof(int64_t) * h->n);
     return N2V2R_OK;
   });
 }
@@ -217,8 +221,7 @@
     bo.ensure(sizeof(int64_t) * n);
     HIPCHK(hipMemcpyAsync(dd.p, D, sizeof(double) * n * n_cols, hipMemcpyHostToDevice, h->stream));
     run_borda(h, dd.as<double>(), n, n_cols, n_cols, bo.as<int64_t>());
-    HIPCHK(hipMemcpyAsync(borda, bo.p, sizeof(int64_t) * n, hipMemcpyDeviceToHost, h->stream));
-    HIPCHK(hipStreamSynchronize(h->stream));
+    result_d2h(h, borda, bo.p, sizeof(int64_t) * n);
     return N2V2R_OK;
   });
 }
@@ -264,13 +267,13 @@
     }
     run_borda(h, dd.as<double>(), n, n_cols, n_cols, bo.as<int64_t>(), tf.as<int32_t>(),
               n_given > 0 ? &given : nullptr);
-    HIPCHK(hipMemcpyAsync(borda, bo.p, sizeof(int64_t) * n, hipMemcpyDeviceToHost, h->stream));
     if (tied)
       HIPCHK(hipMemcpyAsync(tied, tf.p, sizeof(int32_t) * n_cols, hipMemcpyDeviceToHost,
                             h->stream));
-    HIPCHK(hipStreamSynchronize(h->stream));
-    return N2V2R_OK;
-  });
-}
-
-}
+    result_d2h(h, borda, bo.p, sizeof(int64_t) * n);
+    HIPCHK(hipStreamSynchronize(h->stream));
+    return N2V2R_OK;
+  });
+}
+
+}
diff --git a/node2vec2rank_amd/csrc/stage_ring.h b/node2vec2rank_amd/csrc/stage_ring.h
--- /dev/null
+++ b/node2vec2rank_amd/csrc/stage_ring.h
@@ -0,0 +1,147 @@
+#pragma once
+
+#include <algorithm>
+#include <condition_variable>
+#include <cstddef>
+#include <cstdint>
+#include <cstring>
+#include <functional>
+#include <mutex>
+#include <system_error>
+#include <thread>
+#include <vector>
+
+namespace n2v2r_stage {
+
+constexpr int MAX_WORKERS = 8;
+
+class Pool {
+ public:
+  explicit Pool(int nthreads) {
+    nthreads = std::max(1, std::min(nthreads, MAX_WORKERS));
+    try {
+      for (int t = 1; t < nthreads; ++t) th_.emplace_back([this, t] { loop(t); });
+    } catch (const std::system_error&) {
+    }
+  }
+  Pool(const Pool&) = delete;
+  Pool& operator=(const Pool&) = delete;
+  ~Pool() {
+    {
+      std::lock_guard<std::mutex> lk(m_);
+      stop_ = true;
+    }
+    cv_.notify_all();
+    for (auto& t : th_) t.join();
+  }
+  int threads() const { return (int)th_.size() + 1; }
+  void run(const std::function<void(int)>& fn) {
+    if (th_.empty()) return fn(0);
+    {
+      std::lock_guard<std::mutex> lk(m_);
+      fn_ = &fn;
+      pending_ = (int)th_.size();
+      ++gen_;
+    }
+    cv_.notify_all();
+    fn(0);
+    std::unique_lock<std::mutex> lk(m_);
+    done_.wait(lk, [&] { return pending_ == 0; });
+    fn_ = nullptr;
+  }
+
+ private:
+  void loop(int t) {
+    uint64_t seen = 0;
+    for (;;) {
+      const std::function<void(int)>* fn;
+      {
+        std::unique_lock<std::mutex> lk(m_);
+        cv_.wait(lk, [&] { return stop_ || gen_ != seen; });
+        if (stop_) return;
+        seen = gen_;
+        fn = fn_;
+      }
+      (*fn)(t);
+      std::lock_guard<std::mutex> lk(m_);
+      if (--pending_ == 0) done_.notify_one();
+    }
+  }
+  std::vector<std::thread> th_;
+  std::mutex m_;
+  std::condition_variable cv_, done_;
+  const std::function<void(int)>* fn_ = nullptr;
+  uint64_t gen_ = 0;
+  int pending_ = 0;
+  bool stop_ = false;
+};
+
+struct Ring {
+  unsigned char* base = nullptr;
+  size_t chunk = 0;
+  int slots = 0;
+  unsigned char* slot(int s) const { return base + (size_t)s * chunk; }
+};
+
+inline void piece(size_t nb, int t, int nt, size_t& a, size_t& b) {
+  const size_t per = ((nb + nt - 1) / nt + 63) / 64 * 64;
+  a = std::min(nb, per * (size_t)t);
+  b = std::min(nb, a + per);
+}
+
+inline bool all_ones_f32(const float* v, size_t e0, size_t e1) {
+  bool good = true;
+  for (size_t i = e0; i < e1; ++i) good &= v[i] == 1.0f;
+  return good;
+}
+
+inline bool monotone_i64(const int64_t* v, size_t e0, size_t e1, size_t total) {
+  bool good = true;
+  const size_t last = std::min(e1, total ? total - 1 : 0);
+  for (size_t i = e0; i < last; ++i) good &= v[i] <= v[i + 1];
+  return good;
+}
+
+template <class Beside, class Ok>
+bool scan_beside(Pool& pool, size_t elems, Beside&& beside, Ok&& ok) {
+  const int nt = pool.threads();
+  const int ns = nt > 1 ? nt - 1 : 1;
+  char good[MAX_WORKERS];
+  pool.run([&](int t) {
+    if (t == 0) beside();
+    if (t == 0 && nt > 1) return;
+    const int s = nt > 1 ? t - 1 : 0;
+    const size_t per = (elems + ns - 1) / ns;
+    const size_t e0 = std::min(elems, per * (size_t)s), e1 = std::min(elems, e0 + per);
+    good[s] = ok(e0, e1) ? 1 : 0;
+  });
+  bool all = true;
+  for (int s = 0; s < ns; ++s) all &= good[s] != 0;
+  return all;
+}
+
+template <class Fetch, class Wait>
+void download(Pool& pool, Ring& ring, void* dst_, size_t bytes, Fetch&& fetch, Wait&& wait) {
+  unsigned char* dst = static_cast<unsigned char*>(dst_);
+  const int nt = pool.threads();
+  const size_t nchunks = (bytes + ring.chunk - 1) / ring.chunk;
+  size_t issued = 0;
+  for (size_t c = 0; c < nchunks; ++c) {
+    for (; issued < nchunks && issued < c + (size_t)ring.slots; ++issued) {
+      const size_t off = issued * ring.chunk;
+      const int s = (int)(issued % ring.slots);
+      fetch(s, ring.slot(s), off, std::min(ring.chunk, bytes - off));
+    }
+    const int s = (int)(c % ring.slots);
+    const size_t off = c * ring.chunk, nb = std::min(ring.chunk, bytes - off);
+    wait(s);
+    const unsigned char* from = ring.slot(s);
+    pool.run([&](int t) {
+      size_t a, b;
+      piece(nb, t, nt, a, b);
+      std::memcpy(dst + off + a, from + a, b - a);
+    });
+  }
+}
+
+}
```

New measurement: 692,000 nodes/s (median of 6 runs). No clear change (+0.3%).
